# Kmatsuo57/cell-image-analysis

Measured on AMD Instinct MI355X. Metric: cells/sec screened (CAE fwd + recon-MSE + SVM score), 64x64, higher is better.
Workload: dtype f32 (results in the fp32 error class; the contractions run as split 16-bit products on the matrix pipe, fp32 accumulate: conv1..conv6 as 2 fp16 terms x 3 products with exact power-of-two scales from each cell's own data, the PCA GEMM as 3 bf16 terms x 6 products, conv7's 32 -> 16 channel contraction; 1 GPU; BASELINE.json configs[2]: screening inference, 1000000 synthetic 64x64 crops on one GPU, resident in HBM, CAE fwd + recon MSE/MAE + RobustScaler + PCA(100) + 2x OCSVM score on device; cells_per_gpu=1000000, global_cells=1000000, chunk_cells=65536, detector_train_cells=5000, weights=random init (Glorot, non-trivial BN), seed 42, parallelism=dp1

## Files before the change

### cell-image-analysis_amd/build.py

```python
import os
import subprocess
import sys
from concurrent.futures import ThreadPoolExecutor

HERE = os.path.dirname(os.path.abspath(__file__))
CSRC = os.path.join(HERE, "csrc")
OUT = os.path.join(HERE, "libcellscreen.so")
BUILD = os.path.join(HERE, "build")
SOURCES = ["api.hip", "conv_mfma.hip", "conv_out.hip", "detector.hip", "train.hip", "train_api.hip", "train_generic.hip", "preprocess.hip",
           "conv_wino_cs.hip", "conv12_fused.hip", "conv45_h2.hip", "conv_generic.hip", "conv_generic_x3.hip", "conv_wino_up.hip", "fit.hip", "extract.hip", "segment.hip", "match.hip", "expand.hip", "intensity.hip", "quantile.hip", "texture.hip", "shape.hip", "neighbors.hip", "colocalize.hip", "radial.hip"]
HEADERS = ["common.hpp", "split16.hpp", "kernel_setup.hpp", "api_internal.hpp", "train_internal.hpp", "segment_internal.hpp", "stage_host.hpp", "label_tile.hpp", "label_boxes.hpp", "hull_chain.hpp", "tensor_archive.hpp", os.path.join("..", "..", "include", "cellscreen.h")]
HIPCC = os.environ.get("HIPCC", "/opt/rocm/bin/hipcc")
FLAGS = ["-O3", "--offload-arch=gfx950", "-fPIC", "-std=c++17", "-Wall", "-Wno-unused-function",
         "-fno-gpu-rdc"]


def source_hash():
    import hashlib
    h = hashlib.sha256()
    for name in sorted(SOURCES) + sorted(HEADERS):
        with open(os.path.join(CSRC, name), "rb") as f:
            h.update(name.encode() + b"\0" + f.read() + b"\0")
    return h.hexdigest()


def _newer(target, deps):
    if not os.path.exists(target):
        return False
    t = os.path.getmtime(target)
    return all(os.path.getmtime(d) <= t for d in deps)


def build(force=False, keep_temps=False, verbose=True):
    os.makedirs(BUILD, exist_ok=True)
    hdrs = [os.path.join(CSRC, h) for h in HEADERS]
    jobs = []
    objs = []
    for src in SOURCES:
        s = os.path.join(CSRC, src)
        o = os.path.join(BUILD, src.replace(".hip", ".o"))
        objs.append(o)
        if force or not _newer(o, [s] + hdrs):
            cmd = [HIPCC] + FLAGS + ["-c", s, "-o", o]
            if keep_temps:
                cmd += ["-save-temps=obj", "-Rpass-analysis=kernel-resource-usage"]
            jobs.append(cmd)

    def run(cmd):
        r = subprocess.run(cmd, capture_output=True, text=True, cwd=BUILD)
        return cmd, r

    if jobs:
        with ThreadPoolExecutor(max_workers=4) as ex:
            for cmd, r in ex.map(run, jobs):
                if verbose and (r.stdout.strip() or r.stderr.strip()):
                    sys.stderr.write(r.stdout + r.stderr)
                if r.returncode != 0:
                    raise RuntimeError("hipcc failed: " + " ".join(cmd) + "\n" + r.stderr)
    if force or jobs or not _newer(OUT, objs):
        cmd = [HIPCC, "--offload-arch=gfx950", "-shared", "-fPIC", "-o", OUT] + objs
        r = subprocess.run(cmd, capture_output=True, text=True)
        if r.returncode != 0:
            raise RuntimeError("link failed: " + r.stderr)
    return OUT


if __name__ == "__main__":
    print(build(force="--force" in sys.argv, keep_temps="--keep-temps" in sys.argv))
```

### cell-image-analysis_amd/csrc/api.hip

```cpp
#include "api_internal.hpp"
#include "tensor_archive.hpp"

using namespace cs;

static thread_local std::string g_err;

namespace cs {
int fail(int code, const char* fmt, ...)
{
    char buf[1024];
    va_list ap;
    va_start(ap, fmt);
    vsnprintf(buf, sizeof buf, fmt, ap);
    va_end(ap);
    g_err = buf;
    return code;
}
const char* last_error_cstr() { return g_err.c_str(); }
}

static const char* kKernelNames[K_COUNT] = {"conv1_relu_bn_pool", "conv2_relu_bn_pool", "conv3_relu_bn_pool",
                                            "conv4_relu_bn",      "conv5_up_relu_bn",   "conv6_up_relu_bn",
                                            "conv7_up_sigmoid_err", "scaler_pca",       "ocsvm_decision",
                                            "finalize",           "synth_crops",        "conv6_conv7_fused_err",
                                            "conv1_conv2_fused"};

struct ConvSet {
    DevBuf winocs[3];
    DevBuf c12w1;
    DevBuf c3h2, c4h2, c5h2, c6h2;
    float c3h2_inv = 1.0f, c4h2_inv = 1.0f, c5h2_inv = 1.0f, c6h2_inv = 1.0f;
    DevBuf c12w1h2;
    float c12w1h2_inv = 1.0f;
    DevBuf c12h2;
    float c12h2_inv = 1.0f, p1a = 0.0f, p1b = 0.0f;
    DevBuf c12;
    DevBuf winoup[6];
    DevBuf wfrag[6];
    DevBuf ep[6];
    int n = 0;
};

struct GenSet {
    DevBuf w[CS_MAX_CONV], ep[CS_MAX_CONV], wf[CS_MAX_CONV], wx3[CS_MAX_CONV];
    bool folded[CS_MAX_CONV] = {false}, x3[CS_MAX_CONV] = {false};
    DevBuf wh2[CS_MAX_CONV];
    float h2_inv[CS_MAX_CONV] = {0};
};

struct Arch {
    bool ref = true;
    int H = kH, W = kW, n_conv = kNConv, n_enc = kNEnc;
    int ch[CS_MAX_CONV] = {0};
    int gh[CS_MAX_CONV] = {0}, gw[CS_MAX_CONV] = {0};
    size_t floats[CS_MAX_CONV] = {0};
    size_t npix = (size_t)kH * kW;
    size_t feat() const { return floats[n_enc - 1]; }
    int cin(int l) const { return l == 0 ? 1 : ch[l - 1]; }
};

struct ProfEvent { int kid; hipEvent_t a, b; int64_t cells; };

constexpr int64_t kPackedResultCells = 65536;

struct cs_model {
    int device = 0;
    hipStream_t stream = nullptr;
    hipStream_t copy_stream = nullptr;
    hipEvent_t ev_in[2] = {nullptr, nullptr}, ev_used[2] = {nullptr, nullptr};
    Arch arch;
    ConvSet ae, enc;
    GenSet gae, genc;
    bool shared_encoder = true;
    int precision = CS_PRECISION_SPLIT16;
    unsigned debug_flags = 0;
    bool split16 = true;
    bool fuse12 = true, fuse45 = true, fuse67 = true, small_split = true;
    int errparts = 4;
    DevBuf w7eff, b7;
    bool has_det = false;
    int F = 0, fpad = 0, C = 0, cpad = 0;
    DevBuf center, scale, comps, comps_x3, mean_proj;
    struct Svm { DevBuf svT, svn, coef; int nsv = 0, nsv_pad = 0; double gamma = 0, rho = 0; } svm[2];
    int64_t chunk = 0;
    int64_t ws_cells = 0;
    DevBuf xin, xin2, act[CS_MAX_CONV], featE, pca, errpart, dec[2], o_mse, o_mae, o_sc[2], o_pr[2], recon;
    DevBuf det_ws;
    DevBuf o_pack;
    void* h_pack = nullptr;
    size_t h_pack_bytes = 0;
    bool prof = false;
    std::vector<ProfEvent> pending;
    double prof_ms[K_COUNT] = {0};
    int64_t prof_launches[K_COUNT] = {0};
    int64_t prof_cells[K_COUNT] = {0};
    ~cs_model()
    {
        if (h_pack) (void)hipHostFree(h_pack);
        for (auto& e : pending) { (void)hipEventDestroy(e.a); (void)hipEventDestroy(e.b); }
        for (int i = 0; i < 2; ++i) {
            if (ev_in[i]) (void)hipEventDestroy(ev_in[i]);
            if (ev_used[i]) (void)hipEventDestroy(ev_used[i]);
        }
        if (copy_stream) (void)hipStreamDestroy(copy_stream);
        if (stream) (void)hipStreamDestroy(stream);
    }
};

namespace cs {
int upload(DevBuf& d, const void* src, size_t bytes)
{
    int rc = d.ensure(bytes ? bytes : 16);
    if (rc) return rc;
    if (bytes) HIPCHK(hipMemcpy(d.p, src, bytes, hipMemcpyHostToDevice));
    return CS_OK;
}

int check_arch(const cs_cae_weights* w, int expect_convs, const char* what)
{
    if (!w) return fail(CS_ERR_INVALID, "%s weights are NULL", what);
    if (w->height != kH || w->width != kW)
        return fail(CS_ERR_UNSUPPORTED, "%s: input %dx%d unsupported (this build has kernels for 64x64)", what, w->height, w->width);
    if (w->n_conv != expect_convs || (expect_convs == kNConv && w->n_enc != kNEnc))
        return fail(CS_ERR_UNSUPPORTED, "%s: n_conv=%d n_enc=%d unsupported (expected %d/%d)", what, w->n_conv, w->n_enc, expect_convs, kNEnc);
    for (int l = 0; l < expect_convs; ++l) {
        if (w->channels[l] != kRefChannels[l])
            return fail(CS_ERR_UNSUPPORTED, "%s: conv %d has %d filters, this build expects %d", what, l, w->channels[l], kRefChannels[l]);
        if (!w->kernel[l] || !w->bias[l]) return fail(CS_ERR_INVALID, "%s: conv %d kernel/bias is NULL", what, l);
        const bool has_bn = l < kNConv - 1;
        if (has_bn && (!w->bn_gamma[l] || !w->bn_beta[l] || !w->bn_mean[l] || !w->bn_var[l]))
            return fail(CS_ERR_INVALID, "%s: conv %d BatchNormalization arrays are NULL", what, l);
    }
    return CS_OK;
}

int describe_arch(const cs_cae_weights* w, Arch& a)
{
    if (!w) return fail(CS_ERR_INVALID, "autoencoder weights are NULL");
    a.H = w->height; a.W = w->width; a.n_conv = w->n_conv; a.n_enc = w->n_enc;
    if (a.n_conv < 3 || a.n_conv > CS_MAX_CONV || a.n_enc < 1 || a.n_conv != 2 * a.n_enc + 1)
        return fail(CS_ERR_UNSUPPORTED, "autoencoder: n_conv=%d n_enc=%d is not the reference grammar (n_conv = 2 n_enc + 1)", a.n_conv, a.n_enc);
    if (a.H <= 0 || a.W <= 0 || a.H % (1 << a.n_enc) || a.W % (1 << a.n_enc))
        return fail(CS_ERR_UNSUPPORTED, "autoencoder: input %dx%d is not divisible by 2^n_enc", a.H, a.W);
    a.ref = a.H == kH && a.W == kW && a.n_conv == kNConv && a.n_enc == kNEnc;
    for (int l = 0; l < a.n_conv; ++l) {
        a.ch[l] = w->channels[l];
        if (a.ch[l] <= 0) return fail(CS_ERR_INVALID, "autoencoder: conv %d has %d filters", l, a.ch[l]);
        if (a.ref && a.ch[l] != kRefChannels[l]) a.ref = false;
    }
    if (a.ch[a.n_conv - 1] != 1) return fail(CS_ERR_UNSUPPORTED, "autoencoder: the last conv must have 1 filter (has %d)", a.ch[a.n_conv - 1]);
    int h = a.H, wd = a.W;
    for (int l = 0; l < a.n_conv; ++l) {
        if (l > a.n_enc) { h *= 2; wd *= 2; }
        a.gh[l] = h; a.gw[l] = wd;
        if (l < a.n_enc) { h /= 2; wd /= 2; }
        a.floats[l] = (size_t)h * wd * a.ch[l];
    }
    a.npix = (size_t)a.H * a.W;
    if (!a.ref) {
        char why[160];
        for (int l = 0; l < a.n_conv; ++l)
            if (!conv_generic_supported(a.gh[l], a.gw[l], a.cin(l), a.ch[l], why, sizeof why))
                return fail(CS_ERR_UNSUPPORTED, "autoencoder conv %d: %s", l, why);
    }
    for (int l = 0; l < a.n_conv; ++l) {
        if (!w->kernel[l] || !w->bias[l]) return fail(CS_ERR_INVALID, "autoencoder: conv %d kernel/bias is NULL", l);
        if (l < a.n_conv - 1 && (!w->bn_gamma[l] || !w->bn_beta[l] || !w->bn_mean[l] || !w->bn_var[l]))
            return fail(CS_ERR_INVALID, "autoencoder: conv %d BatchNormalization arrays are NULL", l);
    }
    return CS_OK;
}

int check_encoder(const cs_cae_weights* e, const Arch& a)
{
    if (e->height != a.H || e->width != a.W || e->n_conv != a.n_enc)
        return fail(CS_ERR_UNSUPPORTED, "encoder: %dx%d with %d convs does not match the autoencoder's encoder half (%dx%d, %d)",
                    e->height, e->width, e->n_conv, a.H, a.W, a.n_enc);
    for (int l = 0; l < a.n_enc; ++l) {
        if (e->channels[l] != a.ch[l]) return fail(CS_ERR_UNSUPPORTED, "encoder: conv %d has %d filters, the autoencoder %d", l, e->channels[l], a.ch[l]);
        if (!e->kernel[l] || !e->bias[l] || !e->bn_gamma[l] || !e->bn_beta[l] || !e->bn_mean[l] || !e->bn_var[l])
            return fail(CS_ERR_INVALID, "encoder: conv %d arrays are NULL", l);
    }
    return CS_OK;
}

int require_gfx950(int device_id)
{
    int ndev = 0;
    if (hipGetDeviceCount(&ndev) != hipSuccess || ndev <= 0)
        return fail(CS_ERR_NO_DEVICE, "no HIP device visible; libcellscreen has no CPU path");
    if (device_id < 0 || device_id >= ndev) return fail(CS_ERR_INVALID, "device_id %d out of range [0,%d)", device_id, ndev);
    HIPCHK(hipSetDevice(device_id));
    hipDeviceProp_t prop;
    HIPCHK(hipGetDeviceProperties(&prop, device_id));
    if (strncmp(prop.gcnArchName, "gfx950", 6) != 0)
        return fail(CS_ERR_NO_DEVICE, "device %d is %s; this library is built for gfx950 only", device_id, prop.gcnArchName);
    return CS_OK;
}
}

static int pack_set(ConvSet& set, const cs_cae_weights* w, int count)
{
    std::vector<float> tmp;
    for (int l = 0; l < count; ++l) {
        const int cin = l == 0 ? 1 : kRefChannels[l - 1], cout = kRefChannels[l];
        const bool folded = (l == 4 || l == 5);
        const size_t nf = folded ? pack_conv_fragments_folded(cin, cout, nullptr, nullptr) : pack_conv_fragments(cin, cout, nullptr, nullptr);
        tmp.resize(nf);
        if (folded) pack_conv_fragments_folded(cin, cout, w->kernel[l], tmp.data());
        else pack_conv_fragments(cin, cout, w->kernel[l], tmp.data());
        int rc = upload(set.wfrag[l], tmp.data(), nf * sizeof(float));
        if (rc) return rc;
        std::vector<float> ep(3 * cout);
        for (int c = 0; c < cout; ++c) {
            const float s = w->bn_gamma[l][c] / sqrtf(w->bn_var[l][c] + w->bn_eps);
            ep[c] = w->bias[l][c];
            ep[cout + c] = s;
            ep[2 * cout + c] = w->bn_beta[l][c] - w->bn_mean[l][c] * s;
        }
        rc = upload(set.ep[l], ep.data(), ep.size() * sizeof(float));
        if (rc) return rc;
        if (l == 4 || l == 5) {
            tmp.resize(pack_wino_up_fragments(l, nullptr, nullptr));
            pack_wino_up_fragments(l, w->kernel[l], tmp.data());
            rc = upload(set.winoup[l], tmp.data(), tmp.size() * sizeof(float));
            if (rc) return rc;
        }
        if (l == 1 || l == 2) {
            tmp.resize(pack_wino_cs_fragments(l, nullptr, nullptr));
            pack_wino_cs_fragments(l, w->kernel[l], tmp.data());
            rc = upload(set.winocs[l], tmp.data(), tmp.size() * sizeof(float));
            if (rc) return rc;
        }
        if (l == 2) {
            std::vector<uint16_t> h2(pack_wino3_h2(nullptr, nullptr, nullptr));
            pack_wino3_h2(w->kernel[l], h2.data(), &set.c3h2_inv);
            rc = upload(set.c3h2, h2.data(), h2.size() * sizeof(uint16_t));
            if (rc) return rc;
        }
        if (l == 3) {
            std::vector<uint16_t> h2(pack_conv4_f16x2(nullptr, nullptr, nullptr));
            pack_conv4_f16x2(w->kernel[l], h2.data(), &set.c4h2_inv);
            rc = upload(set.c4h2, h2.data(), h2.size() * sizeof(uint16_t));
            if (rc) return rc;
        }
        if (l == 4) {
            std::vector<float> weff(pack_generic_folded(cin, cout, nullptr, nullptr));
            pack_generic_folded(cin, cout, w->kernel[l], weff.data());
            std::vector<uint16_t> h2(pack_conv5_f16x2(nullptr, nullptr, nullptr));
            pack_conv5_f16x2(weff.data(), h2.data(), &set.c5h2_inv);
            rc = upload(set.c5h2, h2.data(), h2.size() * sizeof(uint16_t));
            if (rc) return rc;
        }
        if (l == 5) {
            std::vector<float> weff(pack_generic_folded(cin, cout, nullptr, nullptr));
            pack_generic_folded(cin, cout, w->kernel[l], weff.data());
            std::vector<uint16_t> h2(pack_conv6_f16x2(nullptr, nullptr, nullptr));
            pack_conv6_f16x2(weff.data(), h2.data(), &set.c6h2_inv);
            rc = upload(set.c6h2, h2.data(), h2.size() * sizeof(uint16_t));
            if (rc) return rc;
        }
        if (l == 0) {
            tmp.resize(pack_conv12_conv1_fragments(nullptr, nullptr, nullptr));
            pack_conv12_conv1_fragments(w->kernel[l], ep.data() + cout, tmp.data());
            rc = upload(set.c12w1, tmp.data(), tmp.size() * sizeof(float));
            if (rc) return rc;
            pack_conv12_p1_bound(w->kernel[l], ep.data(), &set.p1a, &set.p1b);
            std::vector<unsigned int> wh(pack_conv12_conv1_h2(nullptr, nullptr, nullptr, nullptr));
            pack_conv12_conv1_h2(w->kernel[l], ep.data() + cout, wh.data(), &set.c12w1h2_inv);
            rc = upload(set.c12w1h2, wh.data(), wh.size() * sizeof(unsigned int));
            if (rc) return rc;
        }
        if (l == 1) {
            tmp.resize(pack_conv12_fragments(nullptr, nullptr, nullptr));
            pack_conv12_fragments(w->kernel[l], ep.data() + cout, tmp.data());
            rc = upload(set.c12, tmp.data(), tmp.size() * sizeof(float));
            if (rc) return rc;
            std::vector<unsigned int> uh(pack_conv12_fragments_h2(nullptr, nullptr, nullptr, nullptr));
            pack_conv12_fragments_h2(w->kernel[l], ep.data() + cout, uh.data(), &set.c12h2_inv);
            rc = upload(set.c12h2, uh.data(), uh.size() * sizeof(unsigned int));
            if (rc) return rc;
        }
    }
    set.n = count;
    return CS_OK;
}

static int pack_generic(GenSet& set, const cs_cae_weights* w, const Arch& a, int count, bool split16)
{
    for (int l = 0; l < count; ++l) {
        const int cin = a.cin(l), cout = a.ch[l];
        int rc = upload(set.w[l], w->kernel[l], sizeof(float) * 9 * cin * cout);
        if (rc) return rc;
        set.folded[l] = l > a.n_enc && ((l < a.n_conv - 1 && conv_generic_folds(a.gh[l], a.gw[l], cin, cout)) ||
                                        (l == a.n_conv - 1 && cout == 1 && cin % 4 == 0));
        if (set.folded[l]) {
            std::vector<float> wf(pack_generic_folded(cin, cout, nullptr, nullptr));
            pack_generic_folded(cin, cout, w->kernel[l], wf.data());
            if ((rc = upload(set.wf[l], wf.data(), wf.size() * sizeof(float)))) return rc;
            if (split16 && l == a.n_conv - 1 && cout == 1 && conv_last_x3_takes(a.gh[l], a.gw[l], cin)) {
                std::vector<uint16_t> pl(pack_last_bf16x3(cin, nullptr, nullptr));
                pack_last_bf16x3(cin, wf.data(), pl.data());
                if ((rc = upload(set.wx3[l], pl.data(), pl.size() * sizeof(uint16_t)))) return rc;
                set.x3[l] = true;
            }
            if (split16 && l < a.n_conv - 1 && conv_generic_x3_takes(a.gh[l], a.gw[l], cin, cout, 1)) {
                std::vector<uint16_t> pl(pack_generic_bf16x3(16, cin, cout, nullptr, nullptr));
                pack_generic_bf16x3(16, cin, cout, wf.data(), pl.data());
                if ((rc = upload(set.wx3[l], pl.data(), pl.size() * sizeof(uint16_t)))) return rc;
                set.x3[l] = true;
                std::vector<uint16_t> ph(pack_generic_f16x2(16, cin, cout, nullptr, nullptr, nullptr));
                pack_generic_f16x2(16, cin, cout, wf.data(), ph.data(), &set.h2_inv[l]);
                if ((rc = upload(set.wh2[l], ph.data(), ph.size() * sizeof(uint16_t)))) return rc;
            }
        } else if (split16 && l <= a.n_enc && l < a.n_conv - 1 && conv_generic_x3_takes(a.gh[l], a.gw[l], cin, cout, 0)) {
            std::vector<uint16_t> pl(pack_generic_bf16x3(9, cin, cout, nullptr, nullptr));
            pack_generic_bf16x3(9, cin, cout, w->kernel[l], pl.data());
            if ((rc = upload(set.wx3[l], pl.data(), pl.size() * sizeof(uint16_t)))) return rc;
            set.x3[l] = true;
            std::vector<uint16_t> ph(pack_generic_f16x2(9, cin, cout, nullptr, nullptr, nullptr));
            pack_generic_f16x2(9, cin, cout, w->kernel[l], ph.data(), &set.h2_inv[l]);
            if ((rc = upload(set.wh2[l], ph.data(), ph.size() * sizeof(uint16_t)))) return rc;
        }
        std::vector<float> ep(3 * cout, 0.0f);
        const bool has_bn = w->bn_gamma[l] != nullptr;
        for (int c = 0; c < cout; ++c) {
            ep[c] = w->bias[l][c];
            if (has_bn) {
                const float s_ = w->bn_gamma[l][c] / sqrtf(w->bn_var[l][c] + w->bn_eps);
                ep[cout + c] = s_;
                ep[2 * cout + c] = w->bn_beta[l][c] - w->bn_mean[l][c] * s_;
            }
        }
        if ((rc = upload(set.ep[l], ep.data(), ep.size() * sizeof(float)))) return rc;
    }
    return CS_OK;
}

static bool same_encoder(const cs_cae_weights* a, const cs_cae_weights* e, const Arch& ar)
{
    if (a->bn_eps != e->bn_eps) return false;
    for (int l = 0; l < ar.n_enc; ++l) {
        const int cin = ar.cin(l), cout = ar.ch[l];
        if (memcmp(a->kernel[l], e->kernel[l], sizeof(float) * 9 * cin * cout)) return false;
        if (memcmp(a->bias[l], e->bias[l], sizeof(float) * cout)) return false;
        if (memcmp(a->bn_gamma[l], e->bn_gamma[l], sizeof(float) * cout)) return false;
        if (memcmp(a->bn_beta[l], e->bn_beta[l], sizeof(float) * cout)) return false;
        if (memcmp(a->bn_mean[l], e->bn_mean[l], sizeof(float) * cout)) return false;
        if (memcmp(a->bn_var[l], e->bn_var[l], sizeof(float) * cout)) return false;
    }
    return true;
}

static int pack_svm(cs_model::Svm& s, const cs_ocsvm_params& p, int D, const char* what)
{
    if (p.n_sv <= 0 || !p.support_vectors || !p.dual_coef)
        return fail(CS_ERR_INVALID, "%s detector: n_sv=%d or NULL arrays", what, p.n_sv);
    s.nsv = p.n_sv;
    s.nsv_pad = (p.n_sv + 15) / 16 * 16;
    s.gamma = p.gamma;
    s.rho = p.rho;
    std::vector<double> svT((size_t)D * s.nsv_pad, 0.0), coef(s.nsv_pad, 0.0), svn(s.nsv_pad, 0.0);
    for (int i = 0; i < p.n_sv; ++i) {
        coef[i] = p.dual_coef[i];
        double nn = 0.0;
        for (int d = 0; d < D; ++d) {
            const double v = p.support_vectors[(size_t)i * D + d];
            svT[(size_t)d * s.nsv_pad + i] = v;
            nn = fma(v, v, nn);
        }
        svn[i] = nn;
    }
    {
        int rcn = upload(s.svn, svn.data(), svn.size() * sizeof(double));
        if (rcn) return rcn;
    }
    int rc = upload(s.svT, svT.data(), svT.size() * sizeof(double));
    if (rc) return rc;
    return upload(s.coef, coef.data(), coef.size() * sizeof(double));
}

static int64_t eff_chunk(const cs_model* m, int in_kind)
{
    if (m->chunk > 0) return m->chunk;
    if (in_kind == CS_MEM_HOST) return 16384;
    size_t per_cell = m->arch.npix * sizeof(float);
    for (int l = 0; l < m->arch.n_conv - 1; ++l) per_cell += m->arch.floats[l] * sizeof(float);
    int64_t c = (int64_t)((size_t)28e9 / (per_cell ? per_cell : 1));
    c = c / 1024 * 1024;
    return c < 1024 ? 1024 : (c > 65536 ? 65536 : c);
}

static int ensure_workspace(cs_model* m, int64_t cells, bool need_recon)
{
    if (cells > m->ws_cells) {
        int rc;
        if ((rc = m->xin.ensure((size_t)cells * m->arch.npix * sizeof(float)))) return rc;
        const bool skip_p1 = m->arch.ref && m->fuse12;
        for (int l = skip_p1 ? 1 : 0; l < m->arch.n_conv - 1; ++l)
            if ((rc = m->act[l].ensure((size_t)cells * m->arch.floats[l] * sizeof(float)))) return rc;
        if ((rc = m->featE.ensure((size_t)cells * m->arch.feat() * sizeof(float)))) return rc;
        if ((rc = m->pca.ensure((size_t)cells * 256 * sizeof(float)))) return rc;
        if (m->small_split && (rc = m->det_ws.ensure(det_split_ws_bytes(m->C)))) return rc;
        if ((rc = m->errpart.ensure((size_t)cells * 16 * sizeof(float)))) return rc;
        for (int d = 0; d < 2; ++d) {
            if ((rc = m->dec[d].ensure((size_t)cells * sizeof(double)))) return rc;
            if ((rc = m->o_sc[d].ensure((size_t)cells * sizeof(double)))) return rc;
            if ((rc = m->o_pr[d].ensure((size_t)cells))) return rc;
        }
        if ((rc = m->o_mse.ensure((size_t)cells * sizeof(float)))) return rc;
        if ((rc = m->o_mae.ensure((size_t)cells * sizeof(float)))) return rc;
        m->ws_cells = cells;
    }
    if (need_recon || !m->arch.ref) {
        int rc = m->recon.ensure((size_t)m->ws_cells * m->arch.npix * sizeof(float));
        if (rc) return rc;
    }
    return CS_OK;
}

struct Launch {
    cs_model* m; int kid; int64_t cells; ProfEvent ev; bool on;
    Launch(cs_model* m_, int kid_, int64_t cells_) : m(m_), kid(kid_), cells(cells_), on(m_->prof)
    {
        if (on) {
            ev.kid = kid; ev.cells = cells;
            if (hipEventCreate(&ev.a) != hipSuccess || hipEventCreate(&ev.b) != hipSuccess) { on = false; return; }
            (void)hipEventRecord(ev.a, m->stream);
        }
    }
    ~Launch()
    {
        if (on) { (void)hipEventRecord(ev.b, m->stream); m->pending.push_back(ev); }
    }
};

static int drain_profile(cs_model* m)
{
    for (auto& e : m->pending) {
        float ms = 0.0f;
        if (hipEventElapsedTime(&ms, e.a, e.b) == hipSuccess) {
            m->prof_ms[e.kid] += ms;
            m->prof_launches[e.kid] += 1;
            m->prof_cells[e.kid] += e.cells;
        }
        (void)hipEventDestroy(e.a);
        (void)hipEventDestroy(e.b);
    }
    m->pending.clear();
    return CS_OK;
}

#define LAUNCH(kid, cells, call)                                                              \
    do {                                                                                      \
        hipError_t le__;                                                                      \
        { Launch l__(m, kid, cells); le__ = (call); }                                         \
        if (le__ != hipSuccess)                                                               \
            return fail(CS_ERR_HIP, "launch %s failed: %s", kKernelNames[kid], hipGetErrorString(le__)); \
    } while (0)

static int run_convs_generic(cs_model* m, const GenSet& set, const float* x, int64_t nc, int first, int last, float* recon)
{
    const Arch& a = m->arch;
    for (int l = first; l <= last; ++l) {
        const float* in = l == 0 ? x : m->act[l - 1].as<float>();
        const bool is_last = l == a.n_conv - 1;
        float* out = is_last ? (recon ? recon : m->recon.as<float>()) : m->act[l].as<float>();
        const int epi = is_last ? GEN_EPI_SIGMOID : (l < a.n_enc ? GEN_EPI_BN_POOL : GEN_EPI_BN);
        const int kid = l < 6 ? K_CONV1 + l : K_CONV7_ERR;
        if (set.x3[l] && m->split16 && is_last) {
            LAUNCH(kid, nc,
                   launch_conv_last_x3(in, set.wx3[l].as<uint16_t>(), set.ep[l].as<float>(), out, nc, a.gh[l], a.gw[l], a.cin(l), m->stream));
            LAUNCH(K_CONV7_ERR, nc, launch_recon_err(out, x, nc, (int)a.npix, m->errpart.as<float>(), m->stream));
            continue;
        }
        if (set.x3[l] && m->split16) {
            const bool h2 = set.h2_inv[l] != 0.0f;
            LAUNCH(kid, nc,
                   launch_conv_generic_x3(in, h2 ? set.wh2[l].as<uint16_t>() : set.wx3[l].as<uint16_t>(), set.ep[l].as<float>(), out, nc,
                                          a.gh[l], a.gw[l], a.cin(l), a.ch[l], l > a.n_enc, epi, m->stream, h2 ? set.h2_inv[l] : 0.0f));
            continue;
        }
        LAUNCH(kid, nc,
               launch_conv_generic(in, set.w[l].as<float>(), set.ep[l].as<float>(), out, nc, a.gh[l], a.gw[l], a.cin(l), a.ch[l],
                                   l > a.n_enc, epi, m->stream, set.folded[l] ? set.wf[l].as<float>() : nullptr));
        if (is_last)
            LAUNCH(K_CONV7_ERR, nc, launch_recon_err(out, x, nc, (int)a.npix, m->errpart.as<float>(), m->stream));
    }
    m->errparts = 4;
    return CS_OK;
}

static int run_convs(cs_model* m, const ConvSet& set, const float* x, int64_t nc, int first, int last,
                     float* recon)
{
    if (!m->arch.ref) return run_convs_generic(m, &set == &m->enc ? m->genc : m->gae, x, nc, first, last, recon);
    const bool fused = m->fuse67 && first <= 5 && last >= 6 && !recon;
    const bool fused12 = m->fuse12 && first == 0 && last >= 1;
    const bool h2 = m->split16;
    if (fused12) {
        LAUNCH(K_CONV12_FUSED, nc,
               launch_conv12_fused(x, set.c12w1.as<float>(), set.ep[0].as<float>(), set.c12.as<float>(), set.ep[1].as<float>(),
                                   m->act[1].as<float>(), nc, m->stream, h2 ? set.c12h2.as<unsigned int>() : nullptr, set.p1a, set.p1b,
                                   set.c12h2_inv, h2 ? set.c12w1h2.as<unsigned int>() : nullptr, set.c12w1h2_inv));
    }
    if (!fused12 && first == 0) {
        int rc = m->act[0].ensure((size_t)m->ws_cells * m->arch.floats[0] * sizeof(float));
        if (rc) return rc;
    }
    const bool fused45 = m->fuse45 && h2 && first <= 3 && last >= 4;
    for (int l = fused12 ? 2 : first; l <= last && l < (fused ? 5 : 6); ++l) {
        const float* in = l == 0 ? x : m->act[l - 1].as<float>();
        if (l == 3 && fused45) {
            LAUNCH(K_CONV5, nc,
                   launch_conv45_h2(in, set.c4h2.as<uint16_t>(), set.c4h2_inv, set.ep[3].as<float>(), set.c5h2.as<uint16_t>(), set.c5h2_inv,
                                    set.ep[4].as<float>(), m->act[4].as<float>(), nc, m->stream));
            ++l;
            continue;
        }
        if (l == 4 && h2) {
            LAUNCH(K_CONV5, nc,
                   launch_conv5_h2(in, set.c5h2.as<uint16_t>(), set.c5h2_inv, set.ep[l].as<float>(), m->act[l].as<float>(), nc, m->stream));
            continue;
        }
        if (l == 4 || l == 5) {
            LAUNCH(K_CONV1 + l, nc,
                   launch_conv_wino_up(l, in, set.winoup[l].as<float>(), set.ep[l].as<float>(), m->act[l].as<float>(), nc, m->stream));
            continue;
        }
        if (l == 2 && h2) {
            LAUNCH(K_CONV3, nc,
                   launch_conv3_wino_h2(in, set.c3h2.as<uint16_t>(), set.c3h2_inv, set.ep[l].as<float>(), m->act[l].as<float>(), nc, m->stream));
            continue;
        }
        if (l == 1 || l == 2) {
            LAUNCH(K_CONV1 + l, nc,
                   launch_conv_wino_cs(l, in, set.winocs[l].as<float>(), set.ep[l].as<float>(), m->act[l].as<float>(), nc, m->stream));
            continue;
        }
        if (l == 3 && h2) {
            LAUNCH(K_CONV4, nc,
                   launch_conv4_h2(in, set.c4h2.as<uint16_t>(), set.c4h2_inv, set.ep[l].as<float>(), m->act[l].as<float>(), nc, m->stream));
            continue;
        }
        LAUNCH(K_CONV1 + l, nc,
               launch_conv_mfma(l, in, set.wfrag[l].as<float>(), set.ep[l].as<float>(), m->act[l].as<float>(), nc, m->stream, false));
    }
    if (fused && h2) {
        LAUNCH(K_CONV67_FUSED, nc,
               launch_conv67_h2(m->act[4].as<float>(), set.c6h2.as<uint16_t>(), set.c6h2_inv, set.ep[5].as<float>(), x, m->w7eff.as<float>(),
                                m->b7.as<float>(), m->errpart.as<float>(), nc, m->stream));
        m->errparts = conv67_fused_nparts();
    } else if (fused) {
        LAUNCH(K_CONV67_FUSED, nc,
               launch_conv67_fused(m->act[4].as<float>(), set.winoup[5].as<float>(), set.ep[5].as<float>(), x, m->w7eff.as<float>(),
                                   m->b7.as<float>(), m->errpart.as<float>(), nc, m->stream));
        m->errparts = conv67_fused_nparts();
    } else if (last >= 6) {
        LAUNCH(K_CONV7_ERR, nc,
               launch_conv7_err(m->act[5].as<float>(), x, m->w7eff.as<float>(), m->b7.as<float>(), m->errpart.as<float>(), recon, nc, m->stream));
        m->errparts = 4;
    }
    return CS_OK;
}

struct DrainGuard {
    cs_model* m;
    bool armed = true;
    explicit DrainGuard(cs_model* mm) : m(mm) {}
    ~DrainGuard()
    {
        if (armed && m) {
            if (m->copy_stream) (void)hipStreamSynchronize(m->copy_stream);
            if (m->stream) (void)hipStreamSynchronize(m->stream);
        }
    }
    int done(int rc) { armed = false; return rc; }
};

static int begin_call(cs_model* m)
{
    if (!m) return fail(CS_ERR_INVALID, "model handle is NULL");
    HIPCHK(hipSetDevice(m->device));
    return CS_OK;
}

static int end_call(cs_model* m)
{
    HIPCHK(hipStreamSynchronize(m->stream));
    return drain_profile(m);
}

static int stage_in(cs_model* m, const float* base, int kind, int64_t off, int64_t nc, size_t per_cell,
                    DevBuf& staging, const float** dev)
{
    if (kind == CS_MEM_DEVICE) { *dev = base + (size_t)off * per_cell; return CS_OK; }
    int rc = staging.ensure((size_t)nc * per_cell * sizeof(float));
    if (rc) return rc;
    HIPCHK(hipMemcpyAsync(staging.p, base + (size_t)off * per_cell, (size_t)nc * per_cell * sizeof(float),
                          hipMemcpyHostToDevice, m->stream));
    *dev = staging.as<float>();
    return CS_OK;
}

template <class T>
static int stage_out(cs_model* m, T* user, int kind, int64_t off, int64_t count, const T* dev)
{
    if (!user || kind == CS_MEM_DEVICE) return CS_OK;
    HIPCHK(hipMemcpyAsync(user + off, dev, (size_t)count * sizeof(T), hipMemcpyDeviceToHost, m->stream));
    return CS_OK;
}

template <class T>
static T* out_ptr(T* user, int kind, int64_t off, DevBuf& tmp)
{
    if (!user) return nullptr;
    return kind == CS_MEM_DEVICE ? user + off : tmp.as<T>();
}

static int check_kind(int k, const char* what)
{
    if (k != CS_MEM_HOST && k != CS_MEM_DEVICE) return fail(CS_ERR_INVALID, "%s must be CS_MEM_HOST or CS_MEM_DEVICE", what);
    return CS_OK;
}

extern "C" {

int cs_abi_version(void) { return CS_ABI_VERSION; }

const char* cs_status_string(int s)
{
    switch (s) {
        case CS_OK: return "ok";
        case CS_ERR_INVALID: return "invalid argument";
        case CS_ERR_IO: return "i/o error";
        case CS_ERR_FORMAT: return "malformed model file";
        case CS_ERR_NO_DEVICE: return "no usable gfx950 device";
        case CS_ERR_HIP: return "HIP runtime error";
        case CS_ERR_UNSUPPORTED: return "unsupported architecture or size";
        case CS_ERR_NOMEM: return "out of memory";
        case CS_ERR_NO_DETECTOR: return "model has no detector parameters";
        default: return "unknown status";
    }
}

const char* cs_last_error(void) { return last_error_cstr(); }

int cs_device_count(void)
{
    int n = 0;
    if (hipGetDeviceCount(&n) != hipSuccess) return 0;
    return n;
}

static int resolve_options(const cs_model_options* o, int* precision, unsigned* flags)
{
    *precision = CS_PRECISION_SPLIT16;
    *flags = 0;
    if (o) {
        if (o->struct_size < 12 || o->struct_size > 4096) return fail(CS_ERR_INVALID, "cs_model_options.struct_size = %u (set it to sizeof(cs_model_options))", o->struct_size);
        if (o->precision != CS_PRECISION_SPLIT16 && o->precision != CS_PRECISION_FP32_EXACT)
            return fail(CS_ERR_INVALID, "cs_model_options.precision = %d (CS_PRECISION_SPLIT16 or CS_PRECISION_FP32_EXACT)", o->precision);
        const unsigned known = CS_DEBUG_NO_FUSE12 | CS_DEBUG_NO_FUSE45 | CS_DEBUG_NO_FUSE67 | CS_DEBUG_NO_SMALL_SPLIT;
        if (o->debug_flags & ~known) return fail(CS_ERR_INVALID, "cs_model_options.debug_flags = 0x%x has unknown bits", o->debug_flags);
        if (o->struct_size >= sizeof(cs_model_options))
            for (unsigned r : o->reserved) if (r) return fail(CS_ERR_INVALID, "cs_model_options.reserved must be 0");
        *precision = o->precision;
        *flags = o->debug_flags;
    }
    if (const char* e = getenv("CS_DEBUG_PRECISION")) {
        if (!strcmp(e, "exact")) *precision = CS_PRECISION_FP32_EXACT;
        else if (!strcmp(e, "split16")) *precision = CS_PRECISION_SPLIT16;
        else return fail(CS_ERR_INVALID, "CS_DEBUG_PRECISION=%s (exact or split16)", e);
    }
    if (const char* e = getenv("CS_DEBUG_FLAGS")) *flags |= (unsigned)strtoul(e, nullptr, 0) & 0xfu;
    return CS_OK;
}

int cs_model_from_arrays(const cs_cae_weights* autoencoder, const cs_cae_weights* encoder,
                         const cs_detector_params* det, int device_id, const cs_model_options* options, cs_model** out)
{
    if (!out) return fail(CS_ERR_INVALID, "out is NULL");
    *out = nullptr;
    int precision;
    unsigned dflags;
    {
        int rco = resolve_options(options, &precision, &dflags);
        if (rco) return rco;
    }
    Arch arch;
    int rc = describe_arch(autoencoder, arch);
    if (rc) return rc;
    if (arch.ref && (rc = check_arch(autoencoder, kNConv, "autoencoder"))) return rc;
    if (encoder && (rc = check_encoder(encoder, arch))) return rc;
    if ((rc = require_gfx950(device_id))) return rc;

    cs_model* m = new (std::nothrow) cs_model();
    if (!m) return fail(CS_ERR_NOMEM, "host allocation failed");
    m->device = device_id;
    m->arch = arch;
    m->precision = precision;
    m->debug_flags = dflags;
    m->split16 = precision == CS_PRECISION_SPLIT16;
    m->fuse12 = !(dflags & CS_DEBUG_NO_FUSE12);
    m->fuse45 = !(dflags & CS_DEBUG_NO_FUSE45);
    m->fuse67 = !(dflags & CS_DEBUG_NO_FUSE67);
    m->small_split = !(dflags & CS_DEBUG_NO_SMALL_SPLIT);
#define FAIL_IF(x) do { int r__ = (x); if (r__) { delete m; return r__; } } while (0)
    {
        hipError_t e = hipStreamCreateWithFlags(&m->stream, hipStreamNonBlocking);
        if (e == hipSuccess) e = hipStreamCreateWithFlags(&m->copy_stream, hipStreamNonBlocking);
        for (int i = 0; i < 2 && e == hipSuccess; ++i) {
            e = hipEventCreateWithFlags(&m->ev_in[i], hipEventDisableTiming);
            if (e == hipSuccess) e = hipEventCreateWithFlags(&m->ev_used[i], hipEventDisableTiming);
        }
        if (e != hipSuccess) { delete m; return fail(CS_ERR_HIP, "stream/event creation: %s", hipGetErrorString(e)); }
    }
    if (arch.ref) {
        FAIL_IF(pack_set(m->ae, autoencoder, 6));
        float weff[16 * 32];
        conv7_effective_weights(autoencoder->kernel[6], weff);
        FAIL_IF(upload(m->w7eff, weff, sizeof weff));
        FAIL_IF(upload(m->b7, autoencoder->bias[6], sizeof(float)));
    } else {
        FAIL_IF(pack_generic(m->gae, autoencoder, arch, arch.n_conv, m->split16));
    }
    m->shared_encoder = !encoder || same_encoder(autoencoder, encoder, arch);
    if (!m->shared_encoder) {
        if (arch.ref) FAIL_IF(pack_set(m->enc, encoder, kNEnc));
        else FAIL_IF(pack_generic(m->genc, encoder, arch, arch.n_enc, m->split16));
    }

    if (det) {
        if (det->n_features != (int)arch.feat()) {
            delete m;
            return fail(CS_ERR_INVALID, "detector n_features=%d but the encoder emits %zu", det->n_features, arch.feat());
        }
        if (det->n_components <= 0 || det->n_components > 128 || !det->scaler_center || !det->scaler_scale ||
            !det->pca_components || !det->pca_mean_proj) {
            delete m;
            return fail(CS_ERR_INVALID, "detector: n_components=%d (1..128) or NULL arrays", det->n_components);
        }
        m->F = det->n_features;
        m->fpad = (m->F + 511) / 512 * 512;
        m->C = det->n_components;
        m->cpad = (m->C + 15) / 16 * 16;
        FAIL_IF(upload(m->center, det->scaler_center, sizeof(float) * m->F));
        FAIL_IF(upload(m->scale, det->scaler_scale, sizeof(double) * m->F));
        std::vector<float> cp((size_t)m->cpad * m->fpad, 0.0f);
        for (int c = 0; c < m->C; ++c)
            memcpy(&cp[(size_t)c * m->fpad], det->pca_components + (size_t)c * m->F, sizeof(float) * m->F);
        FAIL_IF(upload(m->comps, cp.data(), cp.size() * sizeof(float)));
        {
            std::vector<uint16_t> pl(pack_pca_bf16x3(nullptr, m->cpad, m->fpad, nullptr));
            pack_pca_bf16x3(cp.data(), m->cpad, m->fpad, pl.data());
            FAIL_IF(upload(m->comps_x3, pl.data(), pl.size() * sizeof(uint16_t)));
        }
        FAIL_IF(upload(m->mean_proj, det->pca_mean_proj, sizeof(float) * m->C));
        FAIL_IF(pack_svm(m->svm[0], det->conservative, m->C, "conservative"));
        FAIL_IF(pack_svm(m->svm[1], det->moderate, m->C, "moderate"));
        m->has_det = true;
    }
#undef FAIL_IF
    *out = m;
    return CS_OK;
}

static int fill_weights(const TensorArchive& ar, const std::string& prefix, int n_conv, cs_cae_weights* w,
                        const std::string& path)
{
    for (int l = 0; l < n_conv; ++l) {
        const int cin = l == 0 ? 1 : w->channels[l - 1], cout = w->channels[l];
        const std::string cl = prefix + ".conv" + std::to_string(l), bl = prefix + ".bn" + std::to_string(l);
        const Tensor* k = ar.get(cl + ".kernel");
        const Tensor* b = ar.get(cl + ".bias");
        if (!k || !b || !k->f32() || !b->f32() || k->numel() != (size_t)9 * cin * cout || b->numel() != (size_t)cout)
            return fail(CS_ERR_FORMAT, "%s: missing or mis-shaped %s.kernel/.bias", path.c_str(), cl.c_str());
        w->kernel[l] = k->f32();
        w->bias[l] = b->f32();
        if (l < w->n_conv - 1 || prefix == "enc") {
            const Tensor* g = ar.get(bl + ".gamma"); const Tensor* be = ar.get(bl + ".beta");
            const Tensor* mu = ar.get(bl + ".mean"); const Tensor* va = ar.get(bl + ".var");
            if (!g || !be || !mu || !va || !g->f32() || !be->f32() || !mu->f32() || !va->f32() ||
                g->numel() != (size_t)cout || be->numel() != (size_t)cout || mu->numel() != (size_t)cout || va->numel() != (size_t)cout)
                return fail(CS_ERR_FORMAT, "%s: missing or mis-shaped %s.*", path.c_str(), bl.c_str());
            w->bn_gamma[l] = g->f32(); w->bn_beta[l] = be->f32(); w->bn_mean[l] = mu->f32(); w->bn_var[l] = va->f32();
        }
    }
    return CS_OK;
}

static int fill_svm(const TensorArchive& ar, const std::string& prefix, int C, cs_ocsvm_params* p, const std::string& path)
{
    const Tensor* sv = ar.get(prefix + ".sv"); const Tensor* dc = ar.get(prefix + ".dual_coef");
    const Tensor* g = ar.get(prefix + ".gamma"); const Tensor* r = ar.get(prefix + ".rho");
    if (!sv || !dc || !g || !r || !sv->f64() || !dc->f64() || !g->f64() || !r->f64() || sv->dims.size() != 2 ||
        sv->dims[1] != (uint64_t)C || dc->numel() != sv->dims[0] || g->numel() != 1 || r->numel() != 1)
        return fail(CS_ERR_FORMAT, "%s: missing or mis-shaped %s.*", path.c_str(), prefix.c_str());
    p->n_sv = (int32_t)sv->dims[0];
    p->support_vectors = sv->f64();
    p->dual_coef = dc->f64();
    p->gamma = g->f64()[0];
    p->rho = r->f64()[0];
    return CS_OK;
}

int cs_model_load(const char* model_dir, int device_id, const cs_model_options* options, cs_model** out)
{
    if (!out) return fail(CS_ERR_INVALID, "out is NULL");
    *out = nullptr;
    if (!model_dir) return fail(CS_ERR_INVALID, "model_dir is NULL");
    const std::string dir(model_dir);
    TensorArchive cae, det;
    std::string err = cae.load(dir + "/cae.bin");
    if (!err.empty()) return fail(err.rfind("cannot open", 0) == 0 ? CS_ERR_IO : CS_ERR_FORMAT, "%s", err.c_str());

    const Tensor* meta = cae.get("meta");
    const Tensor* eps = cae.get("bn_eps");
    if (!meta || !meta->i32() || meta->numel() < 5 || !eps || !eps->f32() || eps->numel() != 1)
        return fail(CS_ERR_FORMAT, "%s/cae.bin: missing meta / bn_eps", model_dir);
    const int32_t* mi = meta->i32();
    cs_cae_weights ae;
    memset(&ae, 0, sizeof ae);
    ae.height = mi[0]; ae.width = mi[1]; ae.n_conv = mi[2]; ae.n_enc = mi[3];
    if (ae.n_conv < 2 || ae.n_conv > CS_MAX_CONV || meta->numel() != (size_t)(4 + ae.n_conv))
        return fail(CS_ERR_FORMAT, "%s/cae.bin: bad meta", model_dir);
    for (int l = 0; l < ae.n_conv; ++l) ae.channels[l] = mi[4 + l];
    ae.bn_eps = eps->f32()[0];
    int rc = fill_weights(cae, "ae", ae.n_conv, &ae, dir + "/cae.bin");
    if (rc) return rc;

    cs_cae_weights en;
    const cs_cae_weights* enp = nullptr;
    if (cae.get("enc.conv0.kernel")) {
        en = ae;
        en.n_conv = ae.n_enc;
        for (int l = 0; l < CS_MAX_CONV; ++l) en.kernel[l] = en.bias[l] = en.bn_gamma[l] = en.bn_beta[l] = en.bn_mean[l] = en.bn_var[l] = nullptr;
        rc = fill_weights(cae, "enc", en.n_conv, &en, dir + "/cae.bin");
        if (rc) return rc;
        enp = &en;
    }

    cs_detector_params dp;
    const cs_detector_params* dpp = nullptr;
    FILE* probe = fopen((dir + "/detector.bin").c_str(), "rb");
    if (probe) {
        fclose(probe);
        err = det.load(dir + "/detector.bin");
        if (!err.empty()) return fail(CS_ERR_FORMAT, "%s", err.c_str());
        memset(&dp, 0, sizeof dp);
        const Tensor* ce = det.get("scaler.center"); const Tensor* sc = det.get("scaler.scale");
        const Tensor* co = det.get("pca.components"); const Tensor* mp = det.get("pca.mean_proj");
        if (!ce || !sc || !co || !mp || !ce->f32() || !sc->f64() || !co->f32() || !mp->f32() || co->dims.size() != 2 ||
            ce->numel() != co->dims[1] || sc->numel() != co->dims[1] || mp->numel() != co->dims[0])
            return fail(CS_ERR_FORMAT, "%s/detector.bin: missing or mis-shaped scaler/pca tensors", model_dir);
        dp.n_features = (int32_t)co->dims[1];
        dp.n_components = (int32_t)co->dims[0];
        dp.scaler_center = ce->f32(); dp.scaler_scale = sc->f64();
        dp.pca_components = co->f32(); dp.pca_mean_proj = mp->f32();
        if ((rc = fill_svm(det, "svm_conservative", dp.n_components, &dp.conservative, dir + "/detector.bin"))) return rc;
        if ((rc = fill_svm(det, "svm_moderate", dp.n_components, &dp.moderate, dir + "/detector.bin"))) return rc;
        dpp = &dp;
    }
    return cs_model_from_arrays(&ae, enp, dpp, device_id, options, out);
}

void cs_model_free(cs_model* m)
{
    if (!m) return;
    (void)hipSetDevice(m->device);
    if (m->stream) (void)hipStreamSynchronize(m->stream);
    delete m;
}

int cs_model_get_info(const cs_model* m, cs_model_info* info)
{
    if (!m || !info) return fail(CS_ERR_INVALID, "NULL argument");
    memset(info, 0, sizeof *info);
    info->height = m->arch.H; info->width = m->arch.W; info->n_conv = m->arch.n_conv; info->n_enc = m->arch.n_enc;
    info->feature_dim = (int32_t)m->arch.feat();
    for (int l = 0; l < m->arch.n_conv; ++l) info->channels[l] = m->arch.ch[l];
    info->reference_arch = m->arch.ref ? 1 : 0;
    info->precision = m->precision;
    info->debug_flags = m->debug_flags;
    info->n_components = m->C;
    info->n_sv_conservative = m->svm[0].nsv;
    info->n_sv_moderate = m->svm[1].nsv;
    info->shared_encoder = m->shared_encoder ? 1 : 0;
    info->has_detector = m->has_det ? 1 : 0;
    info->device_id = m->device;
    info->chunk_cells = eff_chunk(m, CS_MEM_DEVICE);
    return CS_OK;
}

int cs_model_set_chunk(cs_model* m, int64_t chunk_cells)
{
    if (!m || chunk_cells < 0 || chunk_cells > (1 << 20)) return fail(CS_ERR_INVALID, "chunk_cells must be in [0, 2^20] (0 = automatic)");
    m->chunk = chunk_cells;
    return CS_OK;
}

static int run_tail(cs_model* m, const float* feat, int64_t nc, float* mse, float* mae, double* sc, double* sm,
                    int8_t* pc, int8_t* pm, bool with_err)
{
    if (m->split16)
        LAUNCH(K_SCALER_PCA, nc,
               launch_scaler_pca_x3(feat, m->center.as<float>(), m->scale.as<double>(), m->comps_x3.as<uint16_t>(),
                                    m->mean_proj.as<float>(), m->F, m->fpad, m->C, m->cpad, m->pca.as<float>(), nc, m->stream, m->det_ws.p));
    else
        LAUNCH(K_SCALER_PCA, nc,
               launch_scaler_pca(feat, m->center.as<float>(), m->scale.as<double>(), m->comps.as<float>(),
                                 m->mean_proj.as<float>(), m->F, m->fpad, m->C, m->cpad, m->pca.as<float>(), nc, m->stream));
    if (m->det_ws.p && nc <= DET_SPLIT_MAX_CELLS) {
        const double* svT[2] = {m->svm[0].svT.as<double>(), m->svm[1].svT.as<double>()};
        const double* svn[2] = {m->svm[0].svn.as<double>(), m->svm[1].svn.as<double>()};
        const double* coef[2] = {m->svm[0].coef.as<double>(), m->svm[1].coef.as<double>()};
        const int nsv[2] = {m->svm[0].nsv_pad, m->svm[1].nsv_pad};
        const double gam[2] = {m->svm[0].gamma, m->svm[1].gamma}, rho[2] = {m->svm[0].rho, m->svm[1].rho};
        LAUNCH(K_SVM, nc,
               launch_ocsvm_pair_split(m->pca.as<float>(), m->C, svT, svn, coef, nsv, gam, rho, m->dec[0].as<double>(), m->dec[1].as<double>(), nc,
                                       m->stream, m->det_ws.p));
    } else
    for (int d = 0; d < 2; ++d)
        LAUNCH(K_SVM, nc,
               launch_ocsvm(m->pca.as<float>(), m->C, m->svm[d].svT.as<double>(), m->svm[d].svn.as<double>(), m->svm[d].coef.as<double>(),
                            m->svm[d].nsv_pad, m->svm[d].gamma, m->svm[d].rho, m->dec[d].as<double>(), nc, m->stream, m->det_ws.p));
    LAUNCH(K_FINALIZE, nc,
           launch_finalize(with_err ? m->errpart.as<float>() : nullptr, m->errparts, (int)m->arch.npix, m->dec[0].as<double>(),
                           m->dec[1].as<double>(), mse, mae, sc, sm, pc, pm, nc, m->stream));
    return CS_OK;
}

int cs_screen(cs_model* m, const float* crops, int64_t n, int crops_kind, float* mse, float* mae,
              double* cons_score, double* mod_score, int8_t* cons_pred, int8_t* mod_pred, int out_kind)
{
    int rc = begin_call(m);
    if (rc) return rc;
    DrainGuard guard(m);
    if (n < 0) return fail(CS_ERR_INVALID, "n is negative");
    if (n == 0) return guard.done(CS_OK);
    if (!crops) return fail(CS_ERR_INVALID, "crops is NULL");
    if ((rc = check_kind(crops_kind, "crops_kind")) || (rc = check_kind(out_kind, "out_kind"))) return rc;
    if (!m->has_det) return fail(CS_ERR_NO_DETECTOR, "cs_screen needs detector parameters");
    const int64_t cc = eff_chunk(m, crops_kind);
    const int64_t ch = n < cc ? n : cc;
    if ((rc = ensure_workspace(m, ch, false))) return rc;
    const bool host_in = crops_kind == CS_MEM_HOST, host_out = out_kind == CS_MEM_HOST;
    const size_t in_bytes = m->arch.npix * sizeof(float);
    DevBuf* stage[2] = {&m->xin, &m->xin2};
    const bool single = n <= ch;
    if (host_in) {
        if ((rc = m->xin.ensure((size_t)ch * in_bytes)) || (n > ch && (rc = m->xin2.ensure((size_t)ch * in_bytes)))) return rc;
        HIPCHK(hipMemcpyAsync(m->xin.p, crops, (size_t)ch * in_bytes, hipMemcpyHostToDevice, single ? m->stream : m->copy_stream));
        if (!single) HIPCHK(hipEventRecord(m->ev_in[0], m->copy_stream));
    }
    const size_t o_off[6] = {0, (size_t)n * 8, (size_t)n * 16, (size_t)n * 20, (size_t)n * 24, (size_t)n * 25};
    const size_t o_total = (size_t)n * 26;
    const bool pack_out = host_out && n <= kPackedResultCells;
    if (host_out) {
        if ((rc = m->o_pack.ensure(o_total))) return rc;
        if (pack_out && m->h_pack_bytes < o_total) {
            if (m->h_pack) { (void)hipHostFree(m->h_pack); m->h_pack = nullptr; m->h_pack_bytes = 0; }
            const size_t cap = (size_t)kPackedResultCells * 26;
            HIPCHK(hipHostMalloc(&m->h_pack, cap, hipHostMallocDefault));
            m->h_pack_bytes = cap;
        }
    }
    char* const o_base = (char*)m->o_pack.p;
    auto dst = [&](auto* user, int which, int64_t off) -> decltype(user) {
        if (!user) return nullptr;
        return host_out ? (decltype(user))(o_base + o_off[which]) + off : user + off;
    };
    auto drain = [&](int code) {
        (void)hipStreamSynchronize(m->copy_stream);
        (void)hipStreamSynchronize(m->stream);
        return code;
    };
    int64_t i = 0;
    for (int64_t off = 0; off < n; off += ch, ++i) {
        const int64_t nc = (n - off) < ch ? (n - off) : ch;
        const int b = (int)(i & 1);
        const float* x = crops + (size_t)off * m->arch.npix;
        if (host_in) {
            if (!single) HIPCHK(hipStreamWaitEvent(m->stream, m->ev_in[b], 0));
            x = stage[b]->as<float>();
        }
        if ((rc = run_convs(m, m->ae, x, nc, 0, m->arch.n_conv - 1, nullptr))) return drain(rc);
        const float* feat = m->act[m->arch.n_enc - 1].as<float>();
        if (!m->shared_encoder) {
            if ((rc = run_convs(m, m->enc, x, nc, 0, m->arch.n_enc - 1, nullptr))) return drain(rc);
            feat = m->act[m->arch.n_enc - 1].as<float>();
        }
        if ((rc = run_tail(m, feat, nc, dst(mse, 2, off), dst(mae, 3, off), dst(cons_score, 0, off),
                           dst(mod_score, 1, off), dst(cons_pred, 4, off), dst(mod_pred, 5, off), true)))
            return drain(rc);
        if (host_in && !single) {
            HIPCHK(hipEventRecord(m->ev_used[b], m->stream));
            const int64_t noff = off + ch;
            if (noff < n) {
                const int64_t nn = (n - noff) < ch ? (n - noff) : ch;
                if (i >= 1) HIPCHK(hipStreamWaitEvent(m->copy_stream, m->ev_used[b ^ 1], 0));
                HIPCHK(hipMemcpyAsync(stage[b ^ 1]->p, crops + (size_t)noff * m->arch.npix, (size_t)nn * in_bytes, hipMemcpyHostToDevice,
                                      m->copy_stream));
                HIPCHK(hipEventRecord(m->ev_in[b ^ 1], m->copy_stream));
            }
        }
    }
    if (pack_out) {
        HIPCHK(hipMemcpyAsync(m->h_pack, o_base, o_total, hipMemcpyDeviceToHost, m->stream));
        if (host_in) HIPCHK(hipStreamSynchronize(m->copy_stream));
        const int erc = end_call(m);
        if (erc) return guard.done(erc);
        const char* h = (const char*)m->h_pack;
        if (cons_score) memcpy(cons_score, h + o_off[0], (size_t)n * 8);
        if (mod_score) memcpy(mod_score, h + o_off[1], (size_t)n * 8);
        if (mse) memcpy(mse, h + o_off[2], (size_t)n * 4);
        if (mae) memcpy(mae, h + o_off[3], (size_t)n * 4);
        if (cons_pred) memcpy(cons_pred, h + o_off[4], (size_t)n);
        if (mod_pred) memcpy(mod_pred, h + o_off[5], (size_t)n);
        return guard.done(CS_OK);
    }
    if (host_out) {
        if (mse) HIPCHK(hipMemcpyAsync(mse, o_base + o_off[2], (size_t)n * sizeof(float), hipMemcpyDeviceToHost, m->stream));
        if (mae) HIPCHK(hipMemcpyAsync(mae, o_base + o_off[3], (size_t)n * sizeof(float), hipMemcpyDeviceToHost, m->stream));
        if (cons_score) HIPCHK(hipMemcpyAsync(cons_score, o_base + o_off[0], (size_t)n * sizeof(double), hipMemcpyDeviceToHost, m->stream));
        if (mod_score) HIPCHK(hipMemcpyAsync(mod_score, o_base + o_off[1], (size_t)n * sizeof(double), hipMemcpyDeviceToHost, m->stream));
        if (cons_pred) HIPCHK(hipMemcpyAsync(cons_pred, o_base + o_off[4], (size_t)n, hipMemcpyDeviceToHost, m->stream));
        if (mod_pred) HIPCHK(hipMemcpyAsync(mod_pred, o_base + o_off[5], (size_t)n, hipMemcpyDeviceToHost, m->stream));
    }
    if (host_in) HIPCHK(hipStreamSynchronize(m->copy_stream));
    return guard.done(end_call(m));
}

int cs_reconstruct(cs_model* m, const float* crops, int64_t n, int crops_kind, float* recon, float* mse,
                   float* mae, int out_kind)
{
    int rc = begin_call(m);
    if (rc) return rc;
    DrainGuard guard(m);
    if (n < 0) return fail(CS_ERR_INVALID, "n is negative");
    if (n == 0) return guard.done(CS_OK);
    if (!crops) return fail(CS_ERR_INVALID, "crops is NULL");
    if ((rc = check_kind(crops_kind, "crops_kind")) || (rc = check_kind(out_kind, "out_kind"))) return rc;
    const int64_t cc = eff_chunk(m, crops_kind);
    const int64_t ch = n < cc ? n : cc;
    const bool host_recon = recon && out_kind == CS_MEM_HOST;
    if ((rc = ensure_workspace(m, ch, host_recon))) return rc;
    for (int64_t off = 0; off < n; off += ch) {
        const int64_t nc = (n - off) < ch ? (n - off) : ch;
        const float* x;
        if ((rc = stage_in(m, crops, crops_kind, off, nc, m->arch.npix, m->xin, &x))) return rc;
        float* d_rec = !recon ? nullptr : (out_kind == CS_MEM_DEVICE ? recon + (size_t)off * m->arch.npix : m->recon.as<float>());
        if ((rc = run_convs(m, m->ae, x, nc, 0, m->arch.n_conv - 1, d_rec))) return rc;
        float* d_mse = out_ptr(mse, out_kind, off, m->o_mse);
        float* d_mae = out_ptr(mae, out_kind, off, m->o_mae);
        LAUNCH(K_FINALIZE, nc,
               launch_finalize(m->errpart.as<float>(), m->errparts, (int)m->arch.npix, nullptr, nullptr, d_mse, d_mae, nullptr, nullptr,
                               nullptr, nullptr, nc, m->stream));
        if ((rc = stage_out(m, mse, out_kind, off, nc, d_mse))) return rc;
        if ((rc = stage_out(m, mae, out_kind, off, nc, d_mae))) return rc;
        if (host_recon)
            HIPCHK(hipMemcpyAsync(recon + (size_t)off * m->arch.npix, d_rec, (size_t)nc * m->arch.npix * sizeof(float),
                                  hipMemcpyDeviceToHost, m->stream));
        if (crops_kind == CS_MEM_HOST || out_kind == CS_MEM_HOST) HIPCHK(hipStreamSynchronize(m->stream));
    }
    return guard.done(end_call(m));
}

int cs_encode(cs_model* m, const float* crops, int64_t n, int crops_kind, int which, float* features, int out_kind)
{
    int rc = begin_call(m);
    if (rc) return rc;
    DrainGuard guard(m);
    if (n < 0) return fail(CS_ERR_INVALID, "n is negative");
    if (n == 0) return guard.done(CS_OK);
    if (!crops || !features) return fail(CS_ERR_INVALID, "crops/features is NULL");
    if (which != 0 && which != 1) return fail(CS_ERR_INVALID, "which must be 0 (autoencoder) or 1 (encoder.keras)");
    if ((rc = check_kind(crops_kind, "crops_kind")) || (rc = check_kind(out_kind, "out_kind"))) return rc;
    const int64_t cc = eff_chunk(m, crops_kind);
    const int64_t ch = n < cc ? n : cc;
    if ((rc = ensure_workspace(m, ch, false))) return rc;
    const ConvSet& set = (which == 1 && !m->shared_encoder) ? m->enc : m->ae;
    const size_t fl = m->arch.feat();
    for (int64_t off = 0; off < n; off += ch) {
        const int64_t nc = (n - off) < ch ? (n - off) : ch;
        const float* x;
        if ((rc = stage_in(m, crops, crops_kind, off, nc, m->arch.npix, m->xin, &x))) return rc;
        if ((rc = run_convs(m, set, x, nc, 0, m->arch.n_enc - 1, nullptr))) return rc;
        HIPCHK(hipMemcpyAsync(features + (size_t)off * fl, m->act[m->arch.n_enc - 1].p, (size_t)nc * fl * sizeof(float),
                              out_kind == CS_MEM_DEVICE ? hipMemcpyDeviceToDevice : hipMemcpyDeviceToHost, m->stream));
        HIPCHK(hipStreamSynchronize(m->stream));
    }
    return guard.done(end_call(m));
}

int cs_layer_output(cs_model* m, const float* crops, int64_t n, int crops_kind, int layer, float* out, int out_kind)
{
    int rc = begin_call(m);
    if (rc) return rc;
    DrainGuard guard(m);
    if (n < 0) return fail(CS_ERR_INVALID, "n is negative");
    if (n == 0) return guard.done(CS_OK);
    if (!crops || !out) return fail(CS_ERR_INVALID, "crops/out is NULL");
    const int last = m->arch.n_conv - 1;
    if (layer < 0 || layer > last) return fail(CS_ERR_INVALID, "layer must be in [0,%d]", last);
    if ((rc = check_kind(crops_kind, "crops_kind")) || (rc = check_kind(out_kind, "out_kind"))) return rc;
    const int64_t cc = eff_chunk(m, crops_kind);
    const int64_t ch = n < cc ? n : cc;
    if ((rc = ensure_workspace(m, ch, layer == last))) return rc;
    const size_t fl = m->arch.floats[layer];
    for (int64_t off = 0; off < n; off += ch) {
        const int64_t nc = (n - off) < ch ? (n - off) : ch;
        const float* x;
        if ((rc = stage_in(m, crops, crops_kind, off, nc, m->arch.npix, m->xin, &x))) return rc;
        if ((rc = run_convs(m, m->ae, x, nc, 0, layer, layer == last ? m->recon.as<float>() : nullptr))) return rc;
        const void* src = layer == last ? m->recon.p : m->act[layer].p;
        HIPCHK(hipMemcpyAsync(out + (size_t)off * fl, src, (size_t)nc * fl * sizeof(float),
                              out_kind == CS_MEM_DEVICE ? hipMemcpyDeviceToDevice : hipMemcpyDeviceToHost, m->stream));
        HIPCHK(hipStreamSynchronize(m->stream));
    }
    return guard.done(end_call(m));
}

int cs_scaler_pca(cs_model* m, const float* features, int64_t n, int in_kind, float* pca_out, int out_kind)
{
    int rc = begin_call(m);
    if (rc) return rc;
    DrainGuard guard(m);
    if (n < 0) return fail(CS_ERR_INVALID, "n is negative");
    if (n == 0) return guard.done(CS_OK);
    if (!features || !pca_out) return fail(CS_ERR_INVALID, "features/pca_out is NULL");
    if ((rc = check_kind(in_kind, "in_kind")) || (rc = check_kind(out_kind, "out_kind"))) return rc;
    if (!m->has_det) return fail(CS_ERR_NO_DETECTOR, "cs_scaler_pca needs detector parameters");
    const int64_t cc = eff_chunk(m, in_kind);
    const int64_t ch = n < cc ? n : cc;
    if ((rc = ensure_workspace(m, ch, false))) return rc;
    for (int64_t off = 0; off < n; off += ch) {
        const int64_t nc = (n - off) < ch ? (n - off) : ch;
        const float* f;
        if ((rc = stage_in(m, features, in_kind, off, nc, (size_t)m->F, m->featE, &f))) return rc;
        if (m->split16)
            LAUNCH(K_SCALER_PCA, nc,
                   launch_scaler_pca_x3(f, m->center.as<float>(), m->scale.as<double>(), m->comps_x3.as<uint16_t>(),
                                        m->mean_proj.as<float>(), m->F, m->fpad, m->C, m->cpad, m->pca.as<float>(), nc, m->stream, m->det_ws.p));
        else
            LAUNCH(K_SCALER_PCA, nc,
                   launch_scaler_pca(f, m->center.as<float>(), m->scale.as<double>(), m->comps.as<float>(),
                                     m->mean_proj.as<float>(), m->F, m->fpad, m->C, m->cpad, m->pca.as<float>(), nc, m->stream));
        HIPCHK(hipMemcpyAsync(pca_out + (size_t)off * m->C, m->pca.p, (size_t)nc * m->C * sizeof(float),
                              out_kind == CS_MEM_DEVICE ? hipMemcpyDeviceToDevice : hipMemcpyDeviceToHost, m->stream));
        HIPCHK(hipStreamSynchronize(m->stream));
    }
    return guard.done(end_call(m));
}

int cs_svm_decision(cs_model* m, const float* pca, int64_t n, int in_kind, double* cons_dec, double* mod_dec, int out_kind)
{
    int rc = begin_call(m);
    if (rc) return rc;
    DrainGuard guard(m);
    if (n < 0) return fail(CS_ERR_INVALID, "n is negative");
    if (n == 0) return guard.done(CS_OK);
    if (!pca) return fail(CS_ERR_INVALID, "pca is NULL");
    if ((rc = check_kind(in_kind, "in_kind")) || (rc = check_kind(out_kind, "out_kind"))) return rc;
    if (!m->has_det) return fail(CS_ERR_NO_DETECTOR, "cs_svm_decision needs detector parameters");
    const int64_t cc = eff_chunk(m, in_kind);
    const int64_t ch = n < cc ? n : cc;
    if ((rc = ensure_workspace(m, ch, false))) return rc;
    double* outs[2] = {cons_dec, mod_dec};
    for (int64_t off = 0; off < n; off += ch) {
        const int64_t nc = (n - off) < ch ? (n - off) : ch;
        const float* p;
        if ((rc = stage_in(m, pca, in_kind, off, nc, (size_t)m->C, m->pca, &p))) return rc;
        for (int d = 0; d < 2; ++d) {
            if (!outs[d]) continue;
            LAUNCH(K_SVM, nc,
                   launch_ocsvm(p, m->C, m->svm[d].svT.as<double>(), m->svm[d].svn.as<double>(), m->svm[d].coef.as<double>(),
                                m->svm[d].nsv_pad, m->svm[d].gamma, m->svm[d].rho, m->dec[d].as<double>(), nc, m->stream, m->det_ws.p));
            HIPCHK(hipMemcpyAsync(outs[d] + off, m->dec[d].p, (size_t)nc * sizeof(double),
                                  out_kind == CS_MEM_DEVICE ? hipMemcpyDeviceToDevice : hipMemcpyDeviceToHost, m->stream));
        }
        HIPCHK(hipStreamSynchronize(m->stream));
    }
    return guard.done(end_call(m));
}

int cs_synth_crops(cs_model* m, uint64_t seed, int64_t first_cell, int64_t n, int32_t npix, float* out_device)
{
    int rc = begin_call(m);
    if (rc) return rc;
    if (n < 0 || npix <= 0) return fail(CS_ERR_INVALID, "n/npix invalid");
    if (n == 0) return CS_OK;
    if (!out_device) return fail(CS_ERR_INVALID, "out_device is NULL");
    LAUNCH(K_SYNTH, n, launch_synth(seed, first_cell, n, npix, out_device, m->stream));
    return end_call(m);
}

int cs_profile_enable(cs_model* m, int on)
{
    if (!m) return fail(CS_ERR_INVALID, "model handle is NULL");
    m->prof = on != 0;
    return CS_OK;
}

int cs_profile_reset(cs_model* m)
{
    if (!m) return fail(CS_ERR_INVALID, "model handle is NULL");
    for (int k = 0; k < K_COUNT; ++k) { m->prof_ms[k] = 0; m->prof_launches[k] = 0; m->prof_cells[k] = 0; }
    return CS_OK;
}

int cs_model_wait_stream(cs_model* m, void* hip_stream)
{
    if (!m) return fail(CS_ERR_INVALID, "model handle is NULL");
    HIPCHK(hipSetDevice(m->device));
    return wait_on_stream(m->stream, hip_stream);
}

int cs_profile_kernel_count(void) { return K_COUNT; }

const char* cs_profile_kernel_name(int k) { return (k >= 0 && k < K_COUNT) ? kKernelNames[k] : ""; }

int cs_profile_get(cs_model* m, int k, double* total_ms, int64_t* launches, int64_t* cells, double* flops)
{
    if (!m || k < 0 || k >= K_COUNT) return fail(CS_ERR_INVALID, "bad kernel id");
    if (total_ms) *total_ms = m->prof_ms[k];
    if (launches) *launches = m->prof_launches[k];
    if (cells) *cells = m->prof_cells[k];
    if (flops) {
        double per_cell = 0.0;
        if (k <= K_CONV7_ERR) per_cell = 2.0 * kLayerMacs[k];
        else if (k == K_CONV67_FUSED) per_cell = 2.0 * (kLayerMacs[5] + kLayerMacs[6]);
        else if (k == K_CONV12_FUSED) per_cell = 2.0 * (kLayerMacs[0] + kLayerMacs[1]);
        else if (k == K_SCALER_PCA) per_cell = 2.0 * (double)m->F * m->C;
        else if (k == K_SVM) per_cell = 0.0;
        *flops = per_cell * (double)m->prof_cells[k];
    }
    return CS_OK;
}

int cs_profile_mfma_per_cell(cs_model* m, int k, double* mfma)
{
    if (!m || !mfma || k < 0 || k >= K_COUNT) return fail(CS_ERR_INVALID, "bad kernel id");
    double v = 0.0;
    if (k == K_SCALER_PCA) {
        *mfma = m->has_det && !m->split16 ? (double)m->fpad * m->cpad / 1024.0 : 0.0;
        return CS_OK;
    }
    if (m->arch.ref) {
        const bool h2 = m->split16;
        switch (k) {
            case K_CONV1: v = 1536; break;
            case K_CONV2: v = 8192; break;
            case K_CONV3: v = h2 ? 0 : 2048; break;
            case K_CONV4: v = h2 ? 0 : 576; break;
            case K_CONV5: v = h2 ? 0 : 1152; break;
            case K_CONV6: v = 4608; break;
            case K_CONV67_FUSED: v = h2 ? 512 : 4608 + 512; break;
            case K_CONV12_FUSED: v = h2 ? 0 : 4608 + 1536 + 48; break;
            default: v = 0.0;
        }
    } else if (k <= K_CONV6 || k == K_CONV7_ERR) {
        const int l = k == K_CONV7_ERR ? m->arch.n_conv - 1 : k - K_CONV1;
        if (l < m->arch.n_conv && !(m->split16 && m->gae.x3[l])) {
            const int cout_pad = (m->arch.ch[l] + 15) / 16 * 16;
            v = (double)m->arch.gh[l] * m->arch.gw[l] / 16.0 * (cout_pad / 16) * (9.0 * m->arch.cin(l) / 4.0);
        }
    }
    *mfma = v;
    return CS_OK;
}

int cs_profile_bf16_mfma_per_cell(cs_model* m, int k, double* mfma)
{
    if (!m || !mfma || k < 0 || k >= K_COUNT) return fail(CS_ERR_INVALID, "bad kernel id");
    double v = 0.0;
    if (!m->split16) { *mfma = 0.0; return CS_OK; }
    if (k == K_SCALER_PCA && m->has_det) {
        *mfma = (double)(m->cpad / 16) * (m->fpad / 32) * 6.0 / 16.0;
        return CS_OK;
    }
    if (m->arch.ref) {
        if (k == K_CONV4) v = 4 * 2 * 9 * 3;
        if (k == K_CONV3) v = 16.0 * 4 * 2 * 2 * 3;
        if (k == K_CONV12_FUSED) v = 66 * 8 * 2 + 36 * 4 * 4 * 3;
        if (k == K_CONV5) v = 4 * 4 * 4 * 4 * 3 + (m->fuse45 ? 4 * 2 * 9 * 3 : 0);
        if (k == K_CONV67_FUSED) v = 4.0 * 16 * 2 * 4 * 2 * 3;
    } else if (k <= K_CONV6) {
        const int l = k - K_CONV1;
        if (l < m->arch.n_conv && m->gae.x3[l]) {
            const int cout_pad = (m->arch.ch[l] + 15) / 16 * 16;
            const double taps = l > m->arch.n_enc ? 4.0 : 9.0;
            const bool last = l == m->arch.n_conv - 1;
            v = (double)m->arch.gh[l] * m->arch.gw[l] / 16.0 * (cout_pad / 16) * taps * (m->arch.cin(l) / 32.0) * ((m->gae.h2_inv[l] != 0.0f && !last) ? 3.0 : 6.0);
        }
    }
    *mfma = v;
    return CS_OK;
}

}
```

### cell-image-analysis_amd/csrc/common.hpp

```cpp
#pragma once
#include <hip/hip_runtime.h>
#include <stdint.h>
#include <stdio.h>

#include "../../include/cellscreen.h"

namespace cs {

typedef float f32x4 __attribute__((ext_vector_type(4)));

struct LayerGeom {
    int H, W, cin, cout;
    bool pool;
    bool ups;
    bool last;
};

enum KernelId {
    K_CONV1 = 0, K_CONV2, K_CONV3, K_CONV4, K_CONV5, K_CONV6, K_CONV7_ERR,
    K_SCALER_PCA, K_SVM, K_FINALIZE, K_SYNTH, K_CONV67_FUSED, K_CONV12_FUSED, K_COUNT
};

hipError_t launch_conv_mfma(int layer, const float* in, const float* wfrag, const float* ep,
                            float* out, int64_t n_cells, hipStream_t stream, bool folded = false);
size_t pack_conv_fragments_folded(int cin, int cout, const float* hwio, float* dst);
hipError_t launch_conv_wino_cs(int layer, const float* in, const float* ufrag, const float* ep, float* out, int64_t n_cells,
                               hipStream_t stream);
size_t pack_wino_cs_fragments(int layer, const float* hwio, float* dst);
hipError_t launch_conv3_wino_h2(const float* in, const uint16_t* uplanes, float inv_sw, const float* ep, float* out, int64_t n_cells,
                                hipStream_t stream);
size_t pack_wino3_h2(const float* hwio, uint16_t* dst, float* inv_sw);
hipError_t launch_conv12_fused(const float* x, const float* w1frag, const float* ep1, const float* ufrag, const float* ep2, float* p2,
                               int64_t n_cells, hipStream_t stream, const unsigned int* ufrag_h2 = nullptr,
                               float p1a = 0.0f, float p1b = 0.0f, float inv_sw = 1.0f, const unsigned int* w1h2 = nullptr, float inv_sw1 = 1.0f);
size_t pack_conv12_conv1_h2(const float* hwio, const float* bn_scale, unsigned int* dst, float* inv_sw1);
size_t pack_conv12_fragments_h2(const float* hwio, const float* bn_scale, unsigned int* dst, float* inv_sw);
void pack_conv12_p1_bound(const float* hwio1, const float* ep1, float* a1, float* b1);
size_t pack_conv12_fragments(const float* hwio, const float* bn_scale, float* dst);
size_t pack_conv12_conv1_fragments(const float* hwio, const float* bn_scale, float* dst);
hipError_t launch_conv4_h2(const float* in, const uint16_t* wfrag, float inv_sw, const float* ep, float* out, int64_t n_cells, hipStream_t stream);
size_t pack_conv4_f16x2(const float* hwio, uint16_t* dst, float* inv_sw);
hipError_t launch_conv5_h2(const float* in, const uint16_t* wfrag, float inv_sw, const float* ep, float* out, int64_t n_cells, hipStream_t stream);
hipError_t launch_conv45_h2(const float* in, const uint16_t* w4, float inv_sw4, const float* ep4, const uint16_t* w5, float inv_sw5,
                            const float* ep5, float* out, int64_t n_cells, hipStream_t stream);
size_t pack_conv5_f16x2(const float* weff, uint16_t* dst, float* inv_sw);
hipError_t launch_conv_wino_up(int layer, const float* in, const float* ufrag, const float* ep, float* out, int64_t n_cells,
                               hipStream_t stream);
size_t pack_wino_up_fragments(int layer, const float* hwio, float* dst);
size_t pack_conv_fragments(int cin, int cout, const float* hwio, float* dst);

hipError_t launch_conv67_fused(const float* a5, const float* ufrag, const float* ep, const float* x, const float* weff_dev,
                               const float* b7_dev, float* errpart, int64_t n_cells, hipStream_t stream);
int conv67_fused_nparts();
hipError_t launch_conv67_h2(const float* a5, const uint16_t* wplanes, float inv_sw, const float* ep, const float* x, const float* weff_dev,
                            const float* b7_dev, float* errpart, int64_t n_cells, hipStream_t stream);
size_t pack_conv6_f16x2(const float* weff, uint16_t* dst, float* inv_sw);

hipError_t launch_conv7_err(const float* a6, const float* x, const float* weff_dev, const float* b7_dev,
                            float* errpart, float* recon, int64_t n_cells, hipStream_t stream);
hipError_t launch_conv7_err_train(const float* a6, const float* x, const float* weff_dev, const float* b7_dev, float* errpart,
                                  float* recon, float* dz, float* dzsum_part, int64_t n_cells, hipStream_t stream);
void conv7_effective_weights(const float* w7_hwio, float* weff);

constexpr int TRAIN_MAX_PARTS = 256;
constexpr int BN_MAX_PARTS = 1024;
struct ReduceDesc { long dst; long len; const float* src; int nparts; long stride; };
hipError_t launch_conv_train_fwd(int layer, const float* in, const float* wfrag, const float* bias,
                                 float* relu_out, int64_t n_cells, hipStream_t stream, float* stats_part = nullptr,
                                 int* stats_parts = nullptr);
hipError_t launch_conv_dgrad(int layer, const float* dz, const float* wfrag_t, float* dx, int64_t n_cells,
                             hipStream_t stream);
hipError_t launch_bn_stats(const float* r, long P, int C, float* part, int* G, hipStream_t s);
hipError_t launch_bn_stats_final(const float* part, int G, int C, float eps, float momentum, float* mov_mean,
                                 float* mov_var, float* stats, hipStream_t s);
hipError_t launch_bn_stats_merge(const float* part, int G, int C, float* out , hipStream_t s);
hipError_t launch_bn_apply(const float* r, int C, const float* gamma, const float* beta, const float* stats, float* a,
                           long N, int H, int W, int pool, hipStream_t s);
hipError_t launch_loss_dz(const float* out, const float* y, long total, float* dz, float* dzsum_part, int* G, hipStream_t s,
                          const float* errpart = nullptr, long nparts = 0, float* out2 = nullptr);
hipError_t launch_loss_scalar(const float* errpart, long nparts, long nelem, float* out2, hipStream_t s);
hipError_t launch_bn_bwd_reduce(const float* da, const float* r, const float* stats, const float* gamma, const float* beta,
                                long N, int H, int W, int C, int pool, float* part, int* G, hipStream_t s);
hipError_t launch_bn_bwd_final(const float* part, int G, int C, double nred, float* sums, float* dgamma, float* dbeta,
                               hipStream_t s);
hipError_t launch_bn_bwd_dz(const float* da, const float* r, const float* stats, const float* gamma, const float* beta,
                            const float* sums, long N, int H, int W, int C, int pool, float* dz, float* dzsum_part,
                            int* Gz, hipStream_t s);
hipError_t launch_wgrad(int layer, const float* xin, const float* dz, float* part, int64_t n_cells, int* nparts,
                        hipStream_t s);
hipError_t launch_reduce_all(const ReduceDesc* descs_dev, int ndesc, long total_len, float* flat_grad, hipStream_t s,
                             const float* errpart = nullptr, long nparts = 0, long nelem = 0, float* out2 = nullptr);
hipError_t launch_adam(float* p, const float* g, float* m, float* v, long n, float alpha, float b1, float b2, float eps, hipStream_t s,
                       const float* batch_scal, double* macc);
enum { GEN_EPI_BN = 0, GEN_EPI_BN_POOL = 1, GEN_EPI_SIGMOID = 2, GEN_EPI_RELU = 3, GEN_EPI_PLAIN = 4 };
int conv_generic_supported(int H, int W, int cin, int cout, char* why, size_t why_len);
hipError_t launch_conv_generic(const float* in, const float* w_hwio, const float* ep, float* out, int64_t n, int H, int W, int cin,
                               int cout, int ups, int epi, hipStream_t stream, const float* w_folded = nullptr);
size_t pack_generic_folded(int cin, int cout, const float* hwio, float* dst);
int conv_generic_x3_takes(int H, int W, int cin, int cout, int ups);
size_t pack_generic_bf16x3(int ntaps, int cin, int cout, const float* w, uint16_t* dst);
hipError_t launch_pack_generic_bf16x3(const float* w, int ntaps, int cin, int cout, uint16_t* dst, hipStream_t stream);
hipError_t launch_conv_generic_x3(const float* in, const uint16_t* wplanes, const float* ep, float* out, int64_t n, int H, int W, int cin,
                                  int cout, int ups, int epi, hipStream_t stream, float inv_sw = 0.0f);
size_t pack_generic_f16x2(int ntaps, int cin, int cout, const float* w, uint16_t* dst, float* inv_sw);
int conv_last_x3_takes(int H, int W, int cin);
size_t pack_last_bf16x3(int cin, const float* weff, uint16_t* dst);
hipError_t launch_conv_last_x3(const float* in, const uint16_t* wplanes, const float* ep, float* out, int64_t n, int H, int W, int cin,
                               hipStream_t stream);
int conv_generic_folds(int H, int W, int cin, int cout);
hipError_t launch_flip_transpose(const float* hwio, int cin, int cout, float* dst, hipStream_t s);
hipError_t launch_sumpool2x2(const float* in, float* out, int64_t n, int H, int W, int C, hipStream_t s);
size_t wgrad_generic_lds_bytes(int W, int cin, int cout);
hipError_t launch_wgrad_generic(const float* xin, const float* dz, float* part, int64_t n, int H, int W, int cin, int cout, int ups,
                                int max_parts, int* nparts, hipStream_t s);
hipError_t launch_recon_err(const float* recon, const float* x, int64_t n, int npix, float* errpart, hipStream_t stream);
hipError_t launch_augment(const float* in, const cs_aug_affine* tf_dev, float* out, int64_t n, int H, int W, hipStream_t s);
hipError_t launch_fit_gather(const float* train, const cs_aug_affine* tf, const int* idx, float* x_out, float* y_out, int64_t n, int H,
                             int W, bool has_tf, hipStream_t s);
struct PackJob { const float* src; float* dst; int cin, cout, transposed, blocks; };
struct PackTable { PackJob job[16]; int n; };
hipError_t launch_pack_all(PackTable& tab, hipStream_t s);
hipError_t launch_pack_frag(const float* hwio, int cin, int cout, int transposed, float* dst, hipStream_t s);
hipError_t launch_pack_w7eff(const float* w7, float* weff, hipStream_t s);
hipError_t launch_pack_ep(const float* bias, const float* gamma, const float* beta, const float* mov_mean,
                          const float* mov_var, float eps, int C, float* ep, hipStream_t s);

hipError_t launch_scaler_pca(const float* feat, const float* center, const double* scale,
                             const float* comps_pad, const float* mean_proj, int F, int fpad, int C,
                             int cpad, float* pca_out, int64_t n_cells, hipStream_t stream);

hipError_t launch_scaler_pca_x3(const float* feat, const float* center, const double* scale, const uint16_t* comps_planes,
                                const float* mean_proj, int F, int fpad, int C, int cpad, float* pca_out, int64_t n_cells,
                                hipStream_t stream, void* split_ws = nullptr);
constexpr int64_t DET_SPLIT_MAX_CELLS = 16384;
size_t det_split_ws_bytes(int C);
size_t pack_pca_bf16x3(const float* comps_pad, int cpad, int fpad, uint16_t* dst);

hipError_t launch_ocsvm(const float* pca, int D, const double* svT , const double* svn ,
                        const double* coef, int nsv_pad, double gamma, double rho, double* dec, int64_t n_cells, hipStream_t stream,
                        void* split_ws = nullptr);

hipError_t launch_ocsvm_pair_split(const float* pca, int D, const double* const svT[2], const double* const svn[2],
                                   const double* const coef[2], const int nsv_pad[2], const double gamma[2], const double rho[2],
                                   double* dec0, double* dec1, int64_t n_cells, hipStream_t stream, void* split_ws);

hipError_t launch_finalize(const float* errpart, int nparts, int npix, const double* dec_c,
                           const double* dec_m, float* mse, float* mae, double* score_c,
                           double* score_m, int8_t* pred_c, int8_t* pred_m, int64_t n_cells,
                           hipStream_t stream);

hipError_t launch_synth(uint64_t seed, int64_t first_cell, int64_t n, int npix, float* out,
                        hipStream_t stream);

}
```

### cell-image-analysis_amd/csrc/detector.hip

```cpp
#include "common.hpp"
#include "kernel_setup.hpp"

#include <cstring>

namespace cs {

namespace {

constexpr int PCA_MT = 4;
constexpr int PCA_CELLS = 16 * PCA_MT;
constexpr int PCA_KC = 256;
constexpr int PCA_LD = PCA_KC + 4;
constexpr int PCA_LDS = PCA_CELLS * PCA_LD * 4;

__global__ __launch_bounds__(256) void scaler_pca_kernel(
    const float* __restrict__ feat, const float* __restrict__ center, const double* __restrict__ scale,
    const float* __restrict__ comps, const float* __restrict__ mean_proj, int F, int fpad, int C,
    int cpad, float* __restrict__ out, long n)
{
    extern __shared__ __attribute__((aligned(16))) char smem[];
    float* xs = (float*)smem;
    const int tid = threadIdx.x, lane = tid & 63;
    const int wave = __builtin_amdgcn_readfirstlane(tid >> 6);
    const int li = lane & 15, kq = lane >> 4;
    const long cell0 = (long)blockIdx.x * PCA_CELLS;
    const int ntiles = cpad / 16;

    f32x4 acc[2][PCA_MT];
#pragma unroll
    for (int t = 0; t < 2; ++t)
#pragma unroll
        for (int m = 0; m < PCA_MT; ++m) acc[t][m] = f32x4{0.0f, 0.0f, 0.0f, 0.0f};

    static_assert(PCA_KC == 256, "one feature column per thread");
    float raw[PCA_CELLS];
    auto issue = [&](int k0) {
        const int gk = k0 + tid < F ? k0 + tid : F - 1;
#pragma unroll
        for (int c = 0; c < PCA_CELLS; ++c) {
            const long cell = cell0 + c < n ? cell0 + c : n - 1;
            raw[c] = feat[cell * F + gk];
        }
    };
    auto stash = [&](int k0) {
        const int gk = k0 + tid;
        const bool kok = gk < F;
        const float ctr = center[kok ? gk : 0];
        const double scl = scale[kok ? gk : 0];
#pragma unroll
        for (int c = 0; c < PCA_CELLS; ++c) {
            const float t = raw[c] - ctr;
            const float v = (float)((double)t / scl);
            xs[c * PCA_LD + tid] = (kok && cell0 + c < n) ? v : 0.0f;
        }
    };
    issue(0);
    for (int k0 = 0; k0 < fpad; k0 += PCA_KC) {
        stash(k0);
        __syncthreads();
        if (k0 + PCA_KC < fpad) issue(k0 + PCA_KC);
        const float* bp[2];
#pragma unroll
        for (int t = 0; t < 2; ++t) {
            const int tile = wave + 4 * t < ntiles ? wave + 4 * t : 0;
            bp[t] = comps + (size_t)(tile * 16 + li) * fpad + k0 + kq * 4;
        }
        f32x4 b[2] = {*(const f32x4*)bp[0], *(const f32x4*)bp[1]};
#pragma unroll 2
        for (int ks = 0; ks < PCA_KC / 16; ++ks) {
            f32x4 a[PCA_MT];
#pragma unroll
            for (int m = 0; m < PCA_MT; ++m)
                a[m] = *(const f32x4*)(xs + (m * 16 + li) * PCA_LD + ks * 16 + kq * 4);
            const int kn = ks + 1 < PCA_KC / 16 ? ks + 1 : ks;
            const f32x4 nb[2] = {*(const f32x4*)(bp[0] + kn * 16), *(const f32x4*)(bp[1] + kn * 16)};
#pragma unroll
            for (int t = 0; t < 2; ++t) {
                if (wave + 4 * t < ntiles) {
#pragma unroll
                    for (int j = 0; j < 4; ++j)
#pragma unroll
                        for (int m = 0; m < PCA_MT; ++m)
                            acc[t][m] = __builtin_amdgcn_mfma_f32_16x16x4f32(a[m][j], b[t][j], acc[t][m], 0, 0, 0);
                }
            }
            b[0] = nb[0];
            b[1] = nb[1];
        }
        __syncthreads();
    }
#pragma unroll
    for (int t = 0; t < 2; ++t) {
        const int comp = (wave + 4 * t) * 16 + li;
        if (wave + 4 * t < ntiles && comp < C) {
            const float mp = mean_proj[comp];
#pragma unroll
            for (int m = 0; m < PCA_MT; ++m)
#pragma unroll
                for (int r = 0; r < 4; ++r) {
                    const long cell = cell0 + m * 16 + 4 * kq + r;
                    if (cell < n) out[cell * C + comp] = acc[t][m][r] - mp;
                }
        }
    }
}

typedef __bf16 bf16x8 __attribute__((ext_vector_type(8)));
typedef __bf16 bf16x2 __attribute__((ext_vector_type(2)));
constexpr int PX_KC = 128;
constexpr int PX_ROW = PX_KC * 2 + 32;
constexpr int PX_PLANE = PCA_CELLS * PX_ROW;
constexpr int PX_LDS = 3 * PX_PLANE;

constexpr int DET_RANGES = 8;

template <bool SPLIT>
__global__ __launch_bounds__(256) void scaler_pca_x3_kernel(
    const float* __restrict__ feat, const float* __restrict__ center, const double* __restrict__ scale,
    const bf16x8* __restrict__ comps , const float* __restrict__ mean_proj, int F, int fpad, int C,
    int cpad, float* __restrict__ out , long n)
{
    extern __shared__ __attribute__((aligned(16))) char smem[];
    const int tid = threadIdx.x, lane = tid & 63;
    const int wave = __builtin_amdgcn_readfirstlane(tid >> 6);
    const int li = lane & 15, kq = lane >> 4;
    const long cell0 = (long)blockIdx.x * PCA_CELLS;
    const int ntiles = cpad / 16;
    const int nkb = fpad / 32;

    f32x4 acc[2][PCA_MT], tot[2][PCA_MT];
#pragma unroll
    for (int t = 0; t < 2; ++t)
#pragma unroll
        for (int m = 0; m < PCA_MT; ++m) acc[t][m] = tot[t][m] = f32x4{0.0f, 0.0f, 0.0f, 0.0f};
    const int nch = fpad / PX_KC;
    int rj = SPLIT ? (int)blockIdx.y : 0;
    const int kbeg = SPLIT ? (nch * rj / DET_RANGES) * PX_KC : 0;
    const int kend = SPLIT ? (nch * (rj + 1) / DET_RANGES) * PX_KC : fpad;

    const int fp = tid & 63, cg = tid >> 6;
    float raw[16][2];
    auto issue = [&](int k0) {
        const int g0 = k0 + 2 * fp < F ? k0 + 2 * fp : F - 1, g1 = k0 + 2 * fp + 1 < F ? k0 + 2 * fp + 1 : F - 1;
#pragma unroll
        for (int c = 0; c < 16; ++c) {
            const long cell = cell0 + cg * 16 + c < n ? cell0 + cg * 16 + c : n - 1;
            raw[c][0] = feat[cell * F + g0];
            raw[c][1] = feat[cell * F + g1];
        }
    };
    auto stash = [&](int k0) {
        const int gk = k0 + 2 * fp;
        const bool ok0 = gk < F, ok1 = gk + 1 < F;
        const float ctr0 = center[ok0 ? gk : 0], ctr1 = center[ok1 ? gk + 1 : 0];
        const double scl0 = scale[ok0 ? gk : 0], scl1 = scale[ok1 ? gk + 1 : 0];
        char* d = smem + (cg * 16) * PX_ROW + fp * 4;
#pragma unroll
        for (int c = 0; c < 16; ++c) {
            const bool cok = cell0 + cg * 16 + c < n;
            float v[2];
            v[0] = (ok0 && cok) ? (float)((double)(raw[c][0] - ctr0) / scl0) : 0.0f;
            v[1] = (ok1 && cok) ? (float)((double)(raw[c][1] - ctr1) / scl1) : 0.0f;
            bf16x2 h1, h2, h3;
#pragma unroll
            for (int j = 0; j < 2; ++j) {
                const __bf16 a1 = (__bf16)v[j];
                const float r1 = v[j] - (float)a1;
                const __bf16 a2 = (__bf16)r1;
                const float r2 = r1 - (float)a2;
                h1[j] = a1; h2[j] = a2; h3[j] = (__bf16)r2;
            }
            *(bf16x2*)(d + c * PX_ROW) = h1;
            *(bf16x2*)(d + c * PX_ROW + PX_PLANE) = h2;
            *(bf16x2*)(d + c * PX_ROW + 2 * PX_PLANE) = h3;
        }
    };
    const bf16x8* bp[2];
#pragma unroll
    for (int t = 0; t < 2; ++t) {
        const int tile = wave + 4 * t < ntiles ? wave + 4 * t : 0;
        bp[t] = comps + (size_t)tile * nkb * 3 * 64 + lane;
    }
    auto load_b = [&](int kb, bf16x8 (&b)[2][3]) {
#pragma unroll
        for (int t = 0; t < 2; ++t)
#pragma unroll
            for (int p = 0; p < 3; ++p) b[t][p] = bp[t][((size_t)kb * 3 + p) * 64];
    };
    bf16x8 bn[2][3];
    if (kbeg < kend) {
        issue(kbeg);
        load_b(kbeg / 32, bn);
    }
    for (int k0 = kbeg; k0 < kend; k0 += PX_KC) {
        stash(k0);
        __syncthreads();
        if (k0 + PX_KC < kend) issue(k0 + PX_KC);
#pragma unroll
        for (int ks = 0; ks < PX_KC / 32; ++ks) {
            bf16x8 b[2][3];
#pragma unroll
            for (int t = 0; t < 2; ++t)
#pragma unroll
                for (int p = 0; p < 3; ++p) b[t][p] = bn[t][p];
            const int kb = k0 / 32 + ks;
            if (kb + 1 < kend / 32) load_b(kb + 1, bn);
#pragma unroll
            for (int m = 0; m < PCA_MT; ++m) {
                const char* ap = smem + (m * 16 + li) * PX_ROW + ks * 64 + kq * 16;
                const bf16x8 a1 = *(const bf16x8*)ap;
                const bf16x8 a2 = *(const bf16x8*)(ap + PX_PLANE);
                const bf16x8 a3 = *(const bf16x8*)(ap + 2 * PX_PLANE);
#pragma unroll
                for (int t = 0; t < 2; ++t) {
                    if (wave + 4 * t < ntiles) {
                        acc[t][m] = __builtin_amdgcn_mfma_f32_16x16x32_bf16(a1, b[t][2], acc[t][m], 0, 0, 0);
                        acc[t][m] = __builtin_amdgcn_mfma_f32_16x16x32_bf16(a2, b[t][1], acc[t][m], 0, 0, 0);
                        acc[t][m] = __builtin_amdgcn_mfma_f32_16x16x32_bf16(a3, b[t][0], acc[t][m], 0, 0, 0);
                        acc[t][m] = __builtin_amdgcn_mfma_f32_16x16x32_bf16(a1, b[t][1], acc[t][m], 0, 0, 0);
                        acc[t][m] = __builtin_amdgcn_mfma_f32_16x16x32_bf16(a2, b[t][0], acc[t][m], 0, 0, 0);
                        acc[t][m] = __builtin_amdgcn_mfma_f32_16x16x32_bf16(a1, b[t][0], acc[t][m], 0, 0, 0);
                    }
                }
            }
        }
        __syncthreads();
        while (rj < DET_RANGES && (nch * (rj + 1) / DET_RANGES) * PX_KC <= k0 + PX_KC) {
            if ((nch * (rj + 1) / DET_RANGES) * PX_KC == k0 + PX_KC) {
#pragma unroll
                for (int t = 0; t < 2; ++t)
#pragma unroll
                    for (int m = 0; m < PCA_MT; ++m) { tot[t][m] += acc[t][m]; acc[t][m] = f32x4{0.0f, 0.0f, 0.0f, 0.0f}; }
            }
            ++rj;
            if (SPLIT) break;
        }
    }
#pragma unroll
    for (int t = 0; t < 2; ++t) {
        const int comp = (wave + 4 * t) * 16 + li;
        if (wave + 4 * t < ntiles && comp < C) {
            const float mp = SPLIT ? 0.0f : mean_proj[comp];
#pragma unroll
            for (int m = 0; m < PCA_MT; ++m)
#pragma unroll
                for (int r = 0; r < 4; ++r) {
                    const long cell = cell0 + m * 16 + 4 * kq + r;
                    if (cell < n) {
                        if constexpr (SPLIT) out[((size_t)blockIdx.y * n + cell) * C + comp] = tot[t][m][r];
                        else out[cell * C + comp] = tot[t][m][r] - mp;
                    }
                }
        }
    }
}

__global__ void pca_split_sum_kernel(const float* __restrict__ part, const float* __restrict__ mean_proj, int C, float* __restrict__ out, long n)
{
    const long i = (long)blockIdx.x * blockDim.x + threadIdx.x;
    if (i >= n * C) return;
    float v = 0.0f;
#pragma unroll
    for (int j = 0; j < DET_RANGES; ++j) v += part[(size_t)j * n * C + i];
    out[i] = v - mean_proj[i % C];
}

typedef double f64x4 __attribute__((ext_vector_type(4)));
constexpr int SVMM_WAVES = 8, SVMM_TILES = 2, SVMM_CELLS = SVMM_WAVES * SVMM_TILES * 16;

struct SvmArgs {
    const double* svT[2];
    const double* svn[2];
    const double* coef[2];
    int nsv_pad[2];
    double gamma[2], rho[2];
};

template <int KS, bool SPLIT>
__global__ __launch_bounds__(64 * SVMM_WAVES, 1) void ocsvm_mfma_kernel(
    const float* __restrict__ pca, int D, SvmArgs sa, double* __restrict__ dec , long n)
{
    const int det = (int)blockIdx.z;
    const double* __restrict__ svT = sa.svT[det];
    const double* __restrict__ svn = sa.svn[det];
    const double* __restrict__ coef = sa.coef[det];
    const int nsv_pad = sa.nsv_pad[det];
    const double gamma = sa.gamma[det], rho = sa.rho[det];
    constexpr int ROWS = 4 * KS + 2;
    __shared__ double sb[2][ROWS][16];
    const int tid = threadIdx.x, lane = tid & 63, wave = tid >> 6;
    const int li = lane & 15, kq = lane >> 4;
    const long cell0 = (long)blockIdx.x * SVMM_CELLS + wave * (SVMM_TILES * 16);

    double xa[SVMM_TILES][KS];
    double rown[SVMM_TILES][4];
#pragma unroll
    for (int t = 0; t < SVMM_TILES; ++t) {
        long cell = cell0 + t * 16 + li;
        if (cell >= n) cell = n - 1;
        double nx = 0.0;
#pragma unroll
        for (int s = 0; s < KS; ++s) {
            const int d = 4 * s + kq;
            const double v = d < D ? (double)pca[cell * D + d] : 0.0;
            xa[t][s] = v;
            nx = fma(v, v, nx);
        }
        nx += __shfl_xor(nx, 16);
        nx += __shfl_xor(nx, 32);
#pragma unroll
        for (int r = 0; r < 4; ++r) rown[t][r] = __shfl(nx, kq + 4 * r);
    }

    constexpr int NST = (ROWS * 16 + 64 * SVMM_WAVES - 1) / (64 * SVMM_WAVES);
    auto fetch = [&](int blk, double v[NST]) {
#pragma unroll
        for (int j = 0; j < NST; ++j) {
            const int e = tid + 64 * SVMM_WAVES * j, row = e >> 4, col = e & 15;
            const size_t sidx = (size_t)blk * 16 + col;
            double x = 0.0;
            if (row < D) x = svT[(size_t)row * nsv_pad + sidx];
            else if (row == 4 * KS) x = svn[sidx];
            else if (row == 4 * KS + 1) x = coef[sidx];
            v[j] = x;
        }
    };
    auto stash = [&](int buf, const double v[NST]) {
#pragma unroll
        for (int j = 0; j < NST; ++j) {
            const int e = tid + 64 * SVMM_WAVES * j;
            if (e < ROWS * 16) sb[buf][e >> 4][e & 15] = v[j];
        }
    };
    const int nblk = nsv_pad / 16;
    int rj = SPLIT ? (int)blockIdx.y : 0;
    const int bbeg = SPLIT ? nblk * rj / DET_RANGES : 0, bend = SPLIT ? nblk * (rj + 1) / DET_RANGES : nblk;
    if (bbeg < bend) {
        double v[NST];
        fetch(bbeg, v);
        stash(bbeg & 1, v);
    }
    __syncthreads();

    double sum[SVMM_TILES][4], tot[SVMM_TILES][4];
#pragma unroll
    for (int t = 0; t < SVMM_TILES; ++t)
#pragma unroll
        for (int r = 0; r < 4; ++r) sum[t][r] = tot[t][r] = 0.0;
    for (int blk = bbeg; blk < bend; ++blk) {
        const int cur = blk & 1;
        double nv[NST];
        if (blk + 1 < bend) fetch(blk + 1, nv);
        f64x4 acc[SVMM_TILES];
#pragma unroll
        for (int t = 0; t < SVMM_TILES; ++t) acc[t] = f64x4{0.0, 0.0, 0.0, 0.0};
#pragma unroll
        for (int s = 0; s < KS; ++s) {
            const double b = sb[cur][4 * s + kq][li];
#pragma unroll
            for (int t = 0; t < SVMM_TILES; ++t) acc[t] = __builtin_amdgcn_mfma_f64_16x16x4f64(xa[t][s], b, acc[t], 0, 0, 0);
        }
        const double sn = sb[cur][4 * KS][li], cf = sb[cur][4 * KS + 1][li];
#pragma unroll
        for (int t = 0; t < SVMM_TILES; ++t)
#pragma unroll
            for (int r = 0; r < 4; ++r) {
                const double d2 = fma(-2.0, acc[t][r], rown[t][r] + sn);
                sum[t][r] = fma(cf, exp(-gamma * d2), sum[t][r]);
            }
        if (blk + 1 < bend) stash(cur ^ 1, nv);
        __syncthreads();
        while (rj < DET_RANGES && nblk * (rj + 1) / DET_RANGES <= blk + 1) {
            if (nblk * (rj + 1) / DET_RANGES == blk + 1) {
#pragma unroll
                for (int t = 0; t < SVMM_TILES; ++t)
#pragma unroll
                    for (int r = 0; r < 4; ++r) {
                        double v = sum[t][r];
                        v += __shfl_xor(v, 1);
                        v += __shfl_xor(v, 2);
                        v += __shfl_xor(v, 4);
                        v += __shfl_xor(v, 8);
                        tot[t][r] += v;
                        sum[t][r] = 0.0;
                    }
            }
            ++rj;
            if (SPLIT) break;
        }
    }
#pragma unroll
    for (int t = 0; t < SVMM_TILES; ++t)
#pragma unroll
        for (int r = 0; r < 4; ++r) {
            const long cell = cell0 + t * 16 + kq + 4 * r;
            if (li == 0 && cell < n) {
                if constexpr (SPLIT) dec[((size_t)det * DET_RANGES + blockIdx.y) * n + cell] = tot[t][r];
                else dec[cell] = tot[t][r] - rho;
            }
        }
}

__global__ void svm_split_sum_kernel(const double* __restrict__ part, double rho0, double rho1, double* __restrict__ dec0,
                                     double* __restrict__ dec1, long n)
{
    const long i = (long)blockIdx.x * blockDim.x + threadIdx.x;
    const int det = (int)blockIdx.y;
    if (i >= n) return;
    double v = 0.0;
#pragma unroll
    for (int j = 0; j < DET_RANGES; ++j) v += part[((size_t)det * DET_RANGES + j) * n + i];
    if (det == 0) dec0[i] = v - rho0;
    else dec1[i] = v - rho1;
}


__global__ void finalize_kernel(const float* __restrict__ errpart, int nparts, int npix,
                                const double* __restrict__ dec_c, const double* __restrict__ dec_m,
                                float* __restrict__ mse, float* __restrict__ mae,
                                double* __restrict__ score_c, double* __restrict__ score_m,
                                int8_t* __restrict__ pred_c, int8_t* __restrict__ pred_m, long n)
{
    const long i = (long)blockIdx.x * blockDim.x + threadIdx.x;
    if (i >= n) return;
    bool bad = false;
    if (errpart) {
        float s2 = 0.0f, s1 = 0.0f;
        for (int p = 0; p < nparts; ++p) {
            s2 += errpart[(i * nparts + p) * 2 + 0];
            s1 += errpart[(i * nparts + p) * 2 + 1];
        }
        if (mse) mse[i] = s2 / (float)npix;
        if (mae) mae[i] = s1 / (float)npix;
        bad = !(fabsf(s2) <= 3.402823466e38f && fabsf(s1) <= 3.402823466e38f);
    }
    const double qnan = __longlong_as_double(0x7ff8000000000000LL);
    if (dec_c) {
        const double d = bad ? qnan : dec_c[i];
        if (score_c) score_c[i] = -d;
        if (pred_c) pred_c[i] = (d > 0) ? 1 : -1;
    }
    if (dec_m) {
        const double d = bad ? qnan : dec_m[i];
        if (score_m) score_m[i] = -d;
        if (pred_m) pred_m[i] = (d > 0) ? 1 : -1;
    }
}

__device__ __forceinline__ uint32_t hash24(uint64_t seed, uint64_t cell, uint32_t pix)
{
    uint64_t z = seed + cell * 0x9E3779B97F4A7C15ULL + (uint64_t)pix * 0xD1B54A32D192ED03ULL;
    z ^= z >> 30; z *= 0xBF58476D1CE4E5B9ULL;
    z ^= z >> 27; z *= 0x94D049BB133111EBULL;
    z ^= z >> 31;
    return (uint32_t)(z >> 40);
}

__global__ void synth_kernel(uint64_t seed, long first_cell, long n, int npix, float* __restrict__ out)
{
    const long total = n * npix;
    for (long i = (long)blockIdx.x * blockDim.x + threadIdx.x; i < total; i += (long)gridDim.x * blockDim.x) {
        const long c = i / npix;
        const int p = (int)(i % npix);
        out[i] = (float)hash24(seed, (uint64_t)(first_cell + c), (uint32_t)p) * (1.0f / 16777216.0f);
    }
}

}

hipError_t launch_scaler_pca(const float* feat, const float* center, const double* scale,
                             const float* comps_pad, const float* mean_proj, int F, int fpad, int C,
                             int cpad, float* pca_out, int64_t n_cells, hipStream_t stream)
{
    if (n_cells <= 0) return hipSuccess;
    if (cpad % 16 || cpad > 128 || fpad % PCA_KC) return hipErrorInvalidValue;
    const unsigned grid = (unsigned)((n_cells + PCA_CELLS - 1) / PCA_CELLS);
    KernelSetup ks;
    if (hipError_t e = kernel_setup<scaler_pca_kernel>(256, PCA_LDS, ks); e != hipSuccess) return e;
    hipLaunchKernelGGL(scaler_pca_kernel, dim3(grid), dim3(256), PCA_LDS, stream, feat, center, scale,
                       comps_pad, mean_proj, F, fpad, C, cpad, pca_out, (long)n_cells);
    return hipGetLastError();
}

size_t pack_pca_bf16x3(const float* comps_pad, int cpad, int fpad, uint16_t* dst)
{
    const size_t n = (size_t)cpad * fpad * 3;
    if (!dst) return n;
    auto rne = [](float x) -> uint16_t {
        uint32_t u;
        memcpy(&u, &x, 4);
        if ((u & 0x7fffffffu) > 0x7f800000u) return (uint16_t)((u >> 16) | 0x40);
        u += 0x7fffu + ((u >> 16) & 1u);
        return (uint16_t)(u >> 16);
    };
    auto val = [](uint16_t h) -> float {
        const uint32_t u = (uint32_t)h << 16;
        float x;
        memcpy(&x, &u, 4);
        return x;
    };
    const int nkb = fpad / 32;
    for (int c = 0; c < cpad; ++c)
        for (int f = 0; f < fpad; ++f) {
            const float v = comps_pad[(size_t)c * fpad + f];
            const uint16_t w1 = rne(v);
            const float r1 = v - val(w1);
            const uint16_t w2 = rne(r1);
            const float r2 = r1 - val(w2);
            const uint16_t pl[3] = {w1, w2, rne(r2)};
            const int tile = c >> 4, li = c & 15, kb = f >> 5, kq = (f >> 3) & 3, j = f & 7;
            for (int p = 0; p < 3; ++p) dst[((((size_t)tile * nkb + kb) * 3 + p) * 64 + kq * 16 + li) * 8 + j] = pl[p];
        }
    return n;
}

size_t det_split_ws_bytes(int C)
{
    const size_t pca = (size_t)DET_RANGES * DET_SPLIT_MAX_CELLS * (size_t)C * sizeof(float);
    const size_t svm = (size_t)2 * DET_RANGES * DET_SPLIT_MAX_CELLS * sizeof(double);
    return pca > svm ? pca : svm;
}

hipError_t launch_scaler_pca_x3(const float* feat, const float* center, const double* scale, const uint16_t* comps_planes,
                                const float* mean_proj, int F, int fpad, int C, int cpad, float* pca_out, int64_t n_cells,
                                hipStream_t stream, void* split_ws)
{
    if (n_cells <= 0) return hipSuccess;
    if (cpad % 16 || cpad > 128 || fpad % PX_KC) return hipErrorInvalidValue;
    const unsigned grid = (unsigned)((n_cells + PCA_CELLS - 1) / PCA_CELLS);
    const bool split = split_ws && n_cells <= DET_SPLIT_MAX_CELLS;
    KernelSetup ks;
    const hipError_t e = !split ? kernel_setup<scaler_pca_x3_kernel<false>>(256, PX_LDS, ks)
                                : kernel_setup<scaler_pca_x3_kernel<true>>(256, PX_LDS, ks);
    if (e != hipSuccess) return e;
    if (split) {
        hipLaunchKernelGGL(scaler_pca_x3_kernel<true>, dim3(grid, DET_RANGES), dim3(256), PX_LDS, stream, feat, center, scale,
                           (const bf16x8*)comps_planes, mean_proj, F, fpad, C, cpad, (float*)split_ws, (long)n_cells);
        const long tot = (long)n_cells * C;
        hipLaunchKernelGGL(pca_split_sum_kernel, dim3((unsigned)((tot + 255) / 256)), dim3(256), 0, stream, (const float*)split_ws, mean_proj,
                           C, pca_out, (long)n_cells);
        return hipGetLastError();
    }
    hipLaunchKernelGGL(scaler_pca_x3_kernel<false>, dim3(grid), dim3(256), PX_LDS, stream, feat, center, scale, (const bf16x8*)comps_planes,
                       mean_proj, F, fpad, C, cpad, pca_out, (long)n_cells);
    return hipGetLastError();
}

template <bool SPLIT>
static void ocsvm_launch(const float* pca, int D, const SvmArgs& sa, double* out, int64_t n_cells, dim3 grid, hipStream_t stream)
{
    if (D <= 100)
        hipLaunchKernelGGL((ocsvm_mfma_kernel<25, SPLIT>), grid, dim3(64 * SVMM_WAVES), 0, stream, pca, D, sa, out, (long)n_cells);
    else
        hipLaunchKernelGGL((ocsvm_mfma_kernel<32, SPLIT>), grid, dim3(64 * SVMM_WAVES), 0, stream, pca, D, sa, out, (long)n_cells);
}

hipError_t launch_ocsvm(const float* pca, int D, const double* svT, const double* svn, const double* coef, int nsv_pad, double gamma,
                        double rho, double* dec, int64_t n_cells, hipStream_t stream, void* split_ws)
{
    if (n_cells <= 0) return hipSuccess;
    if (!svT || !svn || !coef || D < 1 || D > 128 || nsv_pad % 16) return hipErrorInvalidValue;
    const unsigned grid = (unsigned)((n_cells + SVMM_CELLS - 1) / SVMM_CELLS);
    SvmArgs sa{{svT, svT}, {svn, svn}, {coef, coef}, {nsv_pad, nsv_pad}, {gamma, gamma}, {rho, rho}};
    if (split_ws && n_cells <= DET_SPLIT_MAX_CELLS) {
        ocsvm_launch<true>(pca, D, sa, (double*)split_ws, n_cells, dim3(grid, DET_RANGES, 1), stream);
        hipLaunchKernelGGL(svm_split_sum_kernel, dim3((unsigned)((n_cells + 255) / 256), 1), dim3(256), 0, stream, (const double*)split_ws, rho, rho,
                           dec, dec, (long)n_cells);
        return hipGetLastError();
    }
    ocsvm_launch<false>(pca, D, sa, dec, n_cells, dim3(grid), stream);
    return hipGetLastError();
}

hipError_t launch_ocsvm_pair_split(const float* pca, int D, const double* const svT[2], const double* const svn[2],
                                   const double* const coef[2], const int nsv_pad[2], const double gamma[2], const double rho[2],
                                   double* dec0, double* dec1, int64_t n_cells, hipStream_t stream, void* split_ws)
{
    if (n_cells <= 0) return hipSuccess;
    if (!split_ws || n_cells > DET_SPLIT_MAX_CELLS || D < 1 || D > 128 || nsv_pad[0] % 16 || nsv_pad[1] % 16) return hipErrorInvalidValue;
    const unsigned grid = (unsigned)((n_cells + SVMM_CELLS - 1) / SVMM_CELLS);
    SvmArgs sa{{svT[0], svT[1]}, {svn[0], svn[1]}, {coef[0], coef[1]}, {nsv_pad[0], nsv_pad[1]}, {gamma[0], gamma[1]}, {rho[0], rho[1]}};
    ocsvm_launch<true>(pca, D, sa, (double*)split_ws, n_cells, dim3(grid, DET_RANGES, 2), stream);
    hipLaunchKernelGGL(svm_split_sum_kernel, dim3((unsigned)((n_cells + 255) / 256), 2), dim3(256), 0, stream, (const double*)split_ws, rho[0], rho[1],
                       dec0, dec1, (long)n_cells);
    return hipGetLastError();
}

hipError_t launch_finalize(const float* errpart, int nparts, int npix, const double* dec_c,
                           const double* dec_m, float* mse, float* mae, double* score_c,
                           double* score_m, int8_t* pred_c, int8_t* pred_m, int64_t n_cells,
                           hipStream_t stream)
{
    if (n_cells <= 0) return hipSuccess;
    const unsigned grid = (unsigned)((n_cells + 255) / 256);
    hipLaunchKernelGGL(finalize_kernel, dim3(grid), dim3(256), 0, stream, errpart, nparts, npix, dec_c,
                       dec_m, mse, mae, score_c, score_m, pred_c, pred_m, (long)n_cells);
    return hipGetLastError();
}

hipError_t launch_synth(uint64_t seed, int64_t first_cell, int64_t n, int npix, float* out,
                        hipStream_t stream)
{
    if (n <= 0) return hipSuccess;
    const long total = (long)n * npix;
    long blocks = (total + 255) / 256;
    if (blocks > 256L * 32) blocks = 256L * 32;
    hipLaunchKernelGGL(synth_kernel, dim3((unsigned)blocks), dim3(256), 0, stream, seed, (long)first_cell,
                       (long)n, npix, out);
    return hipGetLastError();
}

}
```

### cell-image-analysis_amd/csrc/fit.hip

```cpp
#include "api_internal.hpp"

#include <hip/hip_runtime.h>

#include <algorithm>
#include <cmath>
#include <limits>

namespace cs {

typedef double f64x4 __attribute__((ext_vector_type(4)));

namespace {

__device__ __forceinline__ unsigned f2key(float v)
{
    unsigned u = __float_as_uint(v);
    if (u == 0x80000000u) u = 0u;
    return (u & 0x80000000u) ? ~u : (u | 0x80000000u);
}
__device__ __forceinline__ float key2f(unsigned k)
{
    return __uint_as_float((k & 0x80000000u) ? (k & 0x7FFFFFFFu) : ~k);
}

__global__ __launch_bounds__(256) void keys_transpose_kernel(const float* __restrict__ x, long n, int F, long ld,
                                                             unsigned* __restrict__ keysT, int* __restrict__ nan_count)
{
    __shared__ unsigned tile[32][33];
    const int tx = threadIdx.x & 31, ty = threadIdx.x >> 5;
    const long r0 = (long)blockIdx.x * 32;
    const int c0 = blockIdx.y * 32;
    int nans = 0;
#pragma unroll
    for (int k = 0; k < 4; ++k) {
        const long r = r0 + ty + 8 * k;
        const int c = c0 + tx;
        unsigned key = 0u;
        if (r < n && c < F) {
            const float v = x[r * F + c];
            nans += (__float_as_uint(v) & 0x7F800000u) == 0x7F800000u;
            key = f2key(v);
        }
        tile[ty + 8 * k][tx] = key;
    }
    __syncthreads();
#pragma unroll
    for (int k = 0; k < 4; ++k) {
        const int c = c0 + ty + 8 * k;
        const long r = r0 + tx;
        if (r < n && c < F) keysT[(size_t)c * ld + r] = tile[tx][ty + 8 * k];
    }
    if (nans) atomicAdd(nan_count, nans);
}

constexpr int SEL_THREADS = 1024, SEL_T = 6;
struct SelRanks { unsigned r[SEL_T]; };

__global__ __launch_bounds__(SEL_THREADS) void column_select_kernel(const unsigned* __restrict__ keysT, long n, long ld,
                                                                    SelRanks ranks, float* __restrict__ out )
{
    __shared__ unsigned hist[SEL_T][256];
    __shared__ unsigned s_prefix[SEL_T], s_rank[SEL_T];
    const int tid = threadIdx.x, lane = tid & 63, wave = tid >> 6;
    const unsigned* col = keysT + (size_t)blockIdx.x * ld;
    if (tid < SEL_T) { s_prefix[tid] = 0u; s_rank[tid] = ranks.r[tid]; }
    for (int pass = 0; pass < 4; ++pass) {
        const int shift = 24 - 8 * pass;
        for (int e = tid; e < SEL_T * 256; e += SEL_THREADS) (&hist[0][0])[e] = 0u;
        __syncthreads();
        unsigned pf[SEL_T];
#pragma unroll
        for (int t = 0; t < SEL_T; ++t) pf[t] = s_prefix[t];
        for (long e = tid; e < n; e += SEL_THREADS) {
            const unsigned key = col[e];
            const unsigned bin = (key >> shift) & 255u;
            if (pass == 0) {
                atomicAdd(&hist[0][bin], 1u);
            } else {
                const unsigned hi = key >> (shift + 8);
#pragma unroll
                for (int t = 0; t < SEL_T; ++t)
                    if (hi == pf[t]) atomicAdd(&hist[t][bin], 1u);
            }
        }
        __syncthreads();
        if (wave < SEL_T) {
            const unsigned* h = hist[pass == 0 ? 0 : wave];
            const unsigned c0 = h[4 * lane], c1 = h[4 * lane + 1], c2 = h[4 * lane + 2], c3 = h[4 * lane + 3];
            unsigned incl = c0 + c1 + c2 + c3;
#pragma unroll
            for (int o = 1; o < 64; o <<= 1) {
                const unsigned v = __shfl_up(incl, o);
                if (lane >= o) incl += v;
            }
            unsigned cum = incl - (c0 + c1 + c2 + c3);
            const unsigned rk = s_rank[wave];
            const unsigned cs_[4] = {c0, c1, c2, c3};
#pragma unroll
            for (int b = 0; b < 4; ++b) {
                if (rk >= cum && rk < cum + cs_[b]) {
                    s_prefix[wave] = (pf[wave] << 8) | (unsigned)(4 * lane + b);
                    s_rank[wave] = rk - cum;
                }
                cum += cs_[b];
            }
        }
        __syncthreads();
    }
    if (tid < SEL_T) out[(size_t)blockIdx.x * SEL_T + tid] = key2f(s_prefix[tid]);
}

__global__ __launch_bounds__(256) void scale_kernel(const float* __restrict__ x, const float* __restrict__ center,
                                                    const double* __restrict__ scale, long total, int F, float* __restrict__ xs)
{
    for (long e = (long)blockIdx.x * 256 + threadIdx.x; e < total; e += (long)gridDim.x * 256) {
        const int f = (int)(e % F);
        const float t = __fsub_rn(x[e], center[f]);
        xs[e] = (float)__ddiv_rn((double)t, scale[f]);
    }
}

__global__ __launch_bounds__(64) void column_mean_kernel(const float* __restrict__ xs, long n, int F, float* __restrict__ mean)
{
    const int f = blockIdx.x * 64 + threadIdx.x;
    if (f >= F) return;
    float s = 0.0f;
    long r = 0;
    for (; r + 8 <= n; r += 8) {
        float v[8];
#pragma unroll
        for (int k = 0; k < 8; ++k) v[k] = xs[(r + k) * F + f];
#pragma unroll
        for (int k = 0; k < 8; ++k) s = __fadd_rn(s, v[k]);
    }
    for (; r < n; ++r) s = __fadd_rn(s, xs[r * F + f]);
    mean[f] = __fdiv_rn(s, (float)n);
}

__global__ __launch_bounds__(256) void center_kernel(float* __restrict__ xs, const float* __restrict__ mean, long total, int F)
{
    for (long e = (long)blockIdx.x * 256 + threadIdx.x; e < total; e += (long)gridDim.x * 256)
        xs[e] = __fsub_rn(xs[e], mean[(int)(e % F)]);
}

constexpr int COV_T = 128;
__global__ __launch_bounds__(256) void scatter_kernel(const float* __restrict__ xc, long n, int F, int ksplit,
                                                      double* __restrict__ part )
{
    const int T = F / COV_T;
    int t = blockIdx.x, ta = 0;
    while (t >= T - ta) { t -= T - ta; ++ta; }
    const int tb = ta + t;
    const int ks = blockIdx.y;
    const int lane = threadIdx.x & 63, wave = threadIdx.x >> 6;
    const int li = lane & 15, kq = lane >> 4;
    const int a0 = ta * COV_T + (wave >> 1) * 64, b0 = tb * COV_T + (wave & 1) * 64;
    const long rows = (n + ksplit - 1) / ksplit;
    const long r0 = (long)ks * rows, r1 = n < r0 + rows ? n : r0 + rows;

    f64x4 acc[4][4];
#pragma unroll
    for (int i = 0; i < 4; ++i)
#pragma unroll
        for (int j = 0; j < 4; ++j) acc[i][j] = f64x4{0.0, 0.0, 0.0, 0.0};

    auto load = [&](long r, float a[4], float b[4]) {
        const long row = r + kq;
        const bool ok = row < r1;
        const float* p = xc + (ok ? row : r0) * F;
#pragma unroll
        for (int i = 0; i < 4; ++i) {
            const float va = p[a0 + 16 * i + li], vb = p[b0 + 16 * i + li];
            a[i] = ok ? va : 0.0f;
            b[i] = ok ? vb : 0.0f;
        }
    };
    if (r0 < r1) {
        float a[4], b[4], na[4], nb[4];
        load(r0, a, b);
        for (long r = r0; r < r1; r += 4) {
            const long rn = r + 4 < r1 ? r + 4 : r0;
            load(rn, na, nb);
#pragma unroll
            for (int i = 0; i < 4; ++i)
#pragma unroll
                for (int j = 0; j < 4; ++j)
                    acc[i][j] = __builtin_amdgcn_mfma_f64_16x16x4f64((double)a[i], (double)b[j], acc[i][j], 0, 0, 0);
#pragma unroll
            for (int i = 0; i < 4; ++i) { a[i] = na[i]; b[i] = nb[i]; }
        }
    }
    double* o = part + (size_t)ks * F * F;
#pragma unroll
    for (int i = 0; i < 4; ++i)
#pragma unroll
        for (int j = 0; j < 4; ++j)
#pragma unroll
            for (int rg = 0; rg < 4; ++rg)
                o[(size_t)(a0 + 16 * i + kq + 4 * rg) * F + b0 + 16 * j + li] = acc[i][j][rg];
}

__global__ __launch_bounds__(256) void scatter_merge_kernel(const double* __restrict__ part, int F, int ksplit, double* __restrict__ out)
{
    const long total = (long)F * F;
    for (long e = (long)blockIdx.x * 256 + threadIdx.x; e < total; e += (long)gridDim.x * 256) {
        int a = (int)(e / F), b = (int)(e % F);
        if (b / COV_T < a / COV_T) { const int t = a; a = b; b = t; }
        double s = 0.0;
        for (int k = 0; k < ksplit; ++k) s += part[(size_t)k * total + (size_t)a * F + b];
        out[e] = s;
    }
}

constexpr int SMO_DP = 128;
constexpr int SMO_B = 256;
constexpr double SMO_TAU = 1e-12;
constexpr double SMO_INF = std::numeric_limits<double>::infinity();

struct SmoPickI { double v; int i; int pad; };
struct SmoPickJ { double obj; double g2; int j; int pad; };
struct SmoState {
    int done;
    int final_parity;
    int i;
    int pad;
    double gmax;
    long long n_iter;
};
struct SmoArgs {
    const void* xT;
    const double* xsq;
    long ld;
    int n, D, nb, pad;
    double gamma, eps;
    long long max_iter;
    double* alpha[2];
    double* G[2];
    float* Qi;
    SmoPickI* part_i;
    SmoPickJ* part_j;
    SmoState* state;
};

template <class XT>
__global__ __launch_bounds__(256) void smo_prepare_kernel(const double* __restrict__ x, int n, int D, long ld,
                                                          XT* __restrict__ xT, double* __restrict__ xsq)
{
    const int j = blockIdx.x * 256 + threadIdx.x;
    if (j >= n) return;
    double s = 0.0;
    for (int d = 0; d < D; ++d) {
        const double v = x[(size_t)j * D + d];
        xT[(size_t)d * ld + j] = (XT)v;
        s = fma(v, v, s);
    }
    xsq[j] = s;
}

__device__ __forceinline__ float rbf_q(double gamma, double xsqi, double xsqj, double dot)
{
    return (float)exp(__dmul_rn(-gamma, __dsub_rn(__dadd_rn(xsqi, xsqj), __dmul_rn(2.0, dot))));
}

__device__ __forceinline__ bool later_max(double v, int i, double bv, int bi) { return v > bv || (v == bv && i > bi); }
__device__ __forceinline__ bool later_min(double v, int i, double bv, int bi) { return v < bv || (v == bv && i > bi); }

__device__ __forceinline__ SmoPickI reduce_pick_i(SmoPickI p, SmoPickI* sh )
{
#pragma unroll
    for (int o = 32; o >= 1; o >>= 1) {
        const double v = __shfl_xor(p.v, o);
        const int i = __shfl_xor(p.i, o);
        if (later_max(v, i, p.v, p.i)) { p.v = v; p.i = i; }
    }
    const int lane = threadIdx.x & 63, wave = threadIdx.x >> 6;
    __syncthreads();
    if (lane == 0) sh[wave] = p;
    __syncthreads();
    p = sh[0];
#pragma unroll
    for (int w = 1; w < SMO_B / 64; ++w)
        if (later_max(sh[w].v, sh[w].i, p.v, p.i)) p = sh[w];
    return p;
}

__device__ __forceinline__ SmoPickJ reduce_pick_j(SmoPickJ p, SmoPickJ* sh )
{
#pragma unroll
    for (int o = 32; o >= 1; o >>= 1) {
        const double v = __shfl_xor(p.obj, o), g = __shfl_xor(p.g2, o);
        const int j = __shfl_xor(p.j, o);
        if (later_min(v, j, p.obj, p.j)) { p.obj = v; p.j = j; }
        p.g2 = fmax(p.g2, g);
    }
    const int lane = threadIdx.x & 63, wave = threadIdx.x >> 6;
    __syncthreads();
    if (lane == 0) sh[wave] = p;
    __syncthreads();
    p = sh[0];
#pragma unroll
    for (int w = 1; w < SMO_B / 64; ++w) {
        if (later_min(sh[w].obj, sh[w].j, p.obj, p.j)) { p.obj = sh[w].obj; p.j = sh[w].j; }
        p.g2 = fmax(p.g2, sh[w].g2);
// ... 11 lines not shown
    __shared__ SmoPickI shp[SMO_B / 64];
    const int tid = threadIdx.x;
    const int j = blockIdx.x * SMO_B + tid;
    const int jj = j < a.n ? j : a.n - 1;
    double xj[SMO_DP];
#pragma unroll
    for (int d = 0; d < SMO_DP; ++d) xj[d] = d < a.D ? (double)xT[(size_t)d * a.ld + jj] : 0.0;
    const double xsqj = a.xsq[jj];
    const double* alpha = a.alpha[0];
    double g = 0.0;
    for (int i0 = 0; i0 < n0; i0 += INIT_ROWS) {
        __syncthreads();
        for (int e = tid; e < INIT_ROWS * SMO_DP; e += SMO_B) {
            const int r = e / SMO_DP, d = e % SMO_DP, i = i0 + r;
            xi[r][d] = (i < n0 && d < a.D) ? (double)xT[(size_t)d * a.ld + i] : 0.0;
        }
        if (tid < INIT_ROWS) {
            const int i = i0 + tid;
            xsqi[tid] = i < n0 ? a.xsq[i] : 0.0;
            ali[tid] = i < n0 ? alpha[i] : 0.0;
        }
        __syncthreads();
        const int nr = min(INIT_ROWS, n0 - i0);
        for (int r = 0; r < nr; ++r) {
            double dot = 0.0;
#pragma unroll
            for (int d = 0; d < SMO_DP; ++d) dot = fma(xj[d], xi[r][d], dot);
            const float q = rbf_q(a.gamma, xsqi[r], xsqj, dot);
            g = __dadd_rn(g, __dmul_rn(ali[r], (double)q));
        }
    }
    SmoPickI p{-SMO_INF, -1, 0};
    if (j < a.n) {
        a.G[0][j] = g;
        if (alpha[j] < 1.0) { p.v = -g; p.i = j; }
    }
    p = reduce_pick_i(p, shp);
    if (tid == 0) a.part_i[blockIdx.x] = p;
}

template <class XT>
__global__ __launch_bounds__(SMO_B) void smo_row_i_kernel(SmoArgs a, int parity)
{
    const XT* __restrict__ xT = (const XT*)a.xT;
    __shared__ double xs[SMO_DP];
    __shared__ SmoPickI shi[SMO_B / 64];
    __shared__ SmoPickJ shj[SMO_B / 64];
    const int tid = threadIdx.x;
    if (a.state->done) return;
    if (a.max_iter >= 0 && a.state->n_iter >= a.max_iter) {
        if (blockIdx.x == 0 && tid == 0) { a.state->done = 2; a.state->final_parity = parity; }
        return;
    }
    const double* alpha = a.alpha[parity];
    const double* G = a.G[parity];
    SmoPickI pi{-SMO_INF, -1, 0};
    for (int b = tid; b < a.nb; b += SMO_B) {
        const SmoPickI q = a.part_i[b];
        if (later_max(q.v, q.i, pi.v, pi.i)) pi = q;
    }
    pi = reduce_pick_i(pi, shi);
    const int i = pi.i;
    const double gmax = pi.v;
    if (i < 0) {
        if (blockIdx.x == 0 && tid == 0) { a.state->i = -1; a.state->gmax = gmax; }
        if (tid == 0) a.part_j[blockIdx.x] = SmoPickJ{SMO_INF, -SMO_INF, -1, 0};
        return;
    }
    if (tid < a.D) xs[tid] = (double)xT[(size_t)tid * a.ld + i];
    __syncthreads();
    const double xsqi = a.xsq[i];
    const int j = blockIdx.x * SMO_B + tid;
    SmoPickJ pj{SMO_INF, -SMO_INF, -1, 0};
    if (j < a.n) {
        double dot = 0.0;
        for (int d = 0; d < a.D; ++d) dot = fma((double)xT[(size_t)d * a.ld + j], xs[d], dot);
        const float q = rbf_q(a.gamma, xsqi, a.xsq[j], dot);
        a.Qi[j] = q;
        if (alpha[j] > 0.0) {
            const double gj = G[j];
            pj.g2 = gj;
            const double gd = __dadd_rn(gmax, gj);
            if (gd > 0.0) {
                const double quad = __dsub_rn(2.0, __dmul_rn(2.0, (double)q));
                const double num = __dmul_rn(gd, gd);
                pj.obj = -__ddiv_rn(num, quad > 0.0 ? quad : SMO_TAU);
                pj.j = j;
            }
        }
    }
    pj = reduce_pick_j(pj, shj);
    if (tid == 0) a.part_j[blockIdx.x] = pj;
    if (blockIdx.x == 0 && tid == 0) { a.state->i = i; a.state->gmax = gmax; }
}

template <class XT>
__global__ __launch_bounds__(SMO_B) void smo_update_kernel(SmoArgs a, int parity)
{
    const XT* __restrict__ xT = (const XT*)a.xT;
    __shared__ double xs[SMO_DP];
    __shared__ SmoPickI shi[SMO_B / 64];
    __shared__ SmoPickJ shj[SMO_B / 64];
    const int tid = threadIdx.x;
    if (a.state->done) return;
    const double* alpha = a.alpha[parity];
    const double* G = a.G[parity];
    SmoPickJ pj{SMO_INF, -SMO_INF, -1, 0};
    for (int b = tid; b < a.nb; b += SMO_B) {
        const SmoPickJ q = a.part_j[b];
        if (later_min(q.obj, q.j, pj.obj, pj.j)) { pj.obj = q.obj; pj.j = q.j; }
        pj.g2 = fmax(pj.g2, q.g2);
    }
    pj = reduce_pick_j(pj, shj);
    const int i = a.state->i, j = pj.j;
    const double gmax = a.state->gmax;
    if (i < 0 || j < 0 || __dadd_rn(gmax, pj.g2) < a.eps) {
        if (blockIdx.x == 0 && tid == 0) { a.state->done = 1; a.state->final_parity = parity; }
        return;
    }
    double ai = alpha[i], aj = alpha[j];
    const double old_ai = ai, old_aj = aj;
    {
        const double qij = (double)a.Qi[j];
        double quad = __dsub_rn(2.0, __dmul_rn(2.0, qij));
        if (quad <= 0.0) quad = SMO_TAU;
        const double delta = __ddiv_rn(__dsub_rn(G[i], G[j]), quad);
        const double sum = __dadd_rn(ai, aj);
        ai = __dsub_rn(ai, delta);
        aj = __dadd_rn(aj, delta);
        if (sum > 1.0) {
            if (ai > 1.0) { ai = 1.0; aj = __dsub_rn(sum, 1.0); }
        } else {
            if (aj < 0.0) { aj = 0.0; ai = sum; }
        }
        if (sum > 1.0) {
            if (aj > 1.0) { aj = 1.0; ai = __dsub_rn(sum, 1.0); }
        } else {
            if (ai < 0.0) { ai = 0.0; aj = sum; }
        }
    }
    const double dai = __dsub_rn(ai, old_ai), daj = __dsub_rn(aj, old_aj);
    if (tid < a.D) xs[tid] = (double)xT[(size_t)tid * a.ld + j];
    __syncthreads();
    const double xsqj = a.xsq[j];
    const int k = blockIdx.x * SMO_B + tid;
    SmoPickI pi{-SMO_INF, -1, 0};
    if (k < a.n) {
        double dot = 0.0;
        for (int d = 0; d < a.D; ++d) dot = fma((double)xT[(size_t)d * a.ld + k], xs[d], dot);
        const float qj = rbf_q(a.gamma, xsqj, a.xsq[k], dot);
        const double gn = __dadd_rn(G[k], __dadd_rn(__dmul_rn((double)a.Qi[k], dai), __dmul_rn((double)qj, daj)));
        const double an = k == i ? ai : (k == j ? aj : alpha[k]);
        a.G[parity ^ 1][k] = gn;
        a.alpha[parity ^ 1][k] = an;
        if (an < 1.0) { pi.v = -gn; pi.i = k; }
    }
    pi = reduce_pick_i(pi, shi);
    if (tid == 0) a.part_i[blockIdx.x] = pi;
    if (blockIdx.x == 0 && tid == 0) a.state->n_iter += 1;
}

constexpr int SUB_TILE = 128;
template <class TA>
__global__ __launch_bounds__(256) void atb_kernel(const TA* __restrict__ A, long lda, int ma, const double* __restrict__ B, int ldb,
                                                  long K, long rows_per_slice, double* __restrict__ part)
{
    const int lane = threadIdx.x & 63, wave = threadIdx.x >> 6;
    const int li = lane & 15, kq = lane >> 4;
    const int i0 = blockIdx.x * SUB_TILE + (wave >> 1) * 64, j0 = blockIdx.y * SUB_TILE + (wave & 1) * 64;
    const long r0 = (long)blockIdx.z * rows_per_slice, r1 = K < r0 + rows_per_slice ? K : r0 + rows_per_slice;
    bool iok[4];
#pragma unroll
    for (int i = 0; i < 4; ++i) iok[i] = i0 + 16 * i + li < ma;

    f64x4 acc[4][4];
#pragma unroll
    for (int i = 0; i < 4; ++i)
#pragma unroll
        for (int j = 0; j < 4; ++j) acc[i][j] = f64x4{0.0, 0.0, 0.0, 0.0};

    auto load = [&](long r, double a[4], double b[4]) {
        const long row = r + kq;
        const bool ok = row < r1;
        const TA* pa = A + (ok ? row : r0) * lda;
        const double* pb = B + (ok ? row : r0) * (long)ldb;
#pragma unroll
        for (int i = 0; i < 4; ++i) {
            a[i] = (ok && iok[i]) ? (double)pa[i0 + 16 * i + li] : 0.0;
            const double vb = pb[j0 + 16 * i + li];
            b[i] = ok ? vb : 0.0;
        }
    };
    if (r0 < r1) {
        double a[4], b[4], na[4], nb[4];
        load(r0, a, b);
        for (long r = r0; r < r1; r += 4) {
            const long rn = r + 4 < r1 ? r + 4 : r0;
            load(rn, na, nb);
#pragma unroll
            for (int i = 0; i < 4; ++i)
#pragma unroll
                for (int j = 0; j < 4; ++j) acc[i][j] = __builtin_amdgcn_mfma_f64_16x16x4f64(a[i], b[j], acc[i][j], 0, 0, 0);
#pragma unroll
            for (int i = 0; i < 4; ++i) { a[i] = na[i]; b[i] = nb[i]; }
        }
    }
    const int ldc = SUB_TILE * gridDim.y;
    double* o = part + (size_t)blockIdx.z * ma * ldc;
#pragma unroll
    for (int i = 0; i < 4; ++i)
#pragma unroll
        for (int rg = 0; rg < 4; ++rg) {
            const int row = i0 + 16 * i + kq + 4 * rg;
            if (row < ma)
#pragma unroll
                for (int j = 0; j < 4; ++j) o[(size_t)row * ldc + j0 + 16 * j + li] = acc[i][j][rg];
        }
}

__global__ __launch_bounds__(256) void subspace_merge_kernel(const double* __restrict__ part, long total, int slices, double* __restrict__ out)
{
    for (long e = (long)blockIdx.x * 256 + threadIdx.x; e < total; e += (long)gridDim.x * 256) {
        double s = 0.0;
        for (int k = 0; k < slices; ++k) s += part[(size_t)k * total + e];
        out[e] = s;
    }
}

__global__ __launch_bounds__(256) void transpose_kernel(const float* __restrict__ x, long n, int F, float* __restrict__ xT)
{
    __shared__ float tile[32][33];
    const int tx = threadIdx.x & 31, ty = threadIdx.x >> 5;
    const long r0 = (long)blockIdx.x * 32;
    const int c0 = blockIdx.y * 32;
#pragma unroll
    for (int k = 0; k < 4; ++k) {
        const long r = r0 + ty + 8 * k;
        const int c = c0 + tx;
        tile[ty + 8 * k][tx] = (r < n && c < F) ? x[r * F + c] : 0.0f;
    }
    __syncthreads();
#pragma unroll
    for (int k = 0; k < 4; ++k) {
        const int c = c0 + ty + 8 * k;
        const long r = r0 + tx;
        if (r < n && c < F) xT[(size_t)c * n + r] = tile[tx][ty + 8 * k];
    }
}

__global__ __launch_bounds__(64) void column_sumsq_kernel(const float* __restrict__ xc, long n, int F, double* __restrict__ out)
{
    const int f = blockIdx.x * 64 + threadIdx.x;
    if (f >= F) return;
    double s = 0.0;
    for (long r = 0; r < n; ++r) {
        const double v = (double)xc[r * F + f];
        s = fma(v, v, s);
    }
    out[f] = s;
}

__device__ __forceinline__ unsigned long long splitmix64(unsigned long long z)
{
    z += 0x9E3779B97F4A7C15ull;
    z = (z ^ (z >> 30)) * 0xBF58476D1CE4E5B9ull;
    z = (z ^ (z >> 27)) * 0x94D049BB133111EBull;
    return z ^ (z >> 31);
}
__device__ __forceinline__ double gauss(unsigned long long seed, unsigned salt, long row, int col)
{
    const unsigned long long h = splitmix64(seed ^ splitmix64(((unsigned long long)salt << 40) ^ ((unsigned long long)row << 12) ^ (unsigned)col));
    const unsigned long long h2 = splitmix64(h);
    const double u1 = ((double)(h >> 11) + 1.0) * 0x1.0p-53;
    const double u2 = (double)(h2 >> 11) * 0x1.0p-53;
    return sqrt(-2.0 * log(u1)) * cos(6.283185307179586 * u2);
}

__global__ __launch_bounds__(256) void small_mm_kernel(const double* __restrict__ z, long rows, int Lp, const double* __restrict__ t,
                                                       const int* __restrict__ fresh, unsigned long long seed, unsigned salt,
                                                       double rscale, double* __restrict__ out)
{
    const int per = 256 / Lp;
    const int j = threadIdx.x % Lp;
    const long r = (long)blockIdx.x * per + threadIdx.x / Lp;
    if (r >= rows) return;
    double s = 0.0;
    if (z) {
        const double* zr = z + (size_t)r * Lp;
        for (int i = 0; i < Lp; ++i) s = fma(zr[i], t[(size_t)i * Lp + j], s);
    }
    if (fresh[j]) s += gauss(seed, salt, r, j) * rscale;
    out[(size_t)r * Lp + j] = s;
}

}
}

using namespace cs;

struct cs_fit {
    int device = 0;
    hipStream_t stream = nullptr;
    hipEvent_t ev0 = nullptr, ev1 = nullptr;
    DevBuf feat, keys, sel, nanc, cen, scl, xs, mean, part, scat, comps, mproj, proj;
    DevBuf x, xT, xsq, alpha0, alpha1, G0, G1, Qi, part_i, part_j, state;
    DevBuf sxT, sY, sQ, sZ, sgram, st, sfresh, ssq;
    double last_ms = 0.0;
};

int cs_fit_create(int device_id, cs_fit** out)
{
    if (!out) return fail(CS_ERR_INVALID, "out is NULL");
    *out = nullptr;
    int rc = require_gfx950(device_id);
    if (rc) return rc;
    cs_fit* f = new cs_fit();
    f->device = device_id;
    hipError_t e = hipStreamCreateWithFlags(&f->stream, hipStreamNonBlocking);
    if (e == hipSuccess) e = hipEventCreate(&f->ev0);
    if (e == hipSuccess) e = hipEventCreate(&f->ev1);
    if (e != hipSuccess) {
        delete f;
        return fail(CS_ERR_HIP, "stream/event creation failed: %s", hipGetErrorString(e));
    }
    *out = f;
    return CS_OK;
}

int cs_fit_wait_stream(cs_fit* f, void* hip_stream)
{
    if (!f) return fail(CS_ERR_INVALID, "fit handle is NULL");
    HIPCHK(hipSetDevice(f->device));
    return wait_on_stream(f->stream, hip_stream);
}

void cs_fit_free(cs_fit* f)
{
    if (!f) return;
    (void)hipSetDevice(f->device);
    if (f->ev0) (void)hipEventDestroy(f->ev0);
    if (f->ev1) (void)hipEventDestroy(f->ev1);
    if (f->stream) (void)hipStreamDestroy(f->stream);
    delete f;
}

int cs_fit_last_ms(const cs_fit* f, double* device_ms)
{
    if (!f || !device_ms) return fail(CS_ERR_INVALID, "NULL argument");
    *device_ms = f->last_ms;
    return CS_OK;
}

namespace {

struct Timer {
    cs_fit* f;
    explicit Timer(cs_fit* f_) : f(f_) { (void)hipEventRecord(f->ev0, f->stream); }
    int stop()
    {
        HIPCHK(hipEventRecord(f->ev1, f->stream));
        HIPCHK(hipStreamSynchronize(f->stream));
        float ms = 0.f;
        HIPCHK(hipEventElapsedTime(&ms, f->ev0, f->ev1));
        f->last_ms = ms;
        return CS_OK;
    }
};

int stage_features(cs_fit* f, const float* features, int64_t n, int F, int kind, const float** dev)
{
    if (kind == CS_MEM_DEVICE) { *dev = features; return CS_OK; }
    const size_t bytes = (size_t)n * F * sizeof(float);
    int rc = f->feat.ensure(bytes);
    if (rc) return rc;
    HIPCHK(hipMemcpyAsync(f->feat.p, features, bytes, hipMemcpyHostToDevice, f->stream));
    *dev = f->feat.as<float>();
    return CS_OK;
}

int check_features(const cs_fit* f, const float* features, int64_t n, int F, int kind)
{
    if (!f) return fail(CS_ERR_INVALID, "handle is NULL");
    if (!features) return fail(CS_ERR_INVALID, "features is NULL");
    if (kind != CS_MEM_HOST && kind != CS_MEM_DEVICE) return fail(CS_ERR_INVALID, "memory kind must be CS_MEM_HOST or CS_MEM_DEVICE");
    if (n < 1 || n > (1ll << 30)) return fail(CS_ERR_INVALID, "n=%lld: need 1 .. 2^30 training cells", (long long)n);
    if (F < 1 || F > (1 << 20)) return fail(CS_ERR_INVALID, "n_features=%d out of range (1 .. 2^20)", F);
    return CS_OK;
}

struct QuantilePos { int64_t lo, hi; double gamma; };
QuantilePos quantile_pos(int64_t n, double q)
{
    const double vi = (double)(n - 1) * q;
    QuantilePos p;
    const double fl = std::floor(vi);
    p.gamma = vi - fl;
    p.lo = (int64_t)fl;
    p.hi = p.lo + 1;
    if (vi >= (double)(n - 1)) { p.lo = p.hi = n - 1; }
    if (vi < 0) { p.lo = p.hi = 0; }
    return p;
}
double lerp_f32(float a, float b, double t)
{
    const float diff = b - a;
    volatile double prod = (double)diff * t;
    double r = (double)a + prod;
    if (t >= 0.5) {
        volatile double prod2 = (double)diff * (1.0 - t);
        r = (double)b - prod2;
    }
    return r;
}

}

int cs_fit_scaler(cs_fit* f, const float* features, int64_t n, int32_t n_features, int kind, float* center, double* scale)
{
    int rc = check_features(f, features, n, n_features, kind);
    if (rc) return rc;
    if (!center || !scale) return fail(CS_ERR_INVALID, "NULL output");
    HIPCHK(hipSetDevice(f->device));
    const int F = n_features;
    const float* d_feat;
    if ((rc = stage_features(f, features, n, F, kind, &d_feat))) return rc;
    const long ld = (long)((n + 63) / 64 * 64);
    if ((rc = f->keys.ensure((size_t)F * ld * sizeof(unsigned)))) return rc;
    if ((rc = f->sel.ensure((size_t)F * SEL_T * sizeof(float)))) return rc;
    if ((rc = f->nanc.ensure(sizeof(int)))) return rc;

    const QuantilePos q25 = quantile_pos(n, 0.25), q75 = quantile_pos(n, 0.75);
    SelRanks rk;
    rk.r[0] = (unsigned)((n - 1) / 2); rk.r[1] = (unsigned)(n / 2);
    rk.r[2] = (unsigned)q25.lo; rk.r[3] = (unsigned)q25.hi;
    rk.r[4] = (unsigned)q75.lo; rk.r[5] = (unsigned)q75.hi;

    Timer tm(f);
    HIPCHK(hipMemsetAsync(f->nanc.p, 0, sizeof(int), f->stream));
    hipLaunchKernelGGL(keys_transpose_kernel, dim3((unsigned)((n + 31) / 32), (unsigned)((F + 31) / 32)), dim3(256), 0, f->stream,
                       d_feat, (long)n, F, ld, f->keys.as<unsigned>(), f->nanc.as<int>());
    HIPCHK(hipGetLastError());
    hipLaunchKernelGGL(column_select_kernel, dim3((unsigned)F), dim3(SEL_THREADS), 0, f->stream, f->keys.as<unsigned>(), (long)n, ld,
                       rk, f->sel.as<float>());
    HIPCHK(hipGetLastError());
    std::vector<float> sel((size_t)F * SEL_T);
    int nans = 0;
    HIPCHK(hipMemcpyAsync(sel.data(), f->sel.p, sel.size() * sizeof(float), hipMemcpyDeviceToHost, f->stream));
    HIPCHK(hipMemcpyAsync(&nans, f->nanc.p, sizeof(int), hipMemcpyDeviceToHost, f->stream));
    if ((rc = tm.stop())) return rc;
    if (nans)
        return fail(CS_ERR_UNSUPPORTED, "features hold %d non-finite values (NaN or +-inf): nanmedian / nanpercentile semantics are not "
                    "implemented, and scikit-learn refuses infinities", nans);

    for (int c = 0; c < F; ++c) {
        const float* s = &sel[(size_t)c * SEL_T];
        if (n & 1) center[c] = s[0];
        else { volatile float sum = s[0] + s[1]; center[c] = sum / 2.0f; }
        const double lo = lerp_f32(s[2], s[3], q25.gamma), hi = lerp_f32(s[4], s[5], q75.gamma);
        double sc = hi - lo;
        if (sc < 10.0 * std::numeric_limits<double>::epsilon()) sc = 1.0;
        scale[c] = sc;
    }
    return CS_OK;
}

int cs_fit_pca_moments(cs_fit* f, const float* features, int64_t n, int32_t n_features, int kind, const float* center,
                       const double* scale, float* mean, double* scatter)
{
    int rc = check_features(f, features, n, n_features, kind);
    if (rc) return rc;
    if (!center || !scale || !mean || !scatter) return fail(CS_ERR_INVALID, "NULL argument");
    const int F = n_features;
    if (F % COV_T || F > 8192)
        return fail(CS_ERR_UNSUPPORTED, "n_features=%d: the moment kernel needs a multiple of %d up to 8192", F, COV_T);
    HIPCHK(hipSetDevice(f->device));
    const float* d_feat;
    if ((rc = stage_features(f, features, n, F, kind, &d_feat))) return rc;
    const int T = F / COV_T, tiles = T * (T + 1) / 2;
    int ksplit = std::max(1, std::min(16, (int)(2048 / tiles)));
    ksplit = (int)std::min<int64_t>(ksplit, (n + 3) / 4);
    const size_t FF = (size_t)F * F;
    if ((rc = f->cen.ensure(sizeof(float) * F)) || (rc = f->scl.ensure(sizeof(double) * F)) || (rc = f->mean.ensure(sizeof(float) * F)) ||
        (rc = f->xs.ensure((size_t)n * F * sizeof(float))) || (rc = f->part.ensure(FF * ksplit * sizeof(double))) ||
        (rc = f->scat.ensure(FF * sizeof(double))))
        return rc;
    HIPCHK(hipMemcpyAsync(f->cen.p, center, sizeof(float) * F, hipMemcpyHostToDevice, f->stream));
    HIPCHK(hipMemcpyAsync(f->scl.p, scale, sizeof(double) * F, hipMemcpyHostToDevice, f->stream));
    Timer tm(f);
    const long total = (long)n * F;
    const unsigned eg = (unsigned)std::min<long>((total + 255) / 256, 256L * 64);
    hipLaunchKernelGGL(scale_kernel, dim3(eg), dim3(256), 0, f->stream, d_feat, f->cen.as<float>(), f->scl.as<double>(), total, F,
                       f->xs.as<float>());
    HIPCHK(hipGetLastError());
    hipLaunchKernelGGL(column_mean_kernel, dim3((unsigned)((F + 63) / 64)), dim3(64), 0, f->stream, f->xs.as<float>(), (long)n, F,
                       f->mean.as<float>());
    HIPCHK(hipGetLastError());
    hipLaunchKernelGGL(center_kernel, dim3(eg), dim3(256), 0, f->stream, f->xs.as<float>(), f->mean.as<float>(), total, F);
    HIPCHK(hipGetLastError());
    hipLaunchKernelGGL(scatter_kernel, dim3((unsigned)tiles, (unsigned)ksplit), dim3(256), 0, f->stream, f->xs.as<float>(), (long)n, F,
                       ksplit, f->part.as<double>());
    HIPCHK(hipGetLastError());
    hipLaunchKernelGGL(scatter_merge_kernel, dim3((unsigned)std::min<size_t>((FF + 255) / 256, 256 * 64)), dim3(256), 0, f->stream,
                       f->part.as<double>(), F, ksplit, f->scat.as<double>());
    HIPCHK(hipGetLastError());
    HIPCHK(hipMemcpyAsync(mean, f->mean.p, sizeof(float) * F, hipMemcpyDeviceToHost, f->stream));
    HIPCHK(hipMemcpyAsync(scatter, f->scat.p, FF * sizeof(double), hipMemcpyDeviceToHost, f->stream));
    return tm.stop();
}

int cs_fit_project(cs_fit* f, const float* features, int64_t n, int32_t n_features, int kind, const float* center,
                   const double* scale, const float* components, const float* mean_proj, int32_t n_components, float* out)
{
    int rc = check_features(f, features, n, n_features, kind);
    if (rc) return rc;
    if (!center || !scale || !components || !mean_proj || !out) return fail(CS_ERR_INVALID, "NULL argument");
    if (n_components < 1 || n_components > 128) return fail(CS_ERR_INVALID, "n_components=%d (1..128)", n_components);
    HIPCHK(hipSetDevice(f->device));
    const int F = n_features, C = n_components;
    const float* d_feat;
    if ((rc = stage_features(f, features, n, F, kind, &d_feat))) return rc;
    const int fpad = (F + 511) / 512 * 512, cpad = (C + 15) / 16 * 16;
    std::vector<float> cp((size_t)cpad * fpad, 0.0f);
    for (int c = 0; c < C; ++c) memcpy(&cp[(size_t)c * fpad], components + (size_t)c * F, sizeof(float) * F);
    if ((rc = f->cen.ensure(sizeof(float) * F)) || (rc = f->scl.ensure(sizeof(double) * F)) ||
        (rc = f->comps.ensure(cp.size() * sizeof(float))) || (rc = f->mproj.ensure(sizeof(float) * C)) ||
        (rc = f->proj.ensure((size_t)n * C * sizeof(float))))
        return rc;
    HIPCHK(hipMemcpyAsync(f->cen.p, center, sizeof(float) * F, hipMemcpyHostToDevice, f->stream));
    HIPCHK(hipMemcpyAsync(f->scl.p, scale, sizeof(double) * F, hipMemcpyHostToDevice, f->stream));
    HIPCHK(hipMemcpyAsync(f->comps.p, cp.data(), cp.size() * sizeof(float), hipMemcpyHostToDevice, f->stream));
    HIPCHK(hipMemcpyAsync(f->mproj.p, mean_proj, sizeof(float) * C, hipMemcpyHostToDevice, f->stream));
    Timer tm(f);
    HIPCHK(launch_scaler_pca(d_feat, f->cen.as<float>(), f->scl.as<double>(), f->comps.as<float>(), f->mproj.as<float>(), F, fpad, C,
                             cpad, f->proj.as<float>(), n, f->stream));
    HIPCHK(hipMemcpyAsync(out, f->proj.p, (size_t)n * C * sizeof(float), hipMemcpyDeviceToHost, f->stream));
    return tm.stop();
}

int cs_fit_ocsvm(cs_fit* f, const double* x, int64_t n, int32_t n_components, double gamma, double nu, double eps,
                 int64_t max_iter, double* alpha, double* rho, double* obj, int64_t* n_iter, int32_t* status)
{
    if (!f) return fail(CS_ERR_INVALID, "handle is NULL");
    if (!x || !alpha || !rho) return fail(CS_ERR_INVALID, "NULL argument");
    if (n < 1 || n > (1 << 28)) return fail(CS_ERR_INVALID, "n=%lld: need 1 .. 2^28 training points", (long long)n);
    const int D = n_components;
    if (D < 1 || D > SMO_DP) return fail(CS_ERR_INVALID, "n_components=%d (1..%d)", D, SMO_DP);
    if (!(nu > 0.0 && nu <= 1.0)) return fail(CS_ERR_INVALID, "nu=%g: need 0 < nu <= 1 (libsvm's check)", nu);
    if (!(gamma >= 0.0) || !(eps > 0.0)) return fail(CS_ERR_INVALID, "gamma=%g / eps=%g", gamma, eps);
    HIPCHK(hipSetDevice(f->device));
    const int N = (int)n;
    const long ld = (long)((n + 63) / 64 * 64);
    const int nb = (N + SMO_B - 1) / SMO_B;
    int rc;
    if ((rc = f->x.ensure((size_t)n * D * 8)) || (rc = f->xT.ensure((size_t)D * ld * 8)) || (rc = f->xsq.ensure((size_t)n * 8)) ||
        (rc = f->alpha0.ensure((size_t)n * 8)) || (rc = f->alpha1.ensure((size_t)n * 8)) || (rc = f->G0.ensure((size_t)n * 8)) ||
        (rc = f->G1.ensure((size_t)n * 8)) || (rc = f->Qi.ensure((size_t)n * 4)) || (rc = f->part_i.ensure((size_t)nb * sizeof(SmoPickI))) ||
        (rc = f->part_j.ensure((size_t)nb * sizeof(SmoPickJ))) || (rc = f->state.ensure(sizeof(SmoState))))
        return rc;

    bool as_float = true;
    for (size_t e = 0, ne = (size_t)n * D; e < ne; ++e) {
        if (!std::isfinite(x[e])) return fail(CS_ERR_INVALID, "x holds a non-finite value at element %zu (sklearn's check_array rejects it)", e);
        as_float = as_float && (double)(float)x[e] == x[e];
    }

    std::vector<double> a0((size_t)n, 0.0);
    int n0 = 0;
    {
        double nu_l = 0.0;
        for (int64_t i = 0; i < n; ++i) { volatile double t = 1.0 * nu; nu_l += t; }
        int64_t i = 0;
        while (nu_l > 0 && i < n) {
            a0[(size_t)i] = std::min(1.0, nu_l);
            nu_l -= a0[(size_t)i];
            ++i;
        }
        n0 = (int)i;
    }
    HIPCHK(hipMemcpyAsync(f->x.p, x, (size_t)n * D * 8, hipMemcpyHostToDevice, f->stream));
    HIPCHK(hipMemcpyAsync(f->alpha0.p, a0.data(), (size_t)n * 8, hipMemcpyHostToDevice, f->stream));
    HIPCHK(hipMemsetAsync(f->state.p, 0, sizeof(SmoState), f->stream));
    Timer tm(f);
    SmoArgs a{};
    a.xT = f->xT.p; a.xsq = f->xsq.as<double>(); a.ld = ld; a.n = N; a.D = D; a.nb = nb;
    a.gamma = gamma; a.eps = eps; a.max_iter = max_iter;
    a.alpha[0] = f->alpha0.as<double>(); a.alpha[1] = f->alpha1.as<double>();
    a.G[0] = f->G0.as<double>(); a.G[1] = f->G1.as<double>();
    a.Qi = f->Qi.as<float>(); a.part_i = f->part_i.as<SmoPickI>(); a.part_j = f->part_j.as<SmoPickJ>();
    a.state = f->state.as<SmoState>();
    if (as_float) {
        hipLaunchKernelGGL(smo_prepare_kernel<float>, dim3((unsigned)nb), dim3(256), 0, f->stream, f->x.as<double>(), N, D, ld,
                           f->xT.as<float>(), f->xsq.as<double>());
        hipLaunchKernelGGL(smo_init_kernel<float>, dim3((unsigned)nb), dim3(SMO_B), 0, f->stream, a, n0);
    } else {
        hipLaunchKernelGGL(smo_prepare_kernel<double>, dim3((unsigned)nb), dim3(256), 0, f->stream, f->x.as<double>(), N, D, ld,
                           f->xT.as<double>(), f->xsq.as<double>());
        hipLaunchKernelGGL(smo_init_kernel<double>, dim3((unsigned)nb), dim3(SMO_B), 0, f->stream, a, n0);
    }
    HIPCHK(hipGetLastError());

    const long long hard_cap = 200ll * 1000 * 1000;
    const int batch = 256;
    SmoState st{};
    long long issued = 0;
    int parity = 0;
    while (true) {
        for (int it = 0; it < batch; ++it) {
            if (as_float) {
                hipLaunchKernelGGL(smo_row_i_kernel<float>, dim3((unsigned)nb), dim3(SMO_B), 0, f->stream, a, parity);
                hipLaunchKernelGGL(smo_update_kernel<float>, dim3((unsigned)nb), dim3(SMO_B), 0, f->stream, a, parity);
            } else {
                hipLaunchKernelGGL(smo_row_i_kernel<double>, dim3((unsigned)nb), dim3(SMO_B), 0, f->stream, a, parity);
                hipLaunchKernelGGL(smo_update_kernel<double>, dim3((unsigned)nb), dim3(SMO_B), 0, f->stream, a, parity);
            }
            parity ^= 1;
        }
        HIPCHK(hipGetLastError());
        issued += batch;
        HIPCHK(hipMemcpyAsync(&st, f->state.p, sizeof(SmoState), hipMemcpyDeviceToHost, f->stream));
        HIPCHK(hipStreamSynchronize(f->stream));
        if (st.done) break;
        if (issued >= hard_cap) return fail(CS_ERR_UNSUPPORTED, "SMO did not converge within %lld iterations", hard_cap);
    }
    std::vector<double> G((size_t)n);
    HIPCHK(hipMemcpyAsync(alpha, a.alpha[st.final_parity], (size_t)n * 8, hipMemcpyDeviceToHost, f->stream));
    HIPCHK(hipMemcpyAsync(G.data(), a.G[st.final_parity], (size_t)n * 8, hipMemcpyDeviceToHost, f->stream));
    if ((rc = tm.stop())) return rc;

    {
        int64_t nr_free = 0;
        double ub = SMO_INF, lb = -SMO_INF, sum_free = 0.0;
        for (int64_t i = 0; i < n; ++i) {
            const double yG = G[(size_t)i];
            if (alpha[i] >= 1.0) lb = std::max(lb, yG);
            else if (alpha[i] <= 0.0) ub = std::min(ub, yG);
            else { ++nr_free; sum_free += yG; }
        }
        const double r = nr_free > 0 ? sum_free / (double)nr_free : (ub + lb) / 2;
        if (!std::isfinite(r))
            return fail(CS_ERR_INVALID, "rho is not finite (nu=%g leaves every alpha at a bound): scikit-learn refuses this fit", nu);
        *rho = r;
        if (obj) {
            double v = 0.0;
            for (int64_t i = 0; i < n; ++i) { volatile double t = alpha[i] * (G[(size_t)i] + 0.0); v += t; }
            *obj = v / 2;
        }
    }
    if (n_iter) *n_iter = st.n_iter;
    if (status) *status = st.done == 2 ? 1 : 0;
    return CS_OK;
}

namespace {

constexpr int SUB_MAX_ITER = 100;
constexpr double SUB_RTOL = 1e-5;
constexpr double SUB_ATOL = 1e-12;
constexpr double CHOL_REL = 1e-12;
constexpr double CHOL_ABS = 1e-24;

int sym_eig(int n, const double* a, double* w, double* vout, bool vectors)
{
    std::vector<double> V(a, a + (size_t)n * n), d(n), e(n);
    auto A = [&](int i, int j) -> double& { return V[(size_t)i * n + j]; };
    for (int j = 0; j < n; ++j) d[j] = A(n - 1, j);
    for (int i = n - 1; i > 0; --i) {
        double scale = 0.0, h = 0.0;
        for (int k = 0; k < i; ++k) scale += std::fabs(d[k]);
        if (scale == 0.0) {
            e[i] = d[i - 1];
            for (int j = 0; j < i; ++j) { d[j] = A(i - 1, j); A(i, j) = 0.0; A(j, i) = 0.0; }
        } else {
            for (int k = 0; k < i; ++k) { d[k] /= scale; h += d[k] * d[k]; }
            double f = d[i - 1], g = std::sqrt(h);
            if (f > 0) g = -g;
            e[i] = scale * g;
            h -= f * g;
            d[i - 1] = f - g;
            for (int j = 0; j < i; ++j) e[j] = 0.0;
            for (int j = 0; j < i; ++j) {
                f = d[j];
                A(j, i) = f;
                g = e[j] + A(j, j) * f;
                for (int k = j + 1; k <= i - 1; ++k) { g += A(k, j) * d[k]; e[k] += A(k, j) * f; }
                e[j] = g;
            }
            f = 0.0;
            for (int j = 0; j < i; ++j) { e[j] /= h; f += e[j] * d[j]; }
            const double hh = f / (h + h);
            for (int j = 0; j < i; ++j) e[j] -= hh * d[j];
            for (int j = 0; j < i; ++j) {
                f = d[j]; g = e[j];
                for (int k = j; k <= i - 1; ++k) A(k, j) -= (f * e[k] + g * d[k]);
                d[j] = A(i - 1, j);
                A(i, j) = 0.0;
            }
        }
        d[i] = h;
    }
    if (vectors) {
        for (int i = 0; i < n - 1; ++i) {
            A(n - 1, i) = A(i, i);
            A(i, i) = 1.0;
            const double h = d[i + 1];
            if (h != 0.0) {
                for (int k = 0; k <= i; ++k) d[k] = A(k, i + 1) / h;
                for (int j = 0; j <= i; ++j) {
                    double g = 0.0;
                    for (int k = 0; k <= i; ++k) g += A(k, i + 1) * A(k, j);
                    for (int k = 0; k <= i; ++k) A(k, j) -= g * d[k];
                }
            }
            for (int k = 0; k <= i; ++k) A(k, i + 1) = 0.0;
        }
        for (int j = 0; j < n; ++j) { d[j] = A(n - 1, j); A(n - 1, j) = 0.0; }
        A(n - 1, n - 1) = 1.0;
    } else {
        for (int j = 0; j < n; ++j) d[j] = A(j, j);
    }
    e[0] = 0.0;
    for (int i = 1; i < n; ++i) e[i - 1] = e[i];
    e[n - 1] = 0.0;
    double f = 0.0, tst1 = 0.0;
    const double eps = std::ldexp(1.0, -52);
    for (int l = 0; l < n; ++l) {
        tst1 = std::max(tst1, std::fabs(d[l]) + std::fabs(e[l]));
        int m = l;
        while (m < n - 1 && std::fabs(e[m]) > eps * tst1) ++m;
        if (m > l) {
            int iter = 0;
            do {
                if (++iter > 64) return fail(CS_ERR_UNSUPPORTED, "tridiagonal QL did not converge");
                double g = d[l];
                double p = (d[l + 1] - g) / (2.0 * e[l]);
                double r = std::hypot(p, 1.0);
                if (p < 0) r = -r;
                d[l] = e[l] / (p + r);
                d[l + 1] = e[l] * (p + r);
                const double dl1 = d[l + 1];
                double h = g - d[l];
                for (int i = l + 2; i < n; ++i) d[i] -= h;
                f += h;
                p = d[m];
                double c = 1.0, c2 = c, c3 = c, s = 0.0, s2 = 0.0;
                const double el1 = e[l + 1];
                for (int i = m - 1; i >= l; --i) {
                    c3 = c2; c2 = c; s2 = s;
                    g = c * e[i]; h = c * p;
                    r = std::hypot(p, e[i]);
                    e[i + 1] = s * r;
                    s = e[i] / r; c = p / r;
                    p = c * d[i] - s * g;
                    d[i + 1] = h + s * (c * g + s * d[i]);
                    if (vectors)
                        for (int k = 0; k < n; ++k) {
                            h = A(k, i + 1);
                            A(k, i + 1) = s * A(k, i) + c * h;
                            A(k, i) = c * A(k, i) - s * h;
                        }
                }
                p = -s * s2 * c3 * el1 * e[l] / dl1;
                e[l] = s * p;
                d[l] = c * p;
            } while (std::fabs(e[l]) > eps * tst1);
        }
        d[l] += f;
        e[l] = 0.0;
    }
    std::vector<int> idx(n);
    for (int i = 0; i < n; ++i) idx[i] = i;
    std::stable_sort(idx.begin(), idx.end(), [&](int x, int y) { return d[x] < d[y]; });
    for (int j = 0; j < n; ++j) {
        w[j] = d[idx[j]];
        if (vectors)
            for (int k = 0; k < n; ++k) vout[(size_t)k * n + j] = A(k, idx[j]);
    }
    return CS_OK;
}

int chol_inverse(const double* g, int L, int Lp, double* t, int* fresh)
{
    std::vector<double> R((size_t)L * L, 0.0);
    double gmax = 0.0;
    for (int j = 0; j < L; ++j) gmax = std::max(gmax, g[(size_t)j * Lp + j]);
    int nd = 0;
    for (int j = 0; j < L; ++j) {
        fresh[j] = 0;
        double d = g[(size_t)j * Lp + j];
        const double gjj = d;
        for (int i = 0; i < j; ++i) {
            if (fresh[i]) continue;
            double s = g[(size_t)i * Lp + j];
            for (int p = 0; p < i; ++p) s -= R[(size_t)p * L + i] * R[(size_t)p * L + j];
            R[(size_t)i * L + j] = s / R[(size_t)i * L + i];
            d -= R[(size_t)i * L + j] * R[(size_t)i * L + j];
        }
        if (!(gjj > CHOL_ABS * gmax) || !(d > CHOL_REL * gjj)) {
            fresh[j] = 1;
            ++nd;
            for (int i = 0; i < j; ++i) R[(size_t)i * L + j] = 0.0;
            R[(size_t)j * L + j] = 1.0;
        } else {
            R[(size_t)j * L + j] = std::sqrt(d);
        }
    }
    std::fill(t, t + (size_t)Lp * Lp, 0.0);
    for (int j = 0; j < L; ++j) {
        if (fresh[j]) continue;
        t[(size_t)j * Lp + j] = 1.0 / R[(size_t)j * L + j];
        for (int i = j - 1; i >= 0; --i) {
            double s = 0.0;
            for (int p = i + 1; p <= j; ++p) s += R[(size_t)i * L + p] * t[(size_t)p * Lp + j];
            t[(size_t)i * Lp + j] = -s / R[(size_t)i * L + i];
        }
    }
    for (int j = L; j < Lp; ++j) fresh[j] = 0;
    return nd;
}

long slice_rows(long tiles, long K)
{
    long ks = std::max(1L, std::min(64L, 2048 / std::max(1L, tiles)));
    ks = std::min(ks, std::max(1L, K / 256));
    return (K + ks - 1) / ks;
}

struct Sub {
    cs_fit* f;
    long n;
    int F, L, Lp;
    const float* xs;
    const float* xT;
    double *Y, *Q, *Z, *part, *gram, *t;
    int* fresh;

    template <class TA>
// ... 167 lines not shown
```

Before: 5.451 million cells/s.

## Merge OCSVM support vectors into one union set and use reciprocal scaler

The conservative and moderate OCSVM support-vector sets are deduplicated on the host into a single union matrix with two coefficient columns, so one kernel pass computes both decision functions and shared kernel evaluations happen once. The RobustScaler division is replaced by multiplying with a precomputed reciprocal, and a bit test on the result falls back to a true division only when the rounding could differ. This is meant to cut SVM kernel work and fp64 divides in the detector stage. It adds host-side hashing at load time and a rarely taken slow path in the scaler kernel.

```diff
diff --git a/cell-image-analysis_amd/build.py b/cell-image-analysis_amd/build.py
--- a/cell-image-analysis_amd/build.py
+++ b/cell-image-analysis_amd/build.py
@@ -9,7 +9,7 @@
 BUILD = os.path.join(HERE, "build")
 SOURCES = ["api.hip", "conv_mfma.hip", "conv_out.hip", "detector.hip", "train.hip", "train_api.hip", "train_generic.hip", "preprocess.hip",
            "conv_wino_cs.hip", "conv12_fused.hip", "conv45_h2.hip", "conv_generic.hip", "conv_generic_x3.hip", "conv_wino_up.hip", "fit.hip", "extract.hip", "segment.hip", "match.hip", "expand.hip", "intensity.hip", "quantile.hip", "texture.hip", "shape.hip", "neighbors.hip", "colocalize.hip", "radial.hip"]
-HEADERS = ["common.hpp", "split16.hpp", "kernel_setup.hpp", "api_internal.hpp", "train_internal.hpp", "segment_internal.hpp", "stage_host.hpp", "label_tile.hpp", "label_boxes.hpp", "hull_chain.hpp", "tensor_archive.hpp", os.path.join("..", "..", "include", "cellscreen.h")]
+HEADERS = ["common.hpp", "split16.hpp", "kernel_setup.hpp", "api_internal.hpp", "train_internal.hpp", "segment_internal.hpp", "stage_host.hpp", "label_tile.hpp", "label_boxes.hpp", "hull_chain.hpp", "tensor_archive.hpp", "scaled_feature.hpp", os.path.join("..", "..", "include", "cellscreen.h")]
 HIPCC = os.environ.get("HIPCC", "/opt/rocm/bin/hipcc")
 FLAGS = ["-O3", "--offload-arch=gfx950", "-fPIC", "-std=c++17", "-Wall", "-Wno-unused-function",
          "-fno-gpu-rdc"]
diff --git a/cell-image-analysis_amd/csrc/api.hip b/cell-image-analysis_amd/csrc/api.hip
--- a/cell-image-analysis_amd/csrc/api.hip
+++ b/cell-image-analysis_amd/csrc/api.hip
@@ -1,5 +1,8 @@
 #include "api_internal.hpp"
+#include "scaled_feature.hpp"
 #include "tensor_archive.hpp"
+
+#include <unordered_map>
 
 using namespace cs;
 
@@ -80,8 +83,9 @@
     DevBuf w7eff, b7;
     bool has_det = false;
     int F = 0, fpad = 0, C = 0, cpad = 0;
-    DevBuf center, scale, comps, comps_x3, mean_proj;
-    struct Svm { DevBuf svT, svn, coef; int nsv = 0, nsv_pad = 0; double gamma = 0, rho = 0; } svm[2];
+    DevBuf center, scale, rscale, comps, comps_x3, mean_proj;
+    struct Svm { int nsv = 0, nsv_pad = 0; double gamma = 0, rho = 0; } svm[2];
+    struct SvmUnion { DevBuf svT, svn, coef; int n = 0, n_pad = 0; } svu;
     int64_t chunk = 0;
     int64_t ws_cells = 0;
     DevBuf xin, xin2, act[CS_MAX_CONV], featE, pca, errpart, dec[2], o_mse, o_mae, o_sc[2], o_pr[2], recon;
@@ -352,32 +356,73 @@
     return true;
 }
 
-static int pack_svm(cs_model::Svm& s, const cs_ocsvm_params& p, int D, const char* what)
-{
-    if (p.n_sv <= 0 || !p.support_vectors || !p.dual_coef)
-        return fail(CS_ERR_INVALID, "%s detector: n_sv=%d or NULL arrays", what, p.n_sv);
-    s.nsv = p.n_sv;
-    s.nsv_pad = (p.n_sv + 15) / 16 * 16;
-    s.gamma = p.gamma;
-    s.rho = p.rho;
-    std::vector<double> svT((size_t)D * s.nsv_pad, 0.0), coef(s.nsv_pad, 0.0), svn(s.nsv_pad, 0.0);
-    for (int i = 0; i < p.n_sv; ++i) {
-        coef[i] = p.dual_coef[i];
+static int pack_svm_union(cs_model* m, const cs_ocsvm_params* const p[2], int D)
+{
+    static const char* const what[2] = {"conservative", "moderate"};
+    for (int k = 0; k < 2; ++k) {
+        if (p[k]->n_sv <= 0 || !p[k]->support_vectors || !p[k]->dual_coef)
+            return fail(CS_ERR_INVALID, "%s detector: n_sv=%d or NULL arrays", what[k], p[k]->n_sv);
+        m->svm[k].nsv = p[k]->n_sv;
+        m->svm[k].nsv_pad = (p[k]->n_sv + 15) / 16 * 16;
+        m->svm[k].gamma = p[k]->gamma;
+        m->svm[k].rho = p[k]->rho;
+    }
+    const size_t row = sizeof(double) * (size_t)D;
+    int a = 1;
+    if (p[0]->n_sv != p[1]->n_sv) a = p[0]->n_sv > p[1]->n_sv ? 0 : 1;
+    else {
+        int c = memcmp(p[0]->support_vectors, p[1]->support_vectors, row * p[0]->n_sv);
+        if (!c) c = memcmp(p[0]->dual_coef, p[1]->dual_coef, sizeof(double) * p[0]->n_sv);
+        a = c < 0 ? 0 : 1;
+    }
+    const int b = 1 - a, na = p[a]->n_sv, nb = p[b]->n_sv;
+    auto hash = [&](const double* r) {
+        uint64_t h = 0xcbf29ce484222325ULL;
+        const unsigned char* q = (const unsigned char*)r;
+        for (size_t i = 0; i < row; ++i) h = (h ^ q[i]) * 0x100000001b3ULL;
+        return h;
+    };
+    std::unordered_multimap<uint64_t, int> idx;
+    idx.reserve((size_t)na);
+    for (int i = 0; i < na; ++i) idx.emplace(hash(p[a]->support_vectors + (size_t)i * D), i);
+    std::vector<int> slot(nb, -1);
+    std::vector<char> taken(na, 0);
+    int nu = na;
+    for (int j = 0; j < nb; ++j) {
+        const double* r = p[b]->support_vectors + (size_t)j * D;
+        int best = -1;
+        auto range = idx.equal_range(hash(r));
+        for (auto it = range.first; it != range.second; ++it) {
+            const int i = it->second;
+            if (!taken[i] && (best < 0 || i < best) && !memcmp(p[a]->support_vectors + (size_t)i * D, r, row)) best = i;
+        }
+        if (best >= 0) { taken[best] = 1; slot[j] = best; }
+        else slot[j] = nu++;
+    }
+    cs_model::SvmUnion& u = m->svu;
+    u.n = nu;
+    u.n_pad = (nu + 15) / 16 * 16;
+    std::vector<double> svT((size_t)D * u.n_pad, 0.0), coef((size_t)2 * u.n_pad, 0.0), svn(u.n_pad, 0.0);
+    auto put = [&](int at, const double* r) {
         double nn = 0.0;
         for (int d = 0; d < D; ++d) {
-            const double v = p.support_vectors[(size_t)i * D + d];
-            svT[(size_t)d * s.nsv_pad + i] = v;
-            nn = fma(v, v, nn);
-        }
-        svn[i] = nn;
-    }
-    {
-        int rcn = upload(s.svn, svn.data(), svn.size() * sizeof(double));
-        if (rcn) return rcn;
-    }
-    int rc = upload(s.svT, svT.data(), svT.size() * sizeof(double));
+            svT[(size_t)d * u.n_pad + at] = r[d];
+            nn = fma(r[d], r[d], nn);
+        }
+        svn[at] = nn;
+    };
+    for (int i = 0; i < na; ++i) {
+        put(i, p[a]->support_vectors + (size_t)i * D);
+        coef[(size_t)a * u.n_pad + i] = p[a]->dual_coef[i];
+    }
+    for (int j = 0; j < nb; ++j) {
+        if (slot[j] >= na) put(slot[j], p[b]->support_vectors + (size_t)j * D);
+        coef[(size_t)b * u.n_pad + slot[j]] = p[b]->dual_coef[j];
+    }
+    int rc = upload(u.svn, svn.data(), svn.size() * sizeof(double));
     if (rc) return rc;
-    return upload(s.coef, coef.data(), coef.size() * sizeof(double));
+    if ((rc = upload(u.svT, svT.data(), svT.size() * sizeof(double)))) return rc;
+    return upload(u.coef, coef.data(), coef.size() * sizeof(double));
 }
 
 static int64_t eff_chunk(const cs_model* m, int in_kind)
@@ -747,6 +792,11 @@
         m->cpad = (m->C + 15) / 16 * 16;
         FAIL_IF(upload(m->center, det->scaler_center, sizeof(float) * m->F));
         FAIL_IF(upload(m->scale, det->scaler_scale, sizeof(double) * m->F));
+        {
+            std::vector<double> rs(m->F);
+            for (int f = 0; f < m->F; ++f) rs[f] = scaler_reciprocal(det->scaler_scale[f]);
+            FAIL_IF(upload(m->rscale, rs.data(), sizeof(double) * m->F));
+        }
         std::vector<float> cp((size_t)m->cpad * m->fpad, 0.0f);
         for (int c = 0; c < m->C; ++c)
             memcpy(&cp[(size_t)c * m->fpad], det->pca_components + (size_t)c * m->F, sizeof(float) * m->F);
@@ -757,8 +807,10 @@
             FAIL_IF(upload(m->comps_x3, pl.data(), pl.size() * sizeof(uint16_t)));
         }
         FAIL_IF(upload(m->mean_proj, det->pca_mean_proj, sizeof(float) * m->C));
-        FAIL_IF(pack_svm(m->svm[0], det->conservative, m->C, "conservative"));
-        FAIL_IF(pack_svm(m->svm[1], det->moderate, m->C, "moderate"));
+        {
+            const cs_ocsvm_params* const both[2] = {&det->conservative, &det->moderate};
+            FAIL_IF(pack_svm_union(m, both, m->C));
+        }
         m->has_det = true;
     }
 #undef FAIL_IF
@@ -905,26 +957,18 @@
 {
     if (m->split16)
         LAUNCH(K_SCALER_PCA, nc,
-               launch_scaler_pca_x3(feat, m->center.as<float>(), m->scale.as<double>(), m->comps_x3.as<uint16_t>(),
+               launch_scaler_pca_x3(feat, m->center.as<float>(), m->scale.as<double>(), m->rscale.as<double>(), m->comps_x3.as<uint16_t>(),
                                     m->mean_proj.as<float>(), m->F, m->fpad, m->C, m->cpad, m->pca.as<float>(), nc, m->stream, m->det_ws.p));
     else
         LAUNCH(K_SCALER_PCA, nc,
-               launch_scaler_pca(feat, m->center.as<float>(), m->scale.as<double>(), m->comps.as<float>(),
+               launch_scaler_pca(feat, m->center.as<float>(), m->scale.as<double>(), m->rscale.as<double>(), m->comps.as<float>(),
                                  m->mean_proj.as<float>(), m->F, m->fpad, m->C, m->cpad, m->pca.as<float>(), nc, m->stream));
-    if (m->det_ws.p && nc <= DET_SPLIT_MAX_CELLS) {
-        const double* svT[2] = {m->svm[0].svT.as<double>(), m->svm[1].svT.as<double>()};
-        const double* svn[2] = {m->svm[0].svn.as<double>(), m->svm[1].svn.as<double>()};
-        const double* coef[2] = {m->svm[0].coef.as<double>(), m->svm[1].coef.as<double>()};
-        const int nsv[2] = {m->svm[0].nsv_pad, m->svm[1].nsv_pad};
+    {
         const double gam[2] = {m->svm[0].gamma, m->svm[1].gamma}, rho[2] = {m->svm[0].rho, m->svm[1].rho};
         LAUNCH(K_SVM, nc,
-               launch_ocsvm_pair_split(m->pca.as<float>(), m->C, svT, svn, coef, nsv, gam, rho, m->dec[0].as<double>(), m->dec[1].as<double>(), nc,
-                                       m->stream, m->det_ws.p));
-    } else
-    for (int d = 0; d < 2; ++d)
-        LAUNCH(K_SVM, nc,
-               launch_ocsvm(m->pca.as<float>(), m->C, m->svm[d].svT.as<double>(), m->svm[d].svn.as<double>(), m->svm[d].coef.as<double>(),
-                            m->svm[d].nsv_pad, m->svm[d].gamma, m->svm[d].rho, m->dec[d].as<double>(), nc, m->stream, m->det_ws.p));
+               launch_ocsvm_pair(m->pca.as<float>(), m->C, m->svu.svT.as<double>(), m->svu.svn.as<double>(), m->svu.coef.as<double>(), m->svu.n_pad,
+                                 gam, rho, m->dec[0].as<double>(), m->dec[1].as<double>(), nc, m->stream, m->det_ws.p));
+    }
     LAUNCH(K_FINALIZE, nc,
            launch_finalize(with_err ? m->errpart.as<float>() : nullptr, m->errparts, (int)m->arch.npix, m->dec[0].as<double>(),
                            m->dec[1].as<double>(), mse, mae, sc, sm, pc, pm, nc, m->stream));
@@ -1141,11 +1185,11 @@
         if ((rc = stage_in(m, features, in_kind, off, nc, (size_t)m->F, m->featE, &f))) return rc;
         if (m->split16)
             LAUNCH(K_SCALER_PCA, nc,
-                   launch_scaler_pca_x3(f, m->center.as<float>(), m->scale.as<double>(), m->comps_x3.as<uint16_t>(),
+                   launch_scaler_pca_x3(f, m->center.as<float>(), m->scale.as<double>(), m->rscale.as<double>(), m->comps_x3.as<uint16_t>(),
                                         m->mean_proj.as<float>(), m->F, m->fpad, m->C, m->cpad, m->pca.as<float>(), nc, m->stream, m->det_ws.p));
         else
             LAUNCH(K_SCALER_PCA, nc,
-                   launch_scaler_pca(f, m->center.as<float>(), m->scale.as<double>(), m->comps.as<float>(),
+                   launch_scaler_pca(f, m->center.as<float>(), m->scale.as<double>(), m->rscale.as<double>(), m->comps.as<float>(),
                                      m->mean_proj.as<float>(), m->F, m->fpad, m->C, m->cpad, m->pca.as<float>(), nc, m->stream));
         HIPCHK(hipMemcpyAsync(pca_out + (size_t)off * m->C, m->pca.p, (size_t)nc * m->C * sizeof(float),
                               out_kind == CS_MEM_DEVICE ? hipMemcpyDeviceToDevice : hipMemcpyDeviceToHost, m->stream));
@@ -1172,11 +1216,15 @@
         const int64_t nc = (n - off) < ch ? (n - off) : ch;
         const float* p;
         if ((rc = stage_in(m, pca, in_kind, off, nc, (size_t)m->C, m->pca, &p))) return rc;
+        if (outs[0] || outs[1]) {
+            const double gam[2] = {m->svm[0].gamma, m->svm[1].gamma}, rho[2] = {m->svm[0].rho, m->svm[1].rho};
+            LAUNCH(K_SVM, nc,
+                   launch_ocsvm_pair(p, m->C, m->svu.svT.as<double>(), m->svu.svn.as<double>(), m->svu.coef.as<double>(), m->svu.n_pad, gam, rho,
+                                     outs[0] ? m->dec[0].as<double>() : nullptr, outs[1] ? m->dec[1].as<double>() : nullptr, nc, m->stream,
+                                     m->det_ws.p));
+        }
         for (int d = 0; d < 2; ++d) {
             if (!outs[d]) continue;
-            LAUNCH(K_SVM, nc,
-                   launch_ocsvm(p, m->C, m->svm[d].svT.as<double>(), m->svm[d].svn.as<double>(), m->svm[d].coef.as<double>(),
-                                m->svm[d].nsv_pad, m->svm[d].gamma, m->svm[d].rho, m->dec[d].as<double>(), nc, m->stream, m->det_ws.p));
             HIPCHK(hipMemcpyAsync(outs[d] + off, m->dec[d].p, (size_t)nc * sizeof(double),
                                   out_kind == CS_MEM_DEVICE ? hipMemcpyDeviceToDevice : hipMemcpyDeviceToHost, m->stream));
         }
diff --git a/cell-image-analysis_amd/csrc/common.hpp b/cell-image-analysis_amd/csrc/common.hpp
--- a/cell-image-analysis_amd/csrc/common.hpp
+++ b/cell-image-analysis_amd/csrc/common.hpp
@@ -125,24 +125,20 @@
 hipError_t launch_pack_ep(const float* bias, const float* gamma, const float* beta, const float* mov_mean,
                           const float* mov_var, float eps, int C, float* ep, hipStream_t s);
 
-hipError_t launch_scaler_pca(const float* feat, const float* center, const double* scale,
+hipError_t launch_scaler_pca(const float* feat, const float* center, const double* scale, const double* rscale,
                              const float* comps_pad, const float* mean_proj, int F, int fpad, int C,
                              int cpad, float* pca_out, int64_t n_cells, hipStream_t stream);
 
-hipError_t launch_scaler_pca_x3(const float* feat, const float* center, const double* scale, const uint16_t* comps_planes,
+hipError_t launch_scaler_pca_x3(const float* feat, const float* center, const double* scale, const double* rscale, const uint16_t* comps_planes,
                                 const float* mean_proj, int F, int fpad, int C, int cpad, float* pca_out, int64_t n_cells,
                                 hipStream_t stream, void* split_ws = nullptr);
 constexpr int64_t DET_SPLIT_MAX_CELLS = 16384;
 size_t det_split_ws_bytes(int C);
 size_t pack_pca_bf16x3(const float* comps_pad, int cpad, int fpad, uint16_t* dst);
 
-hipError_t launch_ocsvm(const float* pca, int D, const double* svT , const double* svn ,
-                        const double* coef, int nsv_pad, double gamma, double rho, double* dec, int64_t n_cells, hipStream_t stream,
-                        void* split_ws = nullptr);
-
-hipError_t launch_ocsvm_pair_split(const float* pca, int D, const double* const svT[2], const double* const svn[2],
-                                   const double* const coef[2], const int nsv_pad[2], const double gamma[2], const double rho[2],
-                                   double* dec0, double* dec1, int64_t n_cells, hipStream_t stream, void* split_ws);
+hipError_t launch_ocsvm_pair(const float* pca, int D, const double* svT, const double* svn, const double* coef2, int nu_pad,
+                             const double gamma[2], const double rho[2], double* dec0, double* dec1, int64_t n_cells, hipStream_t stream,
+                             void* split_ws = nullptr);
 
 hipError_t launch_finalize(const float* errpart, int nparts, int npix, const double* dec_c,
                            const double* dec_m, float* mse, float* mae, double* score_c,
diff --git a/cell-image-analysis_amd/csrc/detector.hip b/cell-image-analysis_amd/csrc/detector.hip
--- a/cell-image-analysis_amd/csrc/detector.hip
+++ b/cell-image-analysis_amd/csrc/detector.hip
@@ -1,5 +1,6 @@
 #include "common.hpp"
 #include "kernel_setup.hpp"
+#include "scaled_feature.hpp"
 
 #include <cstring>
 
@@ -13,10 +14,10 @@
 constexpr int PCA_LD = PCA_KC + 4;
 constexpr int PCA_LDS = PCA_CELLS * PCA_LD * 4;
 
-__global__ __launch_bounds__(256) void scaler_pca_kernel(
+__global__ __launch_bounds__(256, 2) void scaler_pca_kernel(
     const float* __restrict__ feat, const float* __restrict__ center, const double* __restrict__ scale,
-    const float* __restrict__ comps, const float* __restrict__ mean_proj, int F, int fpad, int C,
-    int cpad, float* __restrict__ out, long n)
+    const double* __restrict__ rscale , const float* __restrict__ comps,
+    const float* __restrict__ mean_proj, int F, int fpad, int C, int cpad, float* __restrict__ out, long n)
 {
     extern __shared__ __attribute__((aligned(16))) char smem[];
     float* xs = (float*)smem;
@@ -46,12 +47,22 @@
         const int gk = k0 + tid;
         const bool kok = gk < F;
         const float ctr = center[kok ? gk : 0];
-        const double scl = scale[kok ? gk : 0];
+        const double rsc = rscale[kok ? gk : 0];
+        bool redo = false;
 #pragma unroll
         for (int c = 0; c < PCA_CELLS; ++c) {
-            const float t = raw[c] - ctr;
-            const float v = (float)((double)t / scl);
+            bool dv;
+            const float v = scaled_feature_fast(raw[c] - ctr, rsc, dv);
+            redo |= dv;
             xs[c * PCA_LD + tid] = (kok && cell0 + c < n) ? v : 0.0f;
+        }
+        if (__builtin_expect(redo, 0)) {
+            const double scl = scale[kok ? gk : 0];
+            for (int c = 0; c < PCA_CELLS; ++c) {
+                const bool ok = kok && cell0 + c < n;
+                const float x = feat[(ok ? cell0 + c : n - 1) * F + (ok ? gk : F - 1)];
+                xs[c * PCA_LD + tid] = ok ? (float)((double)(x - ctr) / scl) : 0.0f;
+            }
         }
     };
     issue(0);
@@ -115,9 +126,9 @@
 constexpr int DET_RANGES = 8;
 
 template <bool SPLIT>
-__global__ __launch_bounds__(256) void scaler_pca_x3_kernel(
+__global__ __launch_bounds__(256, 2) void scaler_pca_x3_kernel(
     const float* __restrict__ feat, const float* __restrict__ center, const double* __restrict__ scale,
-    const bf16x8* __restrict__ comps , const float* __restrict__ mean_proj, int F, int fpad, int C,
+    const double* __restrict__ rscale , const bf16x8* __restrict__ comps , const float* __restrict__ mean_proj, int F, int fpad, int C,
     int cpad, float* __restrict__ out , long n)
 {
     extern __shared__ __attribute__((aligned(16))) char smem[];
@@ -140,7 +151,19 @@
 
     const int fp = tid & 63, cg = tid >> 6;
     float raw[16][2];
+    const bool pair_loads = !(F & 1) && !((uintptr_t)feat & 7);
     auto issue = [&](int k0) {
+        if (pair_loads) {
+            const int g = k0 + 2 * fp < F ? k0 + 2 * fp : F - 2;
+#pragma unroll
+            for (int c = 0; c < 16; ++c) {
+                const long cell = cell0 + cg * 16 + c < n ? cell0 + cg * 16 + c : n - 1;
+                const float2 v = *(const float2*)(feat + cell * F + g);
+                raw[c][0] = v.x;
+                raw[c][1] = v.y;
+            }
+            return;
+        }
         const int g0 = k0 + 2 * fp < F ? k0 + 2 * fp : F - 1, g1 = k0 + 2 * fp + 1 < F ? k0 + 2 * fp + 1 : F - 1;
 #pragma unroll
         for (int c = 0; c < 16; ++c) {
@@ -149,30 +172,47 @@
             raw[c][1] = feat[cell * F + g1];
         }
     };
+    auto split_store = [&](char* d, const float (&v)[2]) {
+        bf16x2 h1, h2, h3;
+#pragma unroll
+        for (int j = 0; j < 2; ++j) {
+            const __bf16 a1 = (__bf16)v[j];
+            const float r1 = v[j] - (float)a1;
+            const __bf16 a2 = (__bf16)r1;
+            const float r2 = r1 - (float)a2;
+            h1[j] = a1; h2[j] = a2; h3[j] = (__bf16)r2;
+        }
+        *(bf16x2*)d = h1;
+        *(bf16x2*)(d + PX_PLANE) = h2;
+        *(bf16x2*)(d + 2 * PX_PLANE) = h3;
+    };
     auto stash = [&](int k0) {
         const int gk = k0 + 2 * fp;
         const bool ok0 = gk < F, ok1 = gk + 1 < F;
         const float ctr0 = center[ok0 ? gk : 0], ctr1 = center[ok1 ? gk + 1 : 0];
-        const double scl0 = scale[ok0 ? gk : 0], scl1 = scale[ok1 ? gk + 1 : 0];
+        const double rsc0 = rscale[ok0 ? gk : 0], rsc1 = rscale[ok1 ? gk + 1 : 0];
         char* d = smem + (cg * 16) * PX_ROW + fp * 4;
+        bool redo = false;
 #pragma unroll
         for (int c = 0; c < 16; ++c) {
             const bool cok = cell0 + cg * 16 + c < n;
-            float v[2];
-            v[0] = (ok0 && cok) ? (float)((double)(raw[c][0] - ctr0) / scl0) : 0.0f;
-            v[1] = (ok1 && cok) ? (float)((double)(raw[c][1] - ctr1) / scl1) : 0.0f;
-            bf16x2 h1, h2, h3;
-#pragma unroll
-            for (int j = 0; j < 2; ++j) {
-                const __bf16 a1 = (__bf16)v[j];
-                const float r1 = v[j] - (float)a1;
-                const __bf16 a2 = (__bf16)r1;
-                const float r2 = r1 - (float)a2;
-                h1[j] = a1; h2[j] = a2; h3[j] = (__bf16)r2;
-            }
-            *(bf16x2*)(d + c * PX_ROW) = h1;
-            *(bf16x2*)(d + c * PX_ROW + PX_PLANE) = h2;
-            *(bf16x2*)(d + c * PX_ROW + 2 * PX_PLANE) = h3;
+            bool dv0, dv1;
+            const float q0 = scaled_feature_fast(raw[c][0] - ctr0, rsc0, dv0);
+            const float q1 = scaled_feature_fast(raw[c][1] - ctr1, rsc1, dv1);
+            redo |= dv0 | dv1;
+            const float v[2] = {(ok0 && cok) ? q0 : 0.0f, (ok1 && cok) ? q1 : 0.0f};
+            split_store(d + c * PX_ROW, v);
+        }
+        if (__builtin_expect(redo, 0)) {
+            const double scl0 = scale[ok0 ? gk : 0], scl1 = scale[ok1 ? gk + 1 : 0];
+            const int g0 = ok0 ? gk : F - 1, g1 = ok1 ? gk + 1 : F - 1;
+            for (int c = 0; c < 16; ++c) {
+                const bool cok = cell0 + cg * 16 + c < n;
+                const long cell = cok ? cell0 + cg * 16 + c : n - 1;
+                const float v[2] = {(ok0 && cok) ? (float)((double)(feat[cell * F + g0] - ctr0) / scl0) : 0.0f,
+                                    (ok1 && cok) ? (float)((double)(feat[cell * F + g1] - ctr1) / scl1) : 0.0f};
+                split_store(d + c * PX_ROW, v);
+            }
         }
     };
     const bf16x8* bp[2];
@@ -269,31 +309,32 @@
 constexpr int SVMM_WAVES = 8, SVMM_TILES = 2, SVMM_CELLS = SVMM_WAVES * SVMM_TILES * 16;
 
 struct SvmArgs {
-    const double* svT[2];
-    const double* svn[2];
-    const double* coef[2];
-    int nsv_pad[2];
+    const double* svT;
+    const double* svn;
+    const double* coef;
+    int nu_pad;
     double gamma[2], rho[2];
+    double* dec[2];
 };
 
 template <int KS, bool SPLIT>
 __global__ __launch_bounds__(64 * SVMM_WAVES, 1) void ocsvm_mfma_kernel(
-    const float* __restrict__ pca, int D, SvmArgs sa, double* __restrict__ dec , long n)
-{
-    const int det = (int)blockIdx.z;
-    const double* __restrict__ svT = sa.svT[det];
-    const double* __restrict__ svn = sa.svn[det];
-    const double* __restrict__ coef = sa.coef[det];
-    const int nsv_pad = sa.nsv_pad[det];
-    const double gamma = sa.gamma[det], rho = sa.rho[det];
-    constexpr int ROWS = 4 * KS + 2;
+    const float* __restrict__ pca, int D, SvmArgs sa, double* __restrict__ part , long n)
+{
+    const double* __restrict__ svT = sa.svT;
+    const double* __restrict__ svn = sa.svn;
+    const double* __restrict__ coef = sa.coef;
+    const int nsv_pad = sa.nu_pad;
+    const double ng0 = -sa.gamma[0], ng1 = -sa.gamma[1];
+    const bool one_exp = __double_as_longlong(sa.gamma[0]) == __double_as_longlong(sa.gamma[1]);
+    constexpr int ROWS = 4 * KS + 3;
     __shared__ double sb[2][ROWS][16];
     const int tid = threadIdx.x, lane = tid & 63, wave = tid >> 6;
     const int li = lane & 15, kq = lane >> 4;
     const long cell0 = (long)blockIdx.x * SVMM_CELLS + wave * (SVMM_TILES * 16);
 
     double xa[SVMM_TILES][KS];
-    double rown[SVMM_TILES][4];
+    __shared__ double sxn[SVMM_WAVES][SVMM_TILES][16];
 #pragma unroll
     for (int t = 0; t < SVMM_TILES; ++t) {
         long cell = cell0 + t * 16 + li;
@@ -308,8 +349,7 @@
         }
         nx += __shfl_xor(nx, 16);
         nx += __shfl_xor(nx, 32);
-#pragma unroll
-        for (int r = 0; r < 4; ++r) rown[t][r] = __shfl(nx, kq + 4 * r);
+        if (kq == 0) sxn[wave][t][li] = nx;
     }
 
     constexpr int NST = (ROWS * 16 + 64 * SVMM_WAVES - 1) / (64 * SVMM_WAVES);
@@ -322,6 +362,7 @@
             if (row < D) x = svT[(size_t)row * nsv_pad + sidx];
             else if (row == 4 * KS) x = svn[sidx];
             else if (row == 4 * KS + 1) x = coef[sidx];
+            else if (row == 4 * KS + 2) x = coef[(size_t)nsv_pad + sidx];
             v[j] = x;
         }
     };
@@ -342,11 +383,14 @@
     }
     __syncthreads();
 
-    double sum[SVMM_TILES][4], tot[SVMM_TILES][4];
-#pragma unroll
-    for (int t = 0; t < SVMM_TILES; ++t)
-#pragma unroll
-        for (int r = 0; r < 4; ++r) sum[t][r] = tot[t][r] = 0.0;
+    static_assert(2 * SVMM_TILES * 4 == 16, "one total per lane of a row");
+    double sum[2][SVMM_TILES][4], tot = 0.0;
+#pragma unroll
+    for (int k = 0; k < 2; ++k)
+#pragma unroll
+        for (int t = 0; t < SVMM_TILES; ++t)
+#pragma unroll
+            for (int r = 0; r < 4; ++r) sum[k][t][r] = 0.0;
     for (int blk = bbeg; blk < bend; ++blk) {
         const int cur = blk & 1;
         double nv[NST];
@@ -360,45 +404,61 @@
 #pragma unroll
             for (int t = 0; t < SVMM_TILES; ++t) acc[t] = __builtin_amdgcn_mfma_f64_16x16x4f64(xa[t][s], b, acc[t], 0, 0, 0);
         }
-        const double sn = sb[cur][4 * KS][li], cf = sb[cur][4 * KS + 1][li];
-#pragma unroll
-        for (int t = 0; t < SVMM_TILES; ++t)
-#pragma unroll
-            for (int r = 0; r < 4; ++r) {
-                const double d2 = fma(-2.0, acc[t][r], rown[t][r] + sn);
-                sum[t][r] = fma(cf, exp(-gamma * d2), sum[t][r]);
-            }
+        const double sn = sb[cur][4 * KS][li], cf0 = sb[cur][4 * KS + 1][li], cf1 = sb[cur][4 * KS + 2][li];
+        if (one_exp) {
+#pragma unroll
+            for (int t = 0; t < SVMM_TILES; ++t)
+#pragma unroll
+                for (int r = 0; r < 4; ++r) {
+                    const double d2 = fma(-2.0, acc[t][r], sxn[wave][t][kq + 4 * r] + sn);
+                    const double e = exp(ng0 * d2);
+                    sum[0][t][r] = fma(cf0, e, sum[0][t][r]);
+                    sum[1][t][r] = fma(cf1, e, sum[1][t][r]);
+                }
+        } else {
+#pragma unroll
+            for (int t = 0; t < SVMM_TILES; ++t)
+#pragma unroll
+                for (int r = 0; r < 4; ++r) {
+                    const double d2 = fma(-2.0, acc[t][r], sxn[wave][t][kq + 4 * r] + sn);
+                    sum[0][t][r] = fma(cf0, exp(ng0 * d2), sum[0][t][r]);
+                    sum[1][t][r] = fma(cf1, exp(ng1 * d2), sum[1][t][r]);
+                }
+        }
         if (blk + 1 < bend) stash(cur ^ 1, nv);
         __syncthreads();
         while (rj < DET_RANGES && nblk * (rj + 1) / DET_RANGES <= blk + 1) {
             if (nblk * (rj + 1) / DET_RANGES == blk + 1) {
 #pragma unroll
-                for (int t = 0; t < SVMM_TILES; ++t)
-#pragma unroll
-                    for (int r = 0; r < 4; ++r) {
-                        double v = sum[t][r];
-                        v += __shfl_xor(v, 1);
-                        v += __shfl_xor(v, 2);
-                        v += __shfl_xor(v, 4);
-                        v += __shfl_xor(v, 8);
-                        tot[t][r] += v;
-                        sum[t][r] = 0.0;
-                    }
+                for (int k = 0; k < 2; ++k)
+#pragma unroll
+                    for (int t = 0; t < SVMM_TILES; ++t)
+#pragma unroll
+                        for (int r = 0; r < 4; ++r) {
+                            double v = sum[k][t][r];
+                            v += __shfl_xor(v, 1);
+                            v += __shfl_xor(v, 2);
+                            v += __shfl_xor(v, 4);
+                            v += __shfl_xor(v, 8);
+                            if (li == (k * SVMM_TILES + t) * 4 + r) tot += v;
+                            sum[k][t][r] = 0.0;
+                        }
             }
             ++rj;
             if (SPLIT) break;
         }
     }
-#pragma unroll
-    for (int t = 0; t < SVMM_TILES; ++t)
-#pragma unroll
-        for (int r = 0; r < 4; ++r) {
-            const long cell = cell0 + t * 16 + kq + 4 * r;
-            if (li == 0 && cell < n) {
-                if constexpr (SPLIT) dec[((size_t)det * DET_RANGES + blockIdx.y) * n + cell] = tot[t][r];
-                else dec[cell] = tot[t][r] - rho;
-            }
-        }
+    {
+        const int k = li >> 3, t = (li >> 2) & 1, r = li & 3;
+        const long cell = cell0 + t * 16 + kq + 4 * r;
+        if (cell < n) {
+            if constexpr (SPLIT) part[((size_t)k * DET_RANGES + blockIdx.y) * n + cell] = tot;
+            else {
+                double* __restrict__ d = k ? sa.dec[1] : sa.dec[0];
+                if (d) d[cell] = tot - (k ? sa.rho[1] : sa.rho[0]);
+            }
+        }
+    }
 }
 
 __global__ void svm_split_sum_kernel(const double* __restrict__ part, double rho0, double rho1, double* __restrict__ dec0,
@@ -406,12 +466,12 @@
 {
     const long i = (long)blockIdx.x * blockDim.x + threadIdx.x;
     const int det = (int)blockIdx.y;
-    if (i >= n) return;
+    double* __restrict__ dec = det == 0 ? dec0 : dec1;
+    if (i >= n || !dec) return;
     double v = 0.0;
 #pragma unroll
     for (int j = 0; j < DET_RANGES; ++j) v += part[((size_t)det * DET_RANGES + j) * n + i];
-    if (det == 0) dec0[i] = v - rho0;
-    else dec1[i] = v - rho1;
+    dec[i] = v - (det == 0 ? rho0 : rho1);
 }
 
 
@@ -468,7 +528,7 @@
 
 }
 
-hipError_t launch_scaler_pca(const float* feat, const float* center, const double* scale,
+hipError_t launch_scaler_pca(const float* feat, const float* center, const double* scale, const double* rscale,
                              const float* comps_pad, const float* mean_proj, int F, int fpad, int C,
                              int cpad, float* pca_out, int64_t n_cells, hipStream_t stream)
 {
@@ -477,7 +537,7 @@
     const unsigned grid = (unsigned)((n_cells + PCA_CELLS - 1) / PCA_CELLS);
     KernelSetup ks;
     if (hipError_t e = kernel_setup<scaler_pca_kernel>(256, PCA_LDS, ks); e != hipSuccess) return e;
-    hipLaunchKernelGGL(scaler_pca_kernel, dim3(grid), dim3(256), PCA_LDS, stream, feat, center, scale,
+    hipLaunchKernelGGL(scaler_pca_kernel, dim3(grid), dim3(256), PCA_LDS, stream, feat, center, scale, rscale,
                        comps_pad, mean_proj, F, fpad, C, cpad, pca_out, (long)n_cells);
     return hipGetLastError();
 }
@@ -521,7 +581,7 @@
     return pca > svm ? pca : svm;
 }
 
-hipError_t launch_scaler_pca_x3(const float* feat, const float* center, const double* scale, const uint16_t* comps_planes,
+hipError_t launch_scaler_pca_x3(const float* feat, const float* center, const double* scale, const double* rscale, const uint16_t* comps_planes,
                                 const float* mean_proj, int F, int fpad, int C, int cpad, float* pca_out, int64_t n_cells,
                                 hipStream_t stream, void* split_ws)
 {
@@ -534,14 +594,14 @@
                                 : kernel_setup<scaler_pca_x3_kernel<true>>(256, PX_LDS, ks);
     if (e != hipSuccess) return e;
     if (split) {
-        hipLaunchKernelGGL(scaler_pca_x3_kernel<true>, dim3(grid, DET_RANGES), dim3(256), PX_LDS, stream, feat, center, scale,
+        hipLaunchKernelGGL(scaler_pca_x3_kernel<true>, dim3(grid, DET_RANGES), dim3(256), PX_LDS, stream, feat, center, scale, rscale,
                            (const bf16x8*)comps_planes, mean_proj, F, fpad, C, cpad, (float*)split_ws, (long)n_cells);
         const long tot = (long)n_cells * C;
         hipLaunchKernelGGL(pca_split_sum_kernel, dim3((unsigned)((tot + 255) / 256)), dim3(256), 0, stream, (const float*)split_ws, mean_proj,
                            C, pca_out, (long)n_cells);
         return hipGetLastError();
     }
-    hipLaunchKernelGGL(scaler_pca_x3_kernel<false>, dim3(grid), dim3(256), PX_LDS, stream, feat, center, scale, (const bf16x8*)comps_planes,
+    hipLaunchKernelGGL(scaler_pca_x3_kernel<false>, dim3(grid), dim3(256), PX_LDS, stream, feat, center, scale, rscale, (const bf16x8*)comps_planes,
                        mean_proj, F, fpad, C, cpad, pca_out, (long)n_cells);
     return hipGetLastError();
 }
@@ -555,34 +615,21 @@
         hipLaunchKernelGGL((ocsvm_mfma_kernel<32, SPLIT>), grid, dim3(64 * SVMM_WAVES), 0, stream, pca, D, sa, out, (long)n_cells);
 }
 
-hipError_t launch_ocsvm(const float* pca, int D, const double* svT, const double* svn, const double* coef, int nsv_pad, double gamma,
-                        double rho, double* dec, int64_t n_cells, hipStream_t stream, void* split_ws)
-{
-    if (n_cells <= 0) return hipSuccess;
-    if (!svT || !svn || !coef || D < 1 || D > 128 || nsv_pad % 16) return hipErrorInvalidValue;
+hipError_t launch_ocsvm_pair(const float* pca, int D, const double* svT, const double* svn, const double* coef2, int nu_pad,
+                             const double gamma[2], const double rho[2], double* dec0, double* dec1, int64_t n_cells, hipStream_t stream,
+                             void* split_ws)
+{
+    if (n_cells <= 0 || (!dec0 && !dec1)) return hipSuccess;
+    if (!svT || !svn || !coef2 || D < 1 || D > 128 || nu_pad < 16 || nu_pad % 16) return hipErrorInvalidValue;
     const unsigned grid = (unsigned)((n_cells + SVMM_CELLS - 1) / SVMM_CELLS);
-    SvmArgs sa{{svT, svT}, {svn, svn}, {coef, coef}, {nsv_pad, nsv_pad}, {gamma, gamma}, {rho, rho}};
+    SvmArgs sa{svT, svn, coef2, nu_pad, {gamma[0], gamma[1]}, {rho[0], rho[1]}, {dec0, dec1}};
     if (split_ws && n_cells <= DET_SPLIT_MAX_CELLS) {
-        ocsvm_launch<true>(pca, D, sa, (double*)split_ws, n_cells, dim3(grid, DET_RANGES, 1), stream);
-        hipLaunchKernelGGL(svm_split_sum_kernel, dim3((unsigned)((n_cells + 255) / 256), 1), dim3(256), 0, stream, (const double*)split_ws, rho, rho,
-                           dec, dec, (long)n_cells);
+        ocsvm_launch<true>(pca, D, sa, (double*)split_ws, n_cells, dim3(grid, DET_RANGES), stream);
+        hipLaunchKernelGGL(svm_split_sum_kernel, dim3((unsigned)((n_cells + 255) / 256), 2), dim3(256), 0, stream, (const double*)split_ws, rho[0], rho[1],
+                           dec0, dec1, (long)n_cells);
         return hipGetLastError();
     }
-    ocsvm_launch<false>(pca, D, sa, dec, n_cells, dim3(grid), stream);
-    return hipGetLastError();
-}
-
-hipError_t launch_ocsvm_pair_split(const float* pca, int D, const double* const svT[2], const double* const svn[2],
-                                   const double* const coef[2], const int nsv_pad[2], const double gamma[2], const double rho[2],
-                                   double* dec0, double* dec1, int64_t n_cells, hipStream_t stream, void* split_ws)
-{
-    if (n_cells <= 0) return hipSuccess;
-    if (!split_ws || n_cells > DET_SPLIT_MAX_CELLS || D < 1 || D > 128 || nsv_pad[0] % 16 || nsv_pad[1] % 16) return hipErrorInvalidValue;
-    const unsigned grid = (unsigned)((n_cells + SVMM_CELLS - 1) / SVMM_CELLS);
-    SvmArgs sa{{svT[0], svT[1]}, {svn[0], svn[1]}, {coef[0], coef[1]}, {nsv_pad[0], nsv_pad[1]}, {gamma[0], gamma[1]}, {rho[0], rho[1]}};
-    ocsvm_launch<true>(pca, D, sa, (double*)split_ws, n_cells, dim3(grid, DET_RANGES, 2), stream);
-    hipLaunchKernelGGL(svm_split_sum_kernel, dim3((unsigned)((n_cells + 255) / 256), 2), dim3(256), 0, stream, (const double*)split_ws, rho[0], rho[1],
-                       dec0, dec1, (long)n_cells);
+    ocsvm_launch<false>(pca, D, sa, nullptr, n_cells, dim3(grid), stream);
     return hipGetLastError();
 }
 
diff --git a/cell-image-analysis_amd/csrc/fit.hip b/cell-image-analysis_amd/csrc/fit.hip
--- a/cell-image-analysis_amd/csrc/fit.hip
+++ b/cell-image-analysis_amd/csrc/fit.hip
@@ -1,4 +1,5 @@
 #include "api_internal.hpp"
+#include "scaled_feature.hpp"
 
 #include <hip/hip_runtime.h>
 
@@ -616,7 +617,7 @@
     int device = 0;
     hipStream_t stream = nullptr;
     hipEvent_t ev0 = nullptr, ev1 = nullptr;
-    DevBuf feat, keys, sel, nanc, cen, scl, xs, mean, part, scat, comps, mproj, proj;
+    DevBuf feat, keys, sel, nanc, cen, scl, rscl, xs, mean, part, scat, comps, mproj, proj;
     DevBuf x, xT, xsq, alpha0, alpha1, G0, G1, Qi, part_i, part_j, state;
     DevBuf sxT, sY, sQ, sZ, sgram, st, sfresh, ssq;
     double last_ms = 0.0;
@@ -836,16 +837,19 @@
     const int fpad = (F + 511) / 512 * 512, cpad = (C + 15) / 16 * 16;
     std::vector<float> cp((size_t)cpad * fpad, 0.0f);
     for (int c = 0; c < C; ++c) memcpy(&cp[(size_t)c * fpad], components + (size_t)c * F, sizeof(float) * F);
-    if ((rc = f->cen.ensure(sizeof(float) * F)) || (rc = f->scl.ensure(sizeof(double) * F)) ||
+    std::vector<double> rs(F);
+    for (int k = 0; k < F; ++k) rs[k] = scaler_reciprocal(scale[k]);
+    if ((rc = f->cen.ensure(sizeof(float) * F)) || (rc = f->scl.ensure(sizeof(double) * F)) || (rc = f->rscl.ensure(sizeof(double) * F)) ||
         (rc = f->comps.ensure(cp.size() * sizeof(float))) || (rc = f->mproj.ensure(sizeof(float) * C)) ||
         (rc = f->proj.ensure((size_t)n * C * sizeof(float))))
         return rc;
     HIPCHK(hipMemcpyAsync(f->cen.p, center, sizeof(float) * F, hipMemcpyHostToDevice, f->stream));
     HIPCHK(hipMemcpyAsync(f->scl.p, scale, sizeof(double) * F, hipMemcpyHostToDevice, f->stream));
+    HIPCHK(hipMemcpyAsync(f->rscl.p, rs.data(), sizeof(double) * F, hipMemcpyHostToDevice, f->stream));
     HIPCHK(hipMemcpyAsync(f->comps.p, cp.data(), cp.size() * sizeof(float), hipMemcpyHostToDevice, f->stream));
     HIPCHK(hipMemcpyAsync(f->mproj.p, mean_proj, sizeof(float) * C, hipMemcpyHostToDevice, f->stream));
     Timer tm(f);
-    HIPCHK(launch_scaler_pca(d_feat, f->cen.as<float>(), f->scl.as<double>(), f->comps.as<float>(), f->mproj.as<float>(), F, fpad, C,
+    HIPCHK(launch_scaler_pca(d_feat, f->cen.as<float>(), f->scl.as<double>(), f->rscl.as<double>(), f->comps.as<float>(), f->mproj.as<float>(), F, fpad, C,
                              cpad, f->proj.as<float>(), n, f->stream));
     HIPCHK(hipMemcpyAsync(out, f->proj.p, (size_t)n * C * sizeof(float), hipMemcpyDeviceToHost, f->stream));
     return tm.stop();
diff --git a/cell-image-analysis_amd/csrc/scaled_feature.hpp b/cell-image-analysis_amd/csrc/scaled_feature.hpp
--- /dev/null
+++ b/cell-image-analysis_amd/csrc/scaled_feature.hpp
@@ -0,0 +1,56 @@
+#pragma once
+
+#include <cstdint>
+#include <cstring>
+
+#if defined(__HIPCC__) || defined(__CUDACC__)
+#define CS_SF_HD __host__ __device__ __forceinline__
+#else
+#define CS_SF_HD inline
+#endif
+
+namespace cs {
+
+inline double scaler_reciprocal(double scale)
+{
+    const double r = 1.0 / scale;
+    uint64_t b;
+    memcpy(&b, &r, 8);
+    const unsigned e = (unsigned)(b >> 52) & 0x7ffu;
+    if (e == 0 || e == 0x7ffu) {
+        const uint64_t qnan = 0x7ff8000000000000ULL;
+        double n;
+        memcpy(&n, &qnan, 8);
+        return n;
+    }
+    return r;
+}
+
+CS_SF_HD float scaled_feature_fast(float t, double rscale, bool& divide)
+{
+    const double q = (double)t * rscale;
+    uint64_t b;
+#if defined(__HIP_DEVICE_COMPILE__)
+    b = (uint64_t)__double_as_longlong(q);
+#else
+    memcpy(&b, &q, 8);
+#endif
+    const uint32_t lo = (uint32_t)b, hi = (uint32_t)(b >> 32);
+    const bool near_midpoint = ((lo - 0x0ffffff8u) & 0x1fffffffu) <= 16u;
+    const bool out_of_range = (((hi >> 20) & 0x7ffu) - (1023u - 125u)) >= 252u;
+    const bool zero = ((hi << 1) | lo) == 0u;
+    divide = near_midpoint | (out_of_range & !zero);
+    return (float)q;
+}
+
+CS_SF_HD float scaled_feature(float x, float center, double scale, double rscale, bool* divided = nullptr)
+{
+    const float t = x - center;
+    bool divide;
+    const float v = scaled_feature_fast(t, rscale, divide);
+    if (divided) *divided = divide;
+    if (__builtin_expect(divide, 0)) return (float)((double)t / scale);
+    return v;
+}
+
+}
```

Result: no change. 5.477 million cells/s (median of 3 runs) (+0.5%).
